# neuraloperator/pde-policylearning

Hardware: NVIDIA B200
Metric: fno2d_fwd_bwd_samples_per_s (higher is better)
Workload: dtype f32

## Files before the change

include/b2no.h:

```cpp
#ifndef B2NO_H
#define B2NO_H

#include <stdint.h>

#ifdef __cplusplus
extern "C" {
#endif

#define B2NO_MAX_DIM 3
#define B2NO_ABI_VERSION 5

enum { B2NO_NORM_BACKWARD = 0, B2NO_NORM_FORWARD = 1, B2NO_NORM_ORTHO = 2 };
enum { B2NO_ACT_NONE = 0, B2NO_ACT_GELU = 1, B2NO_ACT_RELU = 2, B2NO_ACT_SIGMOID = 3, B2NO_ACT_SELU = 4,
       B2NO_ACT_TANH = 5 };
enum { B2NO_E_ARG = -1, B2NO_E_UNSUPPORTED = -2, B2NO_E_NODEVICE = -3 };

typedef struct {
  int32_t ndim;
  int32_t nin[B2NO_MAX_DIM];
  int32_t nfft[B2NO_MAX_DIM];
  int32_t nout[B2NO_MAX_DIM];
  int32_t half[B2NO_MAX_DIM];
  int32_t norm;
  int32_t spec_layout;
} b2no_geom;

typedef struct b2no_plan b2no_plan;

typedef struct {
  const float* corner[4];
  int64_t stride_i, stride_o;
  int64_t stride_k[B2NO_MAX_DIM];
} b2no_weights;

typedef struct {
  const float* bias;
  const float* pw_w;  const float* pw_x;  int32_t pw_ci;  int32_t pw_transposed;
  const float* pw2_w; const float* pw2_x; int32_t pw2_ci; int32_t pw2_transposed;
  const float* add;
  const float* mul;
  float* preact;
  int32_t act;
  const float* dact_z;
  int32_t dact;
  const float* gate_z;
  const float* gate_h;
  int64_t mul_bstride;
  int64_t gate_bstride;
} b2no_epilogue;

int b2no_version(void);
const char* b2no_error_string(int code);
int b2no_device_info(int* sm_count, int* cc_major, int* cc_minor, int64_t* l2_bytes);

int b2no_plan_create(const b2no_geom* geom, b2no_plan** out);
int b2no_plan_destroy(b2no_plan* plan);
int b2no_plan_layout_supported(const b2no_plan* plan, int64_t batch, int64_t channels);
int b2no_plan_kept(const b2no_plan* plan, int32_t kept[B2NO_MAX_DIM]);
int64_t b2no_plan_workspace_floats(const b2no_plan* plan, int64_t batch, int64_t channels);
int b2no_set_tensor_core_mode(int on);
int b2no_set_precision(int mode);
int64_t b2no_tensor_core_launches(void);

int b2no_dft_forward(const b2no_plan* plan, int which, const float* x, float* spec, float* work,
                     int64_t bc, void* stream);
int b2no_dft_inverse(const b2no_plan* plan, int which, const float* spec, float* y, float* work,
                     int batch, int channels, int64_t pixels, const b2no_epilogue* epi, void* stream);

int b2no_mix(const b2no_plan* plan, int mode, const float* in, const b2no_weights* w, float* out,
             int batch, int ci, int co, int accumulate, void* stream);
int b2no_mix_dw(const b2no_plan* plan, const float* xh, const float* gyh, const b2no_weights* dw,
                int batch, int ci, int co, int accumulate, void* stream);

int b2no_act_bwd(const float* gy, const float* z, float* gz, int64_t n, int act, void* stream);
int64_t b2no_pw_wgrad_scratch_floats(int ci, int co);
int b2no_pw_wgrad(const float* g, const float* x, float* dw, float* db, float* partial, int batch, int ci,
                  int co, int64_t pixels, void* stream);
int b2no_dft_inverse_wgrad(const b2no_plan* plan, int which, const float* spec, float* y, float* work, int batch, int channels,
                           int64_t pixels, const b2no_epilogue* epi, const float* wg_x, int wg_ci, float* dw, float* db,
                           float* partial, void* stream);
int b2no_mlp_head_fwd(const float* x, const float* w1, const float* b1, const float* w2, const float* b2,
                      float* out, int batch, int ci, int hidden, int64_t pixels, int b1_per_sample,
                      int act, void* stream);
int64_t b2no_mlp_head_bwd_scratch_floats(int hidden);
int b2no_mlp_head_bwd_supported(int ci, int hidden, int64_t pixels);
int b2no_mlp_head_bwd(const float* x, const float* w1, const float* b1, const float* w2, const float* g, float* gx,
                      float* gz, float* dw2, float* partial, int batch, int ci, int hidden, int64_t pixels,
                      int b1_per_sample, int act, const float* dact_z, int dact, void* stream);
int64_t b2no_mlp_head_bwd_fused_scratch_floats(int ci, int hidden);
int b2no_mlp_head_bwd_fused_supported(int ci, int hidden, int64_t pixels);
int b2no_mlp_head_bwd_fused(const float* x, const float* w1, const float* b1, const float* w2, const float* g, float* gx,
                            float* grads, float* partial, int batch, int ci, int hidden, int64_t pixels, int act,
                            const float* dact_z, int dact, void* stream);
int b2no_rno_gate_fwd(const float* z, const float* z2, const float* hhat, const float* h, float* out,
                      int64_t n, void* stream);
int b2no_rno_gate_bwd(const float* g, const float* z, const float* z2, const float* hhat, const float* h,
                      float* gz, float* gz2, float* ghhat, float* gh, int64_t n, void* stream);
int b2no_rno_cell_bwd(const float* g, const float* h, const float* zz2, const float* ah, float* g_zz2, float* g_ah,
                      float* g_h, int batch, int c, int64_t p, void* stream);
int b2no_rno_reset_bwd(const float* g_rh, const float* h, const float* ar, float* g_ar, float* g_h, int64_t n,
                       void* stream);
int b2no_rel_l2_sums(const float* x, const float* y, float* sums, int batch, int64_t n_per_sample, void* stream);
int b2no_rel_l2_bwd(const float* x, const float* y, const float* coef, float* dx, int batch,
                    int64_t n_per_sample, void* stream);
int b2no_rel_l2_finish(const float* sums, float* loss, float* coef, int batch, int size_average, void* stream);
int b2no_rel_l2_bwd_g(const float* x, const float* y, const float* coef, const float* g, float* dx, int batch,
                      int64_t n_per_sample, void* stream);

int64_t b2no_pino_residual_scratch_floats(int B, int N, int T, int which);
int b2no_pino_residual_fwd(const float* w, const float* u0, const float* forcing, const float* nu, float t_interval,
                           float* du_p, float* fields, float* partial, float* loss, float* coef, int B, int N, int T,
                           void* stream);
int b2no_pino_residual_bwd(const float* w, const float* u0, const float* forcing, const float* nu, float t_interval,
                           const float* du_p, const float* fields, const float* coef, const float* gup, float* dw,
                           int B, int N, int T, void* stream);

int b2no_adam_step(float* param, const float* grad, float* exp_avg, float* exp_avg_sq, int64_t n, int* step_counter,
                   float lr, float beta1, float beta2, float eps, float weight_decay, float grad_scale, void* stream);
int64_t b2no_kernel_launches(void);

int b2no_gather_segments(float* flat, const void* src_ptrs, const int64_t* offsets, const int64_t* counts, int nseg,
                         void* stream);

int b2no_tc_peak_probe(int kind, int n_mma, double* flops, void* stream);

#ifdef __cplusplus
}
#endif
#endif
```

pde_policylearning_b200/_lib.py:

```python
from __future__ import annotations

import ctypes as C
import os
import subprocess
import sys

_HERE = os.path.dirname(os.path.abspath(__file__))
LIB_PATH = os.environ.get("B2NO_LIB") or os.path.join(_HERE, "libb2no.so")
CSRC = os.path.join(_HERE, "csrc")
SOURCES = ["plan.cu", "spectral.cu", "pointwise.cu", "tc_pointwise.cu", "tc_wgrad.cu", "tc_mlp.cu", "tc_head_bwd.cu", "tc_dft.cu", "tc_mix.cu", "tc_peak.cu", "pino_loss.cu", "optim.cu"]

MAX_DIM = 3
NORM = {"backward": 0, "forward": 1, "ortho": 2}
ACT = {None: 0, "none": 0, "identity": 0, "gelu": 1, "relu": 2, "sigmoid": 3, "selu": 4, "tanh": 5}


class Geom(C.Structure):
    _fields_ = [("ndim", C.c_int32), ("nin", C.c_int32 * MAX_DIM), ("nfft", C.c_int32 * MAX_DIM),
                ("nout", C.c_int32 * MAX_DIM), ("half", C.c_int32 * MAX_DIM), ("norm", C.c_int32),
                ("spec_layout", C.c_int32)]


class Weights(C.Structure):
    _fields_ = [("corner", C.c_void_p * 4), ("stride_i", C.c_int64), ("stride_o", C.c_int64),
                ("stride_k", C.c_int64 * MAX_DIM)]


class Epilogue(C.Structure):
    _fields_ = [("bias", C.c_void_p),
                ("pw_w", C.c_void_p), ("pw_x", C.c_void_p), ("pw_ci", C.c_int32), ("pw_transposed", C.c_int32),
                ("pw2_w", C.c_void_p), ("pw2_x", C.c_void_p), ("pw2_ci", C.c_int32), ("pw2_transposed", C.c_int32),
                ("add", C.c_void_p), ("mul", C.c_void_p), ("preact", C.c_void_p), ("act", C.c_int32),
                ("dact_z", C.c_void_p), ("dact", C.c_int32),
                ("gate_z", C.c_void_p), ("gate_h", C.c_void_p), ("mul_bstride", C.c_int64), ("gate_bstride", C.c_int64)]


NVCC_FLAGS = ["-O3", "-std=c++17", "-gencode", "arch=compute_100a,code=sm_100a", "-lineinfo", "-Xcompiler", "-fPIC"]
HEADERS = [os.path.join(CSRC, "common.cuh"), os.path.join(CSRC, "tc.cuh"), os.path.join(_HERE, "..", "include", "b2no.h")]


def build(force: bool = False, verbose: bool = False) -> str:
    from concurrent.futures import ThreadPoolExecutor
    hdr_time = max(os.path.getmtime(h) for h in HEADERS)
    if not force and os.path.exists(LIB_PATH) and os.path.getmtime(LIB_PATH) >= max(
            [hdr_time] + [os.path.getmtime(os.path.join(CSRC, s)) for s in SOURCES]):
        return LIB_PATH
    bdir = os.path.join(CSRC, "_build")
    os.makedirs(bdir, exist_ok=True)
    jobs, objs = [], []
    for s in SOURCES:
        src, obj = os.path.join(CSRC, s), os.path.join(bdir, s[:-3] + ".o")
        objs.append(obj)
        if force or not os.path.exists(obj) or os.path.getmtime(obj) < max(os.path.getmtime(src), hdr_time):
            jobs.append(["nvcc"] + NVCC_FLAGS + ["-c", "-o", obj, src])
    if not jobs and os.path.exists(LIB_PATH) and os.path.getmtime(LIB_PATH) >= max(os.path.getmtime(o) for o in objs):
        return LIB_PATH

    def run(cmd):
        if verbose:
            print(" ".join(cmd), file=sys.stderr)
        subprocess.run(cmd, check=True)

    with ThreadPoolExecutor(max_workers=min(8, max(1, len(jobs)))) as ex:
        list(ex.map(run, jobs))
    run(["nvcc"] + NVCC_FLAGS + ["-shared", "-o", LIB_PATH] + objs)
    return LIB_PATH


_lib = None


def lib():
    global _lib
    if _lib is not None:
        return _lib
    if not os.path.exists(LIB_PATH):
        raise RuntimeError(
            f"{LIB_PATH} not found: build it with `python -c 'import __graft_entry__ as g; g.build()'` "
            "(nvcc, sm_100a).  There is no CPU / PyTorch fallback for the spectral-conv hot path.")
    L = C.CDLL(LIB_PATH)
    vp, i32, i64 = C.c_void_p, C.c_int, C.c_int64
    L.b2no_version.restype = i32
    L.b2no_error_string.restype = C.c_char_p
    L.b2no_error_string.argtypes = [i32]
    L.b2no_device_info.argtypes = [C.POINTER(i32), C.POINTER(i32), C.POINTER(i32), C.POINTER(i64)]
    L.b2no_plan_create.argtypes = [C.POINTER(Geom), C.POINTER(vp)]
    L.b2no_plan_destroy.argtypes = [vp]
    L.b2no_plan_kept.argtypes = [vp, C.POINTER(C.c_int32 * MAX_DIM)]
    L.b2no_plan_layout_supported.argtypes = [vp, i64, i64]
    L.b2no_plan_workspace_floats.restype = i64
    L.b2no_plan_workspace_floats.argtypes = [vp, i64, i64]
    L.b2no_set_tensor_core_mode.argtypes = [i32]
    L.b2no_set_precision.argtypes = [i32]
    L.b2no_tensor_core_launches.restype = i64
    L.b2no_kernel_launches.restype = i64
    L.b2no_dft_forward.argtypes = [vp, i32, vp, vp, vp, i64, vp]
    L.b2no_dft_inverse.argtypes = [vp, i32, vp, vp, vp, i32, i32, i64, C.POINTER(Epilogue), vp]
    L.b2no_mix.argtypes = [vp, i32, vp, C.POINTER(Weights), vp, i32, i32, i32, i32, vp]
    L.b2no_mix_dw.argtypes = [vp, vp, vp, C.POINTER(Weights), i32, i32, i32, i32, vp]
    L.b2no_act_bwd.argtypes = [vp, vp, vp, i64, i32, vp]
    L.b2no_pw_wgrad_scratch_floats.restype = i64
    L.b2no_pw_wgrad_scratch_floats.argtypes = [i32, i32]
    L.b2no_pw_wgrad.argtypes = [vp, vp, vp, vp, vp, i32, i32, i32, i64, vp]
    L.b2no_dft_inverse_wgrad.argtypes = [vp, i32, vp, vp, vp, i32, i32, i64, C.POINTER(Epilogue), vp, i32, vp, vp, vp, vp]
    L.b2no_mlp_head_fwd.argtypes = [vp, vp, vp, vp, vp, vp, i32, i32, i32, i64, i32, i32, vp]
    L.b2no_mlp_head_bwd_supported.argtypes = [i32, i32, i64]
    L.b2no_mlp_head_bwd_scratch_floats.restype = i64
    L.b2no_mlp_head_bwd_scratch_floats.argtypes = [i32]
    L.b2no_mlp_head_bwd.argtypes = [vp] * 9 + [i32, i32, i32, i64, i32, i32, vp, i32, vp]
    L.b2no_mlp_head_bwd_fused_supported.argtypes = [i32, i32, i64]
    L.b2no_mlp_head_bwd_fused_scratch_floats.restype = i64
    L.b2no_mlp_head_bwd_fused_scratch_floats.argtypes = [i32, i32]
    L.b2no_mlp_head_bwd_fused.argtypes = [vp] * 8 + [i32, i32, i32, i64, i32, vp, i32, vp]
    L.b2no_rno_gate_fwd.argtypes = [vp, vp, vp, vp, vp, i64, vp]
    L.b2no_rno_gate_bwd.argtypes = [vp] * 9 + [i64, vp]
    L.b2no_rno_cell_bwd.argtypes = [vp] * 7 + [i32, i32, i64, vp]
    L.b2no_rno_reset_bwd.argtypes = [vp] * 5 + [i64, vp]
    L.b2no_rel_l2_sums.argtypes = [vp, vp, vp, i32, i64, vp]
    L.b2no_rel_l2_bwd.argtypes = [vp, vp, vp, vp, i32, i64, vp]
    L.b2no_rel_l2_finish.argtypes = [vp, vp, vp, i32, i32, vp]
    L.b2no_rel_l2_bwd_g.argtypes = [vp, vp, vp, vp, vp, i32, i64, vp]
    L.b2no_gather_segments.argtypes = [vp, vp, vp, vp, i32, vp]
    f32 = C.c_float
    L.b2no_adam_step.argtypes = [vp, vp, vp, vp, i64, vp, f32, f32, f32, f32, f32, f32, vp]
    L.b2no_pino_residual_scratch_floats.restype = i64
    L.b2no_pino_residual_scratch_floats.argtypes = [i32, i32, i32, i32]
    L.b2no_pino_residual_fwd.argtypes = [vp, vp, vp, vp, f32, vp, vp, vp, vp, vp, i32, i32, i32, vp]
    L.b2no_pino_residual_bwd.argtypes = [vp, vp, vp, vp, f32, vp, vp, vp, vp, vp, i32, i32, i32, vp]
    L.b2no_tc_peak_probe.argtypes = [i32, i32, C.POINTER(C.c_double), vp]
    for name in EXPORTS:
        getattr(L, name)
    _lib = L
    return L


EXPORTS = [
    "b2no_version", "b2no_error_string", "b2no_device_info",
    "b2no_plan_create", "b2no_plan_destroy", "b2no_plan_kept", "b2no_plan_layout_supported", "b2no_plan_workspace_floats",
    "b2no_set_tensor_core_mode", "b2no_set_precision", "b2no_tensor_core_launches", "b2no_kernel_launches",
    "b2no_dft_forward", "b2no_dft_inverse", "b2no_mix", "b2no_mix_dw",
    "b2no_act_bwd", "b2no_pw_wgrad_scratch_floats", "b2no_pw_wgrad", "b2no_dft_inverse_wgrad", "b2no_mlp_head_fwd", "b2no_mlp_head_bwd_scratch_floats", "b2no_mlp_head_bwd_supported", "b2no_mlp_head_bwd",
    "b2no_mlp_head_bwd_fused_scratch_floats", "b2no_mlp_head_bwd_fused_supported", "b2no_mlp_head_bwd_fused",
    "b2no_rno_gate_fwd", "b2no_rno_gate_bwd", "b2no_rno_cell_bwd", "b2no_rno_reset_bwd", "b2no_rel_l2_sums", "b2no_rel_l2_bwd",
    "b2no_rel_l2_finish", "b2no_rel_l2_bwd_g", "b2no_adam_step", "b2no_gather_segments",
    "b2no_tc_peak_probe", "b2no_pino_residual_scratch_floats", "b2no_pino_residual_fwd", "b2no_pino_residual_bwd",
]


def check(code: int, what: str = "") -> None:
    if code != 0:
        msg = lib().b2no_error_string(int(code)).decode()
        raise RuntimeError(f"b2no {what} failed: {msg} (code {code})")
```

pde_policylearning_b200/csrc/common.cuh:

```cuda
#pragma once
#include <cuda_runtime.h>
#include <stdint.h>
#include "../../include/b2no.h"

#define B2NO_CHECK_CUDA(expr)                      \
  do {                                             \
    cudaError_t _e = (expr);                       \
    if (_e != cudaSuccess) return (int)_e;         \
  } while (0)

extern long long g_b2no_launches;
#define B2NO_LAUNCH_CHECK()                        \
  do {                                             \
    cudaError_t _e = cudaGetLastError();           \
    if (_e != cudaSuccess) return (int)_e;         \
    g_b2no_launches++;                             \
  } while (0)

static inline int b2no_ceil_div(long a, long b) { return (int)((a + b - 1) / b); }
static inline int b2no_round_up(int a, int b) { return ((a + b - 1) / b) * b; }

int b2no_sm_count();
int b2no_tc_passes();
bool b2no_tc_available();
int b2no_tc_mlp_fwd(const float* x, const float* w1, const float* b1, const float* w2, const float* b2, float* out, int batch,
                    int ci, int hidden, int co2, long pixels, int b1_per_sample, int act, cudaStream_t st);
int b2no_tc_wgrad(const float* g, const float* x, float* partial, int max_blocks, int batch, int ci, int co, long pixels,
                  int* nblk, cudaStream_t st);
struct b2no_tc_wg {
  const float* x;
  int ci;
  float* partial;
  int* nblk;
};
int b2no_tc_pointwise(const b2no_plan* plan, int which, const float* spec, float* y, float* work, int batch, int channels,
                      long pixels, const b2no_epilogue* e, cudaStream_t st, const b2no_tc_wg* wg = nullptr);

struct b2no_tc_tables {
  float* timg;
  int Ks, Qp, R;
};

struct b2no_tc_fwd_tables {
  float* tb;
  float* mimg;
  int W, H, N1, Kx, Ky;
};
int b2no_tc_dft_forward(const b2no_plan* plan, int which, const float* x, float* spec, long planes, cudaStream_t st);

struct b2no_plan {
  b2no_geom g;
  b2no_tc_tables tc[2];
  b2no_tc_fwd_tables tcf[2];
  int K[B2NO_MAX_DIM];
  int device;
  float* t_in;
  float* t_out;
  int npad_in, npad_out, q2, qc, nchunk, qpad;
  float2* m_fwd[2];
  float2* m_inv[2];
  float2* m_adjinv[2];
  float2* m_adjfwd[2];
  int* row_corner[2];
  int* row_local[2];
};

struct ModeMap {
  const int* corner[2];
  const int* local[2];
  int K[3];
  int ndim;
};

__device__ __forceinline__ void decode_mode(const ModeMap& mm, const b2no_weights& w, int k, int* corner,
                                            long* woff) {
  int c = 0;
  long off = 0;
  const int d = mm.ndim;
  int rem = k;
  int idx[3] = {0, 0, 0};
  for (int j = d - 1; j >= 0; j--) {
    idx[j] = rem % mm.K[j];
    rem /= mm.K[j];
  }
  for (int j = 0; j < d - 1; j++) {
    c = c * 2 + mm.corner[j][idx[j]];
    off += (long)mm.local[j][idx[j]] * w.stride_k[j];
  }
  off += (long)idx[d - 1] * w.stride_k[d - 1];
  *corner = c;
  *woff = off;
}

static inline ModeMap make_mode_map(const b2no_plan* p) {
  ModeMap mm;
  mm.ndim = p->g.ndim;
  for (int j = 0; j < 3; j++) mm.K[j] = j < p->g.ndim ? p->K[j] : 1;
  for (int j = 0; j < 2; j++) { mm.corner[j] = p->row_corner[j]; mm.local[j] = p->row_local[j]; }
  return mm;
}

static inline int total_modes(const b2no_plan* p) {
  int kt = 1;
  for (int j = 0; j < p->g.ndim; j++) kt *= p->K[j];
  return kt;
}

int b2no_tc_mix_feasible(int batch, int ci, int co, int mode);
int b2no_tc_mix_dw_feasible(int batch, int ci, int co);
int b2no_tc_mix(const b2no_plan* p, int mode, const float* in, const b2no_weights* w, float* out, int batch, int ci, int co,
                int accumulate, cudaStream_t st);
int b2no_tc_mix_dw(const b2no_plan* p, const float* xh, const float* gyh, const b2no_weights* dw, int batch, int ci, int co,
                   int accumulate, cudaStream_t st);

__device__ __forceinline__ float b2no_erf(float x) {
  x = fminf(fmaxf(x, -4.0f), 4.0f);
  const float x2 = x * x;
  float p = -2.72614225801306e-10f;
  p = fmaf(p, x2, 2.77068142495902e-08f);
  p = fmaf(p, x2, -2.10102402082508e-06f);
  p = fmaf(p, x2, -5.69250639462346e-05f);
  p = fmaf(p, x2, -7.34990630326855e-04f);
  p = fmaf(p, x2, -2.95459980854025e-03f);
  p = fmaf(p, x2, -1.60960333262415e-02f);
  float q = -1.45660718464996e-05f;
  q = fmaf(q, x2, -2.13374055278905e-04f);
  q = fmaf(q, x2, -1.68282697438203e-03f);
  q = fmaf(q, x2, -7.37332916720468e-03f);
  q = fmaf(q, x2, -1.42647390514189e-02f);
  return __fdividef(x * p, q);
}

__device__ __forceinline__ float2 b2no_f2(float a) { return make_float2(a, a); }
__device__ __forceinline__ float b2no_rcp(float x) {
  float r;
  asm("rcp.approx.ftz.f32 %0, %1;" : "=f"(r) : "f"(x));
  return r;
}
__device__ __forceinline__ float b2no_ex2(float x) {
  float r;
  asm("ex2.approx.ftz.f32 %0, %1;" : "=f"(r) : "f"(x));
  return r;
}
__device__ __forceinline__ float2 b2no_erf2(float2 x) {
  x.x = fminf(fmaxf(x.x, -4.0f), 4.0f);
  x.y = fminf(fmaxf(x.y, -4.0f), 4.0f);
  const float2 x2 = __fmul2_rn(x, x);
  float2 p = b2no_f2(-2.72614225801306e-10f);
  p = __ffma2_rn(p, x2, b2no_f2(2.77068142495902e-08f));
  p = __ffma2_rn(p, x2, b2no_f2(-2.10102402082508e-06f));
  p = __ffma2_rn(p, x2, b2no_f2(-5.69250639462346e-05f));
  p = __ffma2_rn(p, x2, b2no_f2(-7.34990630326855e-04f));
  p = __ffma2_rn(p, x2, b2no_f2(-2.95459980854025e-03f));
  p = __ffma2_rn(p, x2, b2no_f2(-1.60960333262415e-02f));
  float2 q = b2no_f2(-1.45660718464996e-05f);
  q = __ffma2_rn(q, x2, b2no_f2(-2.13374055278905e-04f));
  q = __ffma2_rn(q, x2, b2no_f2(-1.68282697438203e-03f));
  q = __ffma2_rn(q, x2, b2no_f2(-7.37332916720468e-03f));
  q = __ffma2_rn(q, x2, b2no_f2(-1.42647390514189e-02f));
  const float2 r = make_float2(b2no_rcp(q.x), b2no_rcp(q.y));
  return __fmul2_rn(__fmul2_rn(x, p), r);
}
__device__ __forceinline__ float2 b2no_gelu2(float2 x) {
  const float2 e = b2no_erf2(__fmul2_rn(x, b2no_f2(0.70710678118654752440f)));
  const float2 h = __fmul2_rn(x, b2no_f2(0.5f));
  return __ffma2_rn(h, e, h);
}
__device__ __forceinline__ void b2no_gelu2_both(float2 x, float2* val, float2* grad) {
  const float2 ax = make_float2(fabsf(x.x), fabsf(x.y));
  const float2 den = __ffma2_rn(ax, b2no_f2(0.23164189f), b2no_f2(1.0f));
  const float2 t = make_float2(b2no_rcp(den.x), b2no_rcp(den.y));
  float2 q = __ffma2_rn(b2no_f2(1.061405429f), t, b2no_f2(-1.453152027f));
  q = __ffma2_rn(q, t, b2no_f2(1.421413741f));
  q = __ffma2_rn(q, t, b2no_f2(-0.284496736f));
  q = __ffma2_rn(q, t, b2no_f2(0.254829592f));
  q = __fmul2_rn(q, t);
  const float2 a = __fmul2_rn(__fmul2_rn(x, x), b2no_f2(-0.72134752044448170368f));
  const float2 g = make_float2(b2no_ex2(a.x), b2no_ex2(a.y));
  const float2 h = __ffma2_rn(__fmul2_rn(q, g), b2no_f2(-0.5f), b2no_f2(0.5f));
  const float2 cdf = __fadd2_rn(b2no_f2(0.5f), make_float2(copysignf(h.x, x.x), copysignf(h.y, x.y)));
  *val = __fmul2_rn(x, cdf);
  *grad = __ffma2_rn(__fmul2_rn(x, b2no_f2(0.39894228040143267794f)), g, cdf);
}
__device__ __forceinline__ float2 b2no_gelu2_grad(float2 x) {
  float2 v, g;
  b2no_gelu2_both(x, &v, &g);
  return g;
}

__device__ __forceinline__ float b2no_act(float x, int act) {
  switch (act) {
    case B2NO_ACT_GELU: return 0.5f * x * (1.0f + b2no_erf(x * 0.70710678118654752440f));
    case B2NO_ACT_RELU: return x > 0.f ? x : 0.f;
    case B2NO_ACT_SIGMOID: return 1.0f / (1.0f + expf(-x));
    case B2NO_ACT_SELU: {
      const float scale = 1.0507009873554804934193349852946f, alpha = 1.6732632423543772848170429916717f;
      return x > 0.f ? scale * x : scale * alpha * expm1f(x);
    }
    case B2NO_ACT_TANH: return tanhf(x);
    default: return x;
  }
}

__device__ __forceinline__ float b2no_act_grad(float x, int act) {
  switch (act) {
    case B2NO_ACT_GELU: {
      const float cdf = 0.5f * (1.0f + b2no_erf(x * 0.70710678118654752440f));
      const float pdf = 0.39894228040143267794f * __expf(-0.5f * x * x);
      return cdf + x * pdf;
    }
    case B2NO_ACT_RELU: return x > 0.f ? 1.f : 0.f;
    case B2NO_ACT_SIGMOID: {
      const float s = 1.0f / (1.0f + expf(-x));
      return s * (1.0f - s);
    }
    case B2NO_ACT_SELU: {
      const float scale = 1.0507009873554804934193349852946f, alpha = 1.6732632423543772848170429916717f;
      return x > 0.f ? scale : scale * alpha * expf(x);
    }
    case B2NO_ACT_TANH: {
      const float t = tanhf(x);
      return 1.0f - t * t;
    }
    default: return 1.f;
  }
}
```

pde_policylearning_b200/csrc/spectral.cu:

```cuda
#include <string.h>
#include "common.cuh"

template <int QC>
__global__ void __launch_bounds__(256)
k_r2c_last(const float* __restrict__ x, float* __restrict__ out, const float* __restrict__ tab,
           long R, int N, int npad, int q2, int nchunk) {
  extern __shared__ float s_tab[];
  const int qpad = QC * nchunk;
  for (int i = threadIdx.x; i < qpad * npad; i += blockDim.x) s_tab[i] = tab[i];
  __syncthreads();

  const int lane = threadIdx.x & 31, warp = threadIdx.x >> 5;
  const int npl = (N + 31) >> 5;
  const long ngroups = (R + 7) >> 3;
  for (long g = (long)blockIdx.x * 8 + warp; g < ngroups; g += (long)gridDim.x * 8) {
    const long r0 = g << 3;
    for (int c = 0; c < nchunk; c++) {
      float v[8 * QC];
#pragma unroll
      for (int i = 0; i < 8 * QC; i++) v[i] = 0.f;
      for (int j = 0; j < npl; j++) {
        const int n = lane + (j << 5);
        float xv[8];
#pragma unroll
        for (int r = 0; r < 8; r++) xv[r] = (n < N && r0 + r < R) ? __ldg(x + (r0 + r) * N + n) : 0.f;
        const float* tq = s_tab + (size_t)(c * QC) * npad + n;
#pragma unroll
        for (int q = 0; q < QC; q++) {
          const float t = tq[(size_t)q * npad];
#pragma unroll
          for (int r = 0; r < 8; r++) v[r * QC + q] = fmaf(xv[r], t, v[r * QC + q]);
        }
      }
#pragma unroll
      for (int s = 0; s < 5; s++) {
        const int off = 16 >> s;
        const int half = (8 * QC) >> (s + 1);
        const bool upper = (lane & off) != 0;
#pragma unroll
        for (int i = 0; i < half; i++) {
          const float a = v[i], b = v[i + half];
          const float send = upper ? a : b;
          const float keep = upper ? b : a;
          v[i] = keep + __shfl_xor_sync(0xffffffffu, send, off);
        }
      }
      constexpr int PER = QC / 4;
#pragma unroll
      for (int i = 0; i < PER; i++) {
        const int idx = lane * PER + i;
        const int r = idx / QC, q = c * QC + idx % QC;
        if (r0 + r < R && q < q2) out[(r0 + r) * q2 + q] = v[i];
      }
    }
  }
}

template <int QC>
static int launch_r2c(const float* x, float* out, const float* tab, long R, int N, int npad, int q2,
                      int nchunk, cudaStream_t st) {
  const size_t smem = (size_t)QC * nchunk * npad * sizeof(float);
  if (smem > 200 * 1024) return B2NO_E_UNSUPPORTED;
  if (smem > 48 * 1024)
    B2NO_CHECK_CUDA(cudaFuncSetAttribute(k_r2c_last<QC>, cudaFuncAttributeMaxDynamicSharedMemorySize, (int)smem));
  const long ngroups = (R + 7) / 8;
  long blocks = (ngroups + 7) / 8;
  const long cap = (long)b2no_sm_count() * 8;
  if (blocks > cap) blocks = cap;
  if (blocks < 1) blocks = 1;
  k_r2c_last<QC><<<(unsigned)blocks, 256, smem, st>>>(x, out, tab, R, N, npad, q2, nchunk);
  B2NO_LAUNCH_CHECK();
  return 0;
}

template <int QL>
__global__ void __launch_bounds__(256)
k_r2c_rows(const float* __restrict__ x, float* __restrict__ out, const float* __restrict__ tab, long R, int N, int npad, int q2) {
  extern __shared__ float s_dyn[];
  constexpr int Q2P = 4 * QL;
  float* s_tabT = s_dyn;
  float* s_rows = s_dyn + (size_t)N * Q2P;
  for (int i = threadIdx.x; i < N * Q2P; i += 256) {
    const int n = i / Q2P, q = i - n * Q2P;
    s_tabT[i] = q < q2 ? tab[(size_t)q * npad + n] : 0.f;
  }
  __syncthreads();
  const int lane = threadIdx.x & 31, warp = threadIdx.x >> 5;
  float* rows = s_rows + (size_t)warp * 8 * N;
  const int r = lane >> 2, q0 = (lane & 3) * QL;
  const long ngroups = R >> 3;
  for (long g = (long)blockIdx.x * 8 + warp; g < ngroups; g += (long)gridDim.x * 8) {
    const float4* src = reinterpret_cast<const float4*>(x + (g << 3) * N);
    for (int i = lane; i < 2 * N; i += 32) reinterpret_cast<float4*>(rows)[i] = __ldg(src + i);
    __syncwarp();
    float acc[QL];
#pragma unroll
    for (int i = 0; i < QL; i++) acc[i] = 0.f;
    const float* xr = rows + r * N;
#pragma unroll 4
    for (int n = 0; n < N; n++) {
      const float xv = xr[n];
      const float* t = s_tabT + n * Q2P + q0;
#pragma unroll
      for (int i = 0; i < QL; i++) acc[i] = fmaf(xv, t[i], acc[i]);
    }
    float* dst = out + ((g << 3) + r) * q2 + q0;
#pragma unroll
    for (int i = 0; i < QL; i++)
      if (q0 + i < q2) dst[i] = acc[i];
    __syncwarp();
  }
}

template <int Q2P>
__global__ void __launch_bounds__(256)
k_r2c_rows32(const float* __restrict__ x, float* __restrict__ out, const float* __restrict__ tab, long R, int N, int npad, int q2) {
  extern __shared__ float s_dyn[];
  const int NS = N | 1;
  float* s_tabT = s_dyn;
  float* s_rows = s_dyn + (size_t)N * Q2P;
  for (int i = threadIdx.x; i < N * Q2P; i += 256) {
    const int n = i / Q2P, q = i - n * Q2P;
    s_tabT[i] = q < q2 ? tab[(size_t)q * npad + n] : 0.f;
  }
  __syncthreads();
  const int lane = threadIdx.x & 31, warp = threadIdx.x >> 5;
  float* rows = s_rows + (size_t)warp * 32 * NS;
  const long ngroups = R >> 5;
  for (long g = (long)blockIdx.x * 8 + warp; g < ngroups; g += (long)gridDim.x * 8) {
    const float* src = x + (g << 5) * N;
    if (NS == N) {
      const float4* s4 = reinterpret_cast<const float4*>(src);
      for (int i = lane; i < 8 * N; i += 32) reinterpret_cast<float4*>(rows)[i] = __ldg(s4 + i);
    } else {
      for (int i = lane; i < 32 * N; i += 32) {
        const int rr = i / N, n = i - rr * N;
        rows[rr * NS + n] = __ldg(src + i);
      }
    }
    __syncwarp();
    float acc[Q2P];
#pragma unroll
    for (int i = 0; i < Q2P; i++) acc[i] = 0.f;
    const float* xr = rows + lane * NS;
#pragma unroll 2
    for (int n = 0; n < N; n++) {
      const float xv = xr[n];
      const float4* t4 = reinterpret_cast<const float4*>(s_tabT + n * Q2P);
#pragma unroll
      for (int i = 0; i < Q2P / 4; i++) {
        const float4 t = t4[i];
        acc[4 * i] = fmaf(xv, t.x, acc[4 * i]);
        acc[4 * i + 1] = fmaf(xv, t.y, acc[4 * i + 1]);
        acc[4 * i + 2] = fmaf(xv, t.z, acc[4 * i + 2]);
        acc[4 * i + 3] = fmaf(xv, t.w, acc[4 * i + 3]);
      }
    }
    float* dst = out + ((g << 5) + lane) * q2;
    if (q2 == Q2P) {
#pragma unroll
      for (int i = 0; i < Q2P / 4; i++)
        reinterpret_cast<float4*>(dst)[i] = make_float4(acc[4 * i], acc[4 * i + 1], acc[4 * i + 2], acc[4 * i + 3]);
    } else {
#pragma unroll
      for (int i = 0; i < Q2P; i++)
        if (i < q2) dst[i] = acc[i];
    }
    __syncwarp();
  }
}

template <int Q2P>
static int launch_r2c_rows32(const float* x, float* out, const float* tab, long R, int N, int npad, int q2, cudaStream_t st) {
  const size_t smem = ((size_t)N * Q2P + (size_t)8 * 32 * (N | 1)) * sizeof(float);
  if (smem > 48 * 1024)
    B2NO_CHECK_CUDA(cudaFuncSetAttribute(k_r2c_rows32<Q2P>, cudaFuncAttributeMaxDynamicSharedMemorySize, (int)smem));
  const long ngroups = R / 32;
  long blocks = (ngroups + 7) / 8;
  const long cap = (long)b2no_sm_count() * 4;
  if (blocks > cap) blocks = cap;
  if (blocks < 1) blocks = 1;
  k_r2c_rows32<Q2P><<<(unsigned)blocks, 256, smem, st>>>(x, out, tab, R, N, npad, q2);
  B2NO_LAUNCH_CHECK();
  return 0;
}

template <int QL>
static int launch_r2c_rows(const float* x, float* out, const float* tab, long R, int N, int npad, int q2, cudaStream_t st) {
  const size_t smem = ((size_t)N * 4 * QL + (size_t)8 * 8 * N) * sizeof(float);
  if (smem > 48 * 1024)
    B2NO_CHECK_CUDA(cudaFuncSetAttribute(k_r2c_rows<QL>, cudaFuncAttributeMaxDynamicSharedMemorySize, (int)smem));
  const long ngroups = R / 8;
  long blocks = (ngroups + 7) / 8;
  const long cap = (long)b2no_sm_count() * 8;
  if (blocks > cap) blocks = cap;
  if (blocks < 1) blocks = 1;
  k_r2c_rows<QL><<<(unsigned)blocks, 256, smem, st>>>(x, out, tab, R, N, npad, q2);
  B2NO_LAUNCH_CHECK();
  return 0;
}

static int run_r2c(const b2no_plan* p, int which, const float* x, float* out, long R, cudaStream_t st) {
  const int d = p->g.ndim;
  const int N = which == 0 ? p->g.nin[d - 1] : p->g.nout[d - 1];
  const int npad = which == 0 ? p->npad_in : p->npad_out;
  const float* tab = which == 0 ? p->t_in : p->t_out;
  if (R % 32 == 0 && R >= 32 * 8 * 64 && p->q2 <= 16 && p->q2 % 4 == 0 && N >= 8 && N <= 160 && (((uintptr_t)x) & 15) == 0 &&
      (((uintptr_t)out) & 15) == 0) {
    if (p->q2 <= 8) return launch_r2c_rows32<8>(x, out, tab, R, N, npad, p->q2, st);
    return launch_r2c_rows32<16>(x, out, tab, R, N, npad, p->q2, st);
  }
  if (R % 8 == 0 && p->q2 <= 16 && N >= 8 && N <= 512 && (((uintptr_t)x) & 15) == 0) {
    if (p->q2 <= 4) return launch_r2c_rows<1>(x, out, tab, R, N, npad, p->q2, st);
    if (p->q2 <= 8) return launch_r2c_rows<2>(x, out, tab, R, N, npad, p->q2, st);
    return launch_r2c_rows<4>(x, out, tab, R, N, npad, p->q2, st);
  }
  switch (p->qc) {
    case 4: return launch_r2c<4>(x, out, tab, R, N, npad, p->q2, p->nchunk, st);
    case 8: return launch_r2c<8>(x, out, tab, R, N, npad, p->q2, p->nchunk, st);
    case 12: return launch_r2c<12>(x, out, tab, R, N, npad, p->q2, p->nchunk, st);
    case 16: return launch_r2c<16>(x, out, tab, R, N, npad, p->q2, p->nchunk, st);
  }
  return B2NO_E_UNSUPPORTED;
}

template <int MT>
__global__ void __launch_bounds__(128)
k_cmat(const float2* __restrict__ in, float2* __restrict__ out, const float2* __restrict__ T,
       long outer, int J, int M, int inner) {
  extern __shared__ float2 s_T[];
  const int m0 = blockIdx.y * MT;
  for (int idx = threadIdx.x; idx < J * MT; idx += blockDim.x) {
    const int j = idx / MT, mm = idx - j * MT;
    s_T[idx] = (m0 + mm < M) ? T[(size_t)j * M + m0 + mm] : make_float2(0.f, 0.f);
  }
  __syncthreads();
  const long total = outer * inner;
  for (long t = (long)blockIdx.x * blockDim.x + threadIdx.x; t < total; t += (long)gridDim.x * blockDim.x) {
    const long o = t / inner;
    const int i = (int)(t - o * inner);
    float2 acc[MT];
#pragma unroll
    for (int mm = 0; mm < MT; mm++) acc[mm] = make_float2(0.f, 0.f);
    const float2* src = in + (o * J) * inner + i;
#pragma unroll 4
    for (int j = 0; j < J; j++) {
      const float2 v = __ldg(src + (size_t)j * inner);
      const float2* trow = s_T + j * MT;
#pragma unroll
      for (int mm = 0; mm < MT; mm++) {
        const float2 w = trow[mm];
        acc[mm].x = fmaf(v.x, w.x, fmaf(-v.y, w.y, acc[mm].x));
        acc[mm].y = fmaf(v.x, w.y, fmaf(v.y, w.x, acc[mm].y));
      }
    }
#pragma unroll
    for (int mm = 0; mm < MT; mm++)
      if (m0 + mm < M) out[(o * M + m0 + mm) * inner + i] = acc[mm];
  }
}

template <int MT>
static int launch_cmat(const float2* in, float2* out, const float2* T, long outer, int J, int M, int inner,
                       cudaStream_t st) {
  const size_t smem = (size_t)J * MT * sizeof(float2);
  if (smem > 200 * 1024) return B2NO_E_UNSUPPORTED;
  if (smem > 48 * 1024)
    B2NO_CHECK_CUDA(cudaFuncSetAttribute(k_cmat<MT>, cudaFuncAttributeMaxDynamicSharedMemorySize, (int)smem));
  const long total = outer * inner;
  long bx = (total + 127) / 128;
  const long cap = (long)b2no_sm_count() * 16;
  if (bx > cap) bx = cap;
  if (bx < 1) bx = 1;
  dim3 grid((unsigned)bx, (unsigned)((M + MT - 1) / MT));
  k_cmat<MT><<<grid, 128, smem, st>>>(in, out, T, outer, J, M, inner);
  B2NO_LAUNCH_CHECK();
  return 0;
}

static int run_cmat(const float2* in, float2* out, const float2* T, long outer, int J, int M, int inner,
                    cudaStream_t st) {
  if (M <= 4) return launch_cmat<4>(in, out, T, outer, J, M, inner, st);
  if (M <= 8) return launch_cmat<8>(in, out, T, outer, J, M, inner, st);
  if (M <= 12 || M == 24) return launch_cmat<12>(in, out, T, outer, J, M, inner, st);
  return launch_cmat<16>(in, out, T, outer, J, M, inner, st);
}

template <int KL>
__global__ void __launch_bounds__(256)
k_fwd_plane32(const float* __restrict__ x, float2* __restrict__ spec, const float* __restrict__ tab, int npad,
              const float2* __restrict__ M, long planes, int H, int W, int K0, int Kl, int layout) {
  extern __shared__ float2 sm2[];
  float2* sT = sm2;
  float2* sM = sT + 32 * KL;
  float2* sA = sM + 32 * 32;
  const int lane = threadIdx.x & 31, warp = threadIdx.x >> 5;
  for (int i = threadIdx.x; i < 32 * KL; i += 256) {
    const int w = i / KL, ky = i - w * KL;
    sT[i] = (w < W && ky < Kl) ? make_float2(__ldg(tab + (size_t)(2 * ky) * npad + w), __ldg(tab + (size_t)(2 * ky + 1) * npad + w))
                               : make_float2(0.f, 0.f);
  }
  for (int i = threadIdx.x; i < 32 * 32; i += 256) {
    const int h = i >> 5, kx = i & 31;
    sM[i] = (h < H && kx < K0) ? __ldg(M + (size_t)h * K0 + kx) : make_float2(0.f, 0.f);
  }
  __syncthreads();
  float2* myA = sA + (size_t)warp * 32 * (KL + 2);
  for (long p0 = (long)blockIdx.x * 8; p0 < planes; p0 += (long)gridDim.x * 8) {
    const long plane = p0 + warp;
    const bool live = plane < planes;
    float xr[32];
#pragma unroll
    for (int w = 0; w < 32; w++) xr[w] = 0.f;
    if (live && lane < H) {
      const float4* row = reinterpret_cast<const float4*>(x + ((size_t)plane * H + lane) * W);
#pragma unroll
      for (int w4 = 0; w4 < 8; w4++)
        if (w4 * 4 < W) {
          const float4 v = __ldg(row + w4);
          xr[4 * w4] = v.x; xr[4 * w4 + 1] = v.y; xr[4 * w4 + 2] = v.z; xr[4 * w4 + 3] = v.w;
        }
    }
    float2 acc[KL];
#pragma unroll
    for (int k = 0; k < KL; k++) acc[k] = make_float2(0.f, 0.f);
#pragma unroll
    for (int w = 0; w < 32; w++) {
      if (w < W) {
        const float2 xx = make_float2(xr[w], xr[w]);
#pragma unroll
        for (int k = 0; k < KL; k += 2) {
          const float4 t = *reinterpret_cast<const float4*>(sT + w * KL + k);
          acc[k] = __ffma2_rn(xx, make_float2(t.x, t.y), acc[k]);
          acc[k + 1] = __ffma2_rn(xx, make_float2(t.z, t.w), acc[k + 1]);
        }
      }
    }
#pragma unroll
    for (int k = 0; k < KL; k++) myA[lane * (KL + 2) + k] = acc[k];
    __syncwarp();
    float2 pr[KL], pi[KL];
#pragma unroll
    for (int k = 0; k < KL; k++) { pr[k] = make_float2(0.f, 0.f); pi[k] = make_float2(0.f, 0.f); }
    for (int h = 0; h < H; h++) {
      const float2 m = sM[h * 32 + lane];
      const float2 mr = make_float2(m.x, m.x), mi = make_float2(m.y, m.y);
#pragma unroll
      for (int k = 0; k < KL; k += 2) {
        const float4 a = *reinterpret_cast<const float4*>(myA + h * (KL + 2) + k);
        pr[k] = __ffma2_rn(mr, make_float2(a.x, a.y), pr[k]);
        pi[k] = __ffma2_rn(mi, make_float2(a.x, a.y), pi[k]);
        pr[k + 1] = __ffma2_rn(mr, make_float2(a.z, a.w), pr[k + 1]);
        pi[k + 1] = __ffma2_rn(mi, make_float2(a.z, a.w), pi[k + 1]);
      }
    }
    if (layout == 0) {
      if (live && lane < K0) {
        float2* dst = spec + ((size_t)plane * K0 + lane) * Kl;
#pragma unroll
        for (int k = 0; k < KL; k++)
          if (k < Kl) dst[k] = make_float2(pr[k].x - pi[k].y, pr[k].y + pi[k].x);
      }
      __syncwarp();
    } else {
      if (live && lane < K0) {
        float2* dst = spec + (size_t)lane * Kl * planes + plane;
#pragma unroll
        for (int k = 0; k < KL; k++)
          if (k < Kl) dst[(size_t)k * planes] = make_float2(pr[k].x - pi[k].y, pr[k].y + pi[k].x);
      }
      __syncwarp();
    }
  }
}

static int launch_fwd_plane32(const b2no_plan* p, int which, const float* x, float* spec, long planes, cudaStream_t st) {
  const int32_t* n = which == 0 ? p->g.nin : p->g.nout;
  const int H = n[0], W = n[1], K0 = p->K[0], Kl = p->K[1];
  const float* tab = which == 0 ? p->t_in : p->t_out;
  const int npad = which == 0 ? p->npad_in : p->npad_out;
  const float2* M = which == 0 ? p->m_fwd[0] : p->m_adjinv[0];
  const int KL = Kl <= 8 ? 8 : (Kl <= 12 ? 12 : 16);
  const size_t smem = sizeof(float2) * ((size_t)32 * KL + 32 * 32 + (size_t)8 * 32 * (KL + 2));
  long blocks = (planes + 7) / 8;
  const long cap = (long)b2no_sm_count() * 8;
  if (blocks > cap) blocks = cap;
#define FP32_LAUNCH(K)                                                                                                      \
  do {                                                                                                                      \
    if (smem > 48 * 1024) B2NO_CHECK_CUDA(cudaFuncSetAttribute(k_fwd_plane32<K>, cudaFuncAttributeMaxDynamicSharedMemorySize, (int)smem)); \
    k_fwd_plane32<K><<<(unsigned)blocks, 256, smem, st>>>(x, (float2*)spec, tab, npad, M, planes, H, W, K0, Kl, p->g.spec_layout); \
  } while (0)
  if (KL == 8) FP32_LAUNCH(8); else if (KL == 12) FP32_LAUNCH(12); else FP32_LAUNCH(16);
#undef FP32_LAUNCH
  B2NO_LAUNCH_CHECK();
  return 0;
}

extern "C" int b2no_dft_forward(const b2no_plan* p, int which, const float* x, float* spec, float* work,
                                int64_t bc, void* stream) {
  if (!p || !x || !spec || bc < 1 || (which != 0 && which != 1)) return B2NO_E_ARG;
  cudaStream_t st = (cudaStream_t)stream;
  const int d = p->g.ndim;
  const int32_t* n = which == 0 ? p->g.nin : p->g.nout;
  const int Kl = p->K[d - 1];
  if (d == 1) return run_r2c(p, which, x, spec, bc, st);
  if (d == 2) {
    if (n[0] <= 32 && n[1] <= 32 && n[1] % 4 == 0 && p->K[0] <= 32 && Kl <= 16 && (((uintptr_t)x) & 15) == 0 &&
        (p->g.spec_layout == 0 || p->g.spec_layout == 1))
      return launch_fwd_plane32(p, which, x, spec, (long)bc, st);
    const int rc = b2no_tc_dft_forward(p, which, x, spec, (long)bc, st);
    if (rc != 1) return rc;
  }
  if (p->g.spec_layout != 0) return B2NO_E_UNSUPPORTED;
  if (!work) return B2NO_E_ARG;
  float2* A = (float2*)work;
  if (d == 2) {
    int rc = run_r2c(p, which, x, (float*)A, bc * n[0], st);
    if (rc) return rc;
    const float2* T = which == 0 ? p->m_fwd[0] : p->m_adjinv[0];
    return run_cmat(A, (float2*)spec, T, bc, n[0], p->K[0], Kl, st);
  }
  float2* Bb = A + (size_t)bc * n[0] * n[1] * Kl;
  int rc = run_r2c(p, which, x, (float*)A, bc * n[0] * n[1], st);
  if (rc) return rc;
  const float2* T1 = which == 0 ? p->m_fwd[1] : p->m_adjinv[1];
  rc = run_cmat(A, Bb, T1, bc * n[0], n[1], p->K[1], Kl, st);
  if (rc) return rc;
  const float2* T0 = which == 0 ? p->m_fwd[0] : p->m_adjinv[0];
  return run_cmat(Bb, (float2*)spec, T0, bc, n[0], p->K[0], p->K[1] * Kl, st);
}

template <int BT, int PT, bool CONJT>
__global__ void __launch_bounds__(128)
k_mix(const float2* __restrict__ in, float2* __restrict__ out, b2no_weights w, ModeMap mm, int B, int Cq,
      int Cp, int Kt, int accumulate) {
  const int k = blockIdx.x * blockDim.x + threadIdx.x;
  if (k >= Kt) return;
  const int b0 = blockIdx.y * BT, p0 = blockIdx.z * PT;
  int corner;
  long woff;
  decode_mode(mm, w, k, &corner, &woff);
  const float2* wbase = (const float2*)w.corner[corner] + woff;
  float2 acc[BT][PT];
#pragma unroll
  for (int bb = 0; bb < BT; bb++)
#pragma unroll
    for (int pp = 0; pp < PT; pp++) acc[bb][pp] = make_float2(0.f, 0.f);
  for (int q = 0; q < Cq; q++) {
    float2 xin[BT], wv[PT];
#pragma unroll
    for (int bb = 0; bb < BT; bb++)
      xin[bb] = (b0 + bb < B) ? __ldg(in + ((size_t)(b0 + bb) * Cq + q) * Kt + k) : make_float2(0.f, 0.f);
#pragma unroll
    for (int pp = 0; pp < PT; pp++) {
      float2 t = make_float2(0.f, 0.f);
      if (p0 + pp < Cp) {
        const long off = CONJT ? ((long)(p0 + pp) * w.stride_i + (long)q * w.stride_o)
                               : ((long)q * w.stride_i + (long)(p0 + pp) * w.stride_o);
        t = __ldg(wbase + off);
        if (CONJT) t.y = -t.y;
      }
      wv[pp] = t;
    }
#pragma unroll
    for (int bb = 0; bb < BT; bb++)
#pragma unroll
      for (int pp = 0; pp < PT; pp++) {
        acc[bb][pp].x = fmaf(xin[bb].x, wv[pp].x, fmaf(-xin[bb].y, wv[pp].y, acc[bb][pp].x));
        acc[bb][pp].y = fmaf(xin[bb].x, wv[pp].y, fmaf(xin[bb].y, wv[pp].x, acc[bb][pp].y));
      }
  }
#pragma unroll
  for (int bb = 0; bb < BT; bb++)
#pragma unroll
    for (int pp = 0; pp < PT; pp++)
      if (b0 + bb < B && p0 + pp < Cp) {
        float2* dst = out + ((size_t)(b0 + bb) * Cp + p0 + pp) * Kt + k;
        float2 r = acc[bb][pp];
        if (accumulate) { const float2 old = *dst; r.x += old.x; r.y += old.y; }
        *dst = r;
      }
}

template <bool CONJT>
__global__ void __launch_bounds__(256)
k_mix2(const float2* __restrict__ in, float2* __restrict__ out, b2no_weights w, ModeMap mm, int B, int Cq, int Cp,
       int Kt, int accumulate) {
  const long idx = (long)blockIdx.x * 256 + threadIdx.x;
  if (idx >= (long)B * Cp * Kt) return;
  const int k = (int)(idx % Kt);
  const long t = idx / Kt;
  const int pp = (int)(t % Cp), b = (int)(t / Cp);
  int corner;
  long woff;
  decode_mode(mm, w, k, &corner, &woff);
  const float2* wp = (const float2*)w.corner[corner] + woff + (CONJT ? (long)pp * w.stride_i : (long)pp * w.stride_o);
  const long wq = CONJT ? w.stride_o : w.stride_i;
  const float2* xp = in + (size_t)b * Cq * Kt + k;
  float2 acc = make_float2(0.f, 0.f);
  int q = 0;
  for (; q + 8 <= Cq; q += 8) {
    float2 xv[8], wv[8];
#pragma unroll
    for (int u = 0; u < 8; u++) {
      xv[u] = __ldg(xp + (size_t)(q + u) * Kt);
      wv[u] = __ldg(wp + (long)(q + u) * wq);
    }
#pragma unroll
    for (int u = 0; u < 8; u++) {
      const float wy = CONJT ? -wv[u].y : wv[u].y;
      acc.x = fmaf(xv[u].x, wv[u].x, fmaf(-xv[u].y, wy, acc.x));
      acc.y = fmaf(xv[u].x, wy, fmaf(xv[u].y, wv[u].x, acc.y));
    }
  }
  for (; q < Cq; q++) {
    const float2 xv = __ldg(xp + (size_t)q * Kt), wv = __ldg(wp + (long)q * wq);
    const float wy = CONJT ? -wv.y : wv.y;
    acc.x = fmaf(xv.x, wv.x, fmaf(-xv.y, wy, acc.x));
    acc.y = fmaf(xv.x, wy, fmaf(xv.y, wv.x, acc.y));
  }
  float2* dst = out + ((size_t)b * Cp + pp) * Kt + k;
  if (accumulate) { const float2 old = *dst; acc.x += old.x; acc.y += old.y; }
  *dst = acc;
}

__global__ void __launch_bounds__(256)
k_dw2(const float2* __restrict__ xh, const float2* __restrict__ gyh, b2no_weights w, ModeMap mm, int B, int Ci, int Co,
      int Kt, int accumulate) {
  const long idx = (long)blockIdx.x * 256 + threadIdx.x;
  if (idx >= (long)Ci * Co * Kt) return;
  const int k = (int)(idx % Kt);
  const long t = idx / Kt;
  const int o = (int)(t % Co), i = (int)(t / Co);
  const float2* xp = xh + (size_t)i * Kt + k;
  const float2* gp = gyh + (size_t)o * Kt + k;
  const size_t xs = (size_t)Ci * Kt, gs = (size_t)Co * Kt;
  float2 acc = make_float2(0.f, 0.f);
  int b = 0;
  for (; b + 8 <= B; b += 8) {
    float2 xv[8], gv[8];
#pragma unroll
    for (int u = 0; u < 8; u++) {
      xv[u] = __ldg(xp + (size_t)(b + u) * xs);
      gv[u] = __ldg(gp + (size_t)(b + u) * gs);
    }
#pragma unroll
    for (int u = 0; u < 8; u++) {
      acc.x = fmaf(xv[u].x, gv[u].x, fmaf(xv[u].y, gv[u].y, acc.x));
      acc.y = fmaf(xv[u].x, gv[u].y, fmaf(-xv[u].y, gv[u].x, acc.y));
    }
  }
  for (; b < B; b++) {
    const float2 xv = __ldg(xp + (size_t)b * xs), gv = __ldg(gp + (size_t)b * gs);
    acc.x = fmaf(xv.x, gv.x, fmaf(xv.y, gv.y, acc.x));
    acc.y = fmaf(xv.x, gv.y, fmaf(-xv.y, gv.x, acc.y));
  }
  int corner;
  long woff;
  decode_mode(mm, w, k, &corner, &woff);
  float2* dst = (float2*)w.corner[corner] + woff + (long)i * w.stride_i + (long)o * w.stride_o;
  if (accumulate) { const float2 old = *dst; acc.x += old.x; acc.y += old.y; }
  *dst = acc;
}

extern "C" int b2no_mix(const b2no_plan* p, int mode, const float* in, const b2no_weights* w, float* out,
                        int batch, int ci, int co, int accumulate, void* stream) {
  if (!p || !in || !w || !out || batch < 1 || ci < 1 || co < 1 || (mode != 0 && mode != 1)) return B2NO_E_ARG;
  cudaStream_t st = (cudaStream_t)stream;
  const int Kt = total_modes(p);
  const ModeMap mm = make_mode_map(p);
  {
    const int rc = b2no_tc_mix(p, mode, in, w, out, batch, ci, co, accumulate, st);
    if (rc != 1) return rc;
  }
  if (p->g.spec_layout != 0) return B2NO_E_UNSUPPORTED;
  const int Cq = mode == 0 ? ci : co, Cp = mode == 0 ? co : ci;
  const long total = (long)batch * Cp * Kt;
  const unsigned blocks = (unsigned)((total + 255) / 256);
  if (mode == 0)
    k_mix2<false><<<blocks, 256, 0, st>>>((const float2*)in, (float2*)out, *w, mm, batch, Cq, Cp, Kt, accumulate);
  else
    k_mix2<true><<<blocks, 256, 0, st>>>((const float2*)in, (float2*)out, *w, mm, batch, Cq, Cp, Kt, accumulate);
  B2NO_LAUNCH_CHECK();
  return 0;
}

template <int IT, int OT>
__global__ void __launch_bounds__(128)
k_dw(const float2* __restrict__ xh, const float2* __restrict__ gyh, b2no_weights w, ModeMap mm, int B, int Ci,
     int Co, int Kt, int accumulate) {
  const int k = blockIdx.x * blockDim.x + threadIdx.x;
  if (k >= Kt) return;
  const int i0 = blockIdx.y * IT, o0 = blockIdx.z * OT;
  int corner;
  long woff;
  decode_mode(mm, w, k, &corner, &woff);
  float2 acc[IT][OT];
#pragma unroll
  for (int ii = 0; ii < IT; ii++)
#pragma unroll
    for (int oo = 0; oo < OT; oo++) acc[ii][oo] = make_float2(0.f, 0.f);
  for (int b = 0; b < B; b++) {
    float2 xi[IT], go[OT];
#pragma unroll
    for (int ii = 0; ii < IT; ii++)
      xi[ii] = (i0 + ii < Ci) ? __ldg(xh + ((size_t)b * Ci + i0 + ii) * Kt + k) : make_float2(0.f, 0.f);
#pragma unroll
    for (int oo = 0; oo < OT; oo++)
      go[oo] = (o0 + oo < Co) ? __ldg(gyh + ((size_t)b * Co + o0 + oo) * Kt + k) : make_float2(0.f, 0.f);
#pragma unroll
    for (int ii = 0; ii < IT; ii++)
#pragma unroll
      for (int oo = 0; oo < OT; oo++) {
        acc[ii][oo].x = fmaf(xi[ii].x, go[oo].x, fmaf(xi[ii].y, go[oo].y, acc[ii][oo].x));
        acc[ii][oo].y = fmaf(xi[ii].x, go[oo].y, fmaf(-xi[ii].y, go[oo].x, acc[ii][oo].y));
      }
  }
  float2* wbase = (float2*)w.corner[corner] + woff;
#pragma unroll
  for (int ii = 0; ii < IT; ii++)
#pragma unroll
    for (int oo = 0; oo < OT; oo++)
      if (i0 + ii < Ci && o0 + oo < Co) {
        float2* dst = wbase + (long)(i0 + ii) * w.stride_i + (long)(o0 + oo) * w.stride_o;
        float2 r = acc[ii][oo];
        if (accumulate) { const float2 old = *dst; r.x += old.x; r.y += old.y; }
        *dst = r;
      }
}

template <int BT>
__global__ void __launch_bounds__(256)
k_dw_small(const float2* __restrict__ xh, const float2* __restrict__ gyh, b2no_weights w, ModeMap mm, int B, int Ci, int Co,
           int Kt, int accumulate) {
  const int k = blockIdx.x * 256 + threadIdx.x;
  const int i = blockIdx.y;
  if (k >= Kt) return;
  int corner;
  long woff;
  decode_mode(mm, w, k, &corner, &woff);
  float2 xv[BT];
#pragma unroll
  for (int b = 0; b < BT; b++) xv[b] = b < B ? __ldg(xh + ((size_t)b * Ci + i) * Kt + k) : make_float2(0.f, 0.f);
  float2* dst = (float2*)w.corner[corner] + woff + (long)i * w.stride_i;
  const float2* gp = gyh + k;
  for (int o = 0; o < Co; o++) {
    float2 acc = make_float2(0.f, 0.f);
#pragma unroll
    for (int b = 0; b < BT; b++) {
      if (b < B) {
        const float2 gv = __ldg(gp + ((size_t)b * Co + o) * Kt);
        acc.x = fmaf(xv[b].x, gv.x, fmaf(xv[b].y, gv.y, acc.x));
        acc.y = fmaf(xv[b].x, gv.y, fmaf(-xv[b].y, gv.x, acc.y));
      }
    }
    float2* d = dst + (long)o * w.stride_o;
    if (accumulate) { const float2 old = *d; acc.x += old.x; acc.y += old.y; }
    *d = acc;
  }
}

extern "C" int b2no_mix_dw(const b2no_plan* p, const float* xh, const float* gyh, const b2no_weights* dw,
                           int batch, int ci, int co, int accumulate, void* stream) {
  if (!p || !xh || !gyh || !dw || batch < 1 || ci < 1 || co < 1) return B2NO_E_ARG;
  cudaStream_t st = (cudaStream_t)stream;
  const int Kt = total_modes(p);
  const ModeMap mm = make_mode_map(p);
  {
    const int rc = b2no_tc_mix_dw(p, xh, gyh, dw, batch, ci, co, accumulate, st);
    if (rc != 1) return rc;
  }
  if (p->g.spec_layout != 0) return B2NO_E_UNSUPPORTED;
  if (batch <= 8 && Kt >= 256) {
    dim3 grid((unsigned)((Kt + 255) / 256), (unsigned)ci);
    if (batch <= 4)
      k_dw_small<4><<<grid, 256, 0, st>>>((const float2*)xh, (const float2*)gyh, *dw, mm, batch, ci, co, Kt, accumulate);
    else
      k_dw_small<8><<<grid, 256, 0, st>>>((const float2*)xh, (const float2*)gyh, *dw, mm, batch, ci, co, Kt, accumulate);
    B2NO_LAUNCH_CHECK();
    return 0;
  }
  const long total = (long)ci * co * Kt;
  k_dw2<<<(unsigned)((total + 255) / 256), 256, 0, st>>>((const float2*)xh, (const float2*)gyh, *dw, mm, batch, ci, co, Kt, accumulate);
  B2NO_LAUNCH_CHECK();
  return 0;
}

struct EpiDev {
  const float* bias;
  const float* pw_w; const float* pw_x; int pw_ci; int pw_t;
  const float* pw2_w; const float* pw2_x; int pw2_ci; int pw2_t;
  const float* add;
  const float* mul;
  float* preact;
  int act;
  const float* dz;
  int dact;
  const float* gate_z; const float* gate_h;
  long mul_bs, gate_bs;
};

template <int NPT, int OT>
__global__ void __launch_bounds__(256)
k_c2r_fused(const float2* __restrict__ spec, float* __restrict__ y, const float* __restrict__ tab, EpiDev e,
            int B, int Co, long RPI, int N, long P, int Kd, int npad) {
  extern __shared__ float smem[];
  const int n_ot = (Co + OT - 1) / OT;
  const int copad = n_ot * OT;
  const int q2 = spec ? 2 * Kd : 0;
  float* s_tab = smem;
  float* s_w1 = s_tab + (size_t)q2 * npad;
  float* s_w2 = s_w1 + (size_t)e.pw_ci * copad;
  for (int i = threadIdx.x; i < q2 * npad; i += blockDim.x) s_tab[i] = tab[i];
  for (int i = threadIdx.x; i < e.pw_ci * copad; i += blockDim.x) {
    const int ci = i / copad, o = i - ci * copad;
    float v = 0.f;
    if (o < Co) v = e.pw_t ? e.pw_w[(size_t)ci * Co + o] : e.pw_w[(size_t)o * e.pw_ci + ci];
    s_w1[i] = v;
  }
  for (int i = threadIdx.x; i < e.pw2_ci * copad; i += blockDim.x) {
    const int ci = i / copad, o = i - ci * copad;
    float v = 0.f;
    if (o < Co) v = e.pw2_t ? e.pw2_w[(size_t)ci * Co + o] : e.pw2_w[(size_t)o * e.pw2_ci + ci];
    s_w2[i] = v;
  }
  __syncthreads();

  const int lane = threadIdx.x & 31, warp = threadIdx.x >> 5;
  const int n_nc = (N + 32 * NPT - 1) / (32 * NPT);
  const long n_items = (long)B * RPI * n_nc * n_ot;
  const bool plain = !e.add && !e.preact && !e.mul && !e.dz && !e.gate_z && e.act == B2NO_ACT_NONE;
  for (long item = (long)blockIdx.x * 8 + warp; item < n_items; item += (long)gridDim.x * 8) {
    const int ot = (int)(item % n_ot);
    long t = item / n_ot;
    const int nc = (int)(t % n_nc);
    t /= n_nc;
    const long r = t % RPI;
    const int b = (int)(t / RPI);
    const int o0 = ot * OT;
    const int nbase = nc * 32 * NPT;

    float acc[OT][NPT];
#pragma unroll
    for (int oo = 0; oo < OT; oo++)
#pragma unroll
      for (int j = 0; j < NPT; j++) acc[oo][j] = 0.f;

    if (spec) {
      const float2* sp = spec + (((size_t)b * Co + o0) * RPI + r) * Kd;
      const size_t ostride = (size_t)RPI * Kd;
      for (int k = 0; k < Kd; k++) {
        float tr[NPT], ti[NPT];
#pragma unroll
        for (int j = 0; j < NPT; j++) {
          const int n = nbase + lane + 32 * j;
          tr[j] = s_tab[(size_t)(2 * k) * npad + n];
          ti[j] = s_tab[(size_t)(2 * k + 1) * npad + n];
        }
#pragma unroll
        for (int oo = 0; oo < OT; oo++) {
          if (o0 + oo < Co) {
            const float2 v = __ldg(sp + oo * ostride + k);
#pragma unroll
            for (int j = 0; j < NPT; j++) acc[oo][j] = fmaf(v.x, tr[j], fmaf(v.y, ti[j], acc[oo][j]));
          }
        }
      }
    }
    bool valid[NPT];
    long pix[NPT];
#pragma unroll
    for (int j = 0; j < NPT; j++) {
      const int n = nbase + lane + 32 * j;
      pix[j] = r * N + n;
      valid[j] = (n < N) && (pix[j] < P);
    }
    if (e.pw_ci > 0) {
      const float* xb = e.pw_x + (size_t)b * e.pw_ci * P;
      for (int i = 0; i < e.pw_ci; i++) {
        float xv[NPT];
#pragma unroll
        for (int j = 0; j < NPT; j++) xv[j] = valid[j] ? __ldg(xb + (size_t)i * P + pix[j]) : 0.f;
        const float* wr = s_w1 + (size_t)i * copad + o0;
#pragma unroll
        for (int oo = 0; oo < OT; oo++) {
          const float wv = wr[oo];
#pragma unroll
          for (int j = 0; j < NPT; j++) acc[oo][j] = fmaf(wv, xv[j], acc[oo][j]);
        }
      }
    }
    if (e.pw2_ci > 0) {
      const float* xb = e.pw2_x + (size_t)b * e.pw2_ci * P;
      for (int i = 0; i < e.pw2_ci; i++) {
        float xv[NPT];
#pragma unroll
        for (int j = 0; j < NPT; j++) xv[j] = valid[j] ? __ldg(xb + (size_t)i * P + pix[j]) : 0.f;
        const float* wr = s_w2 + (size_t)i * copad + o0;
#pragma unroll
        for (int oo = 0; oo < OT; oo++) {
          const float wv = wr[oo];
#pragma unroll
          for (int j = 0; j < NPT; j++) acc[oo][j] = fmaf(wv, xv[j], acc[oo][j]);
        }
      }
    }
#pragma unroll
    for (int oo = 0; oo < OT; oo++) {
      const int o = o0 + oo;
      if (o < Co) {
        const float bv = e.bias ? __ldg(e.bias + o) : 0.f;
        if (plain) {
          float* yr = y + ((size_t)b * Co + o) * P + (size_t)r * N + nbase + lane;
#pragma unroll
          for (int j = 0; j < NPT; j++)
            if (valid[j]) yr[32 * j] = acc[oo][j] + bv;
          continue;
        }
#pragma unroll
        for (int j = 0; j < NPT; j++) {
          if (valid[j]) {
            const size_t idx = ((size_t)b * Co + o) * P + pix[j];
            float z = acc[oo][j] + bv;
            if (e.add) z += __ldg(e.add + idx);
            if (e.preact) e.preact[idx] = z;
            float v = b2no_act(z, e.act);
            const size_t inner = (size_t)o * P + pix[j];
            if (e.mul) v *= __ldg(e.mul + (size_t)b * e.mul_bs + inner);
            if (e.dz) v *= b2no_act_grad(__ldg(e.dz + idx), e.dact);
            if (e.gate_z) v = fmaf(1.0f - __ldg(e.gate_z + (size_t)b * e.gate_bs + inner), __ldg(e.gate_h + idx), v);
            y[idx] = v;
          }
        }
      }
    }
  }
}

template <int NPT, int OT>
static int launch_c2r(const float2* spec, float* y, const float* tab, const EpiDev& e, int B, int Co, long RPI,
                      int N, long P, int Kd, int npad, cudaStream_t st) {
  const int n_ot = (Co + OT - 1) / OT;
  const int copad = n_ot * OT;
  const size_t smem = ((size_t)(spec ? 2 * Kd : 0) * npad + (size_t)(e.pw_ci + e.pw2_ci) * copad) * sizeof(float);
  if (smem > 200 * 1024) return B2NO_E_UNSUPPORTED;
  if (smem > 48 * 1024)
    B2NO_CHECK_CUDA(cudaFuncSetAttribute(k_c2r_fused<NPT, OT>, cudaFuncAttributeMaxDynamicSharedMemorySize, (int)smem));
  const int n_nc = (N + 32 * NPT - 1) / (32 * NPT);
  const long n_items = (long)B * RPI * n_nc * n_ot;
  long blocks = (n_items + 7) / 8;
  const long cap = (long)b2no_sm_count() * 4;
  if (blocks > cap) blocks = cap;
  if (blocks < 1) blocks = 1;
  k_c2r_fused<NPT, OT><<<(unsigned)blocks, 256, smem, st>>>(spec, y, tab, e, B, Co, RPI, N, P, Kd, npad);
  B2NO_LAUNCH_CHECK();
  return 0;
}

template <int NPT>
__global__ void __launch_bounds__(256)
k_c2r_plain8(const float2* __restrict__ spec, float* __restrict__ y, const float* __restrict__ tab,
             const float* __restrict__ bias, int B, int Co, long RPI, int N, long P, int npad) {
  constexpr int OT = 16, KD = 8;
  extern __shared__ float s_tab8[];
  for (int i = threadIdx.x; i < 2 * KD * npad; i += blockDim.x) s_tab8[i] = tab[i];
  __syncthreads();
  const int lane = threadIdx.x & 31, warp = threadIdx.x >> 5;
  const int n_ot = (Co + OT - 1) / OT;
  const int n_nc = (N + 32 * NPT - 1) / (32 * NPT);
  const long n_items = (long)B * RPI * n_nc * n_ot;
  const size_t ostride = (size_t)RPI * KD;
  auto fetch = [&](long item, float2 (&v)[4]) {
    const int ot = (int)(item % n_ot);
    long t = item / n_ot / n_nc;
    const long r = t % RPI;
    const int b = (int)(t / RPI);
    const float2* sp = spec + (((size_t)b * Co + ot * OT) * RPI + r) * KD;
#pragma unroll
    for (int m = 0; m < 4; m++) {
      const int idx = lane + 32 * m, oo = idx >> 3, k = idx & 7;
      v[m] = (ot * OT + oo < Co) ? __ldg(sp + oo * ostride + k) : make_float2(0.f, 0.f);
    }
  };
  long item = (long)blockIdx.x * 8 + warp;
  const long step = (long)gridDim.x * 8;
  float2 cur[4], nxt[4];
  if (item < n_items) fetch(item, cur);
  for (; item < n_items; item += step) {
    if (item + step < n_items) fetch(item + step, nxt);
    const int ot = (int)(item % n_ot);
    long t = item / n_ot;
    const int nc = (int)(t % n_nc);
    t /= n_nc;
    const long r = t % RPI;
    const int b = (int)(t / RPI);
    const int o0 = ot * OT, nbase = nc * 32 * NPT;
    float acc[OT][NPT];
#pragma unroll
    for (int oo = 0; oo < OT; oo++)
#pragma unroll
      for (int j = 0; j < NPT; j++) acc[oo][j] = 0.f;
#pragma unroll
    for (int k = 0; k < KD; k++) {
      float tr[NPT], ti[NPT];
#pragma unroll
      for (int j = 0; j < NPT; j++) {
        const int n = nbase + lane + 32 * j;
        tr[j] = s_tab8[(size_t)(2 * k) * npad + n];
        ti[j] = s_tab8[(size_t)(2 * k + 1) * npad + n];
      }
#pragma unroll
      for (int oo = 0; oo < OT; oo++) {
        const int idx = oo * KD + k;
        const float vx = __shfl_sync(0xffffffffu, cur[idx >> 5].x, idx & 31);
        const float vy = __shfl_sync(0xffffffffu, cur[idx >> 5].y, idx & 31);
#pragma unroll
        for (int j = 0; j < NPT; j++) acc[oo][j] = fmaf(vx, tr[j], fmaf(vy, ti[j], acc[oo][j]));
      }
    }
#pragma unroll
    for (int oo = 0; oo < OT; oo++) {
      const int o = o0 + oo;
      if (o < Co) {
        const float bv = bias ? __ldg(bias + o) : 0.f;
        float* yr = y + ((size_t)b * Co + o) * P + (size_t)r * N + nbase + lane;
#pragma unroll
        for (int j = 0; j < NPT; j++) {
          const int n = nbase + lane + 32 * j;
          if (n < N) yr[32 * j] = acc[oo][j] + bv;
        }
      }
    }
#pragma unroll
    for (int m = 0; m < 4; m++) cur[m] = nxt[m];
  }
}

template <int NPT>
static int launch_c2r_plain8(const float2* spec, float* y, const float* tab, const float* bias, int B, int Co, long RPI,
                             int N, long P, int npad, cudaStream_t st) {
  const size_t smem = (size_t)16 * npad * sizeof(float);
  if (smem > 48 * 1024)
    B2NO_CHECK_CUDA(cudaFuncSetAttribute(k_c2r_plain8<NPT>, cudaFuncAttributeMaxDynamicSharedMemorySize, (int)smem));
  const int n_ot = (Co + 15) / 16, n_nc = (N + 32 * NPT - 1) / (32 * NPT);
  const long n_items = (long)B * RPI * n_nc * n_ot;
  long blocks = (n_items + 7) / 8;
  const long cap = (long)b2no_sm_count() * 6;
  if (blocks > cap) blocks = cap;
  if (blocks < 1) blocks = 1;
  k_c2r_plain8<NPT><<<(unsigned)blocks, 256, smem, st>>>(spec, y, tab, bias, B, Co, RPI, N, P, npad);
  B2NO_LAUNCH_CHECK();
  return 0;
}

static int run_c2r(const float2* spec, float* y, const float* tab, const EpiDev& e, int B, int Co, long RPI, int N,
                   long P, int Kd, int npad, cudaStream_t st) {
  constexpr int OT = 16;
  const bool plain = !e.add && !e.preact && !e.mul && !e.dz && !e.gate_z && e.act == B2NO_ACT_NONE;
  if (spec && plain && e.pw_ci == 0 && e.pw2_ci == 0 && Kd == 8 && npad * 16 * 4 <= 160 * 1024) {
    if (N <= 32) return launch_c2r_plain8<1>(spec, y, tab, e.bias, B, Co, RPI, N, P, npad, st);
    if (N <= 64) return launch_c2r_plain8<2>(spec, y, tab, e.bias, B, Co, RPI, N, P, npad, st);
    if (N <= 96) return launch_c2r_plain8<3>(spec, y, tab, e.bias, B, Co, RPI, N, P, npad, st);
    if (N <= 128) return launch_c2r_plain8<4>(spec, y, tab, e.bias, B, Co, RPI, N, P, npad, st);
  }
  if (N <= 32) return launch_c2r<1, OT>(spec, y, tab, e, B, Co, RPI, N, P, Kd, npad, st);
  if (N <= 64) return launch_c2r<2, OT>(spec, y, tab, e, B, Co, RPI, N, P, Kd, npad, st);
  if (N <= 96) return launch_c2r<3, OT>(spec, y, tab, e, B, Co, RPI, N, P, Kd, npad, st);
  return launch_c2r<4, OT>(spec, y, tab, e, B, Co, RPI, N, P, Kd, npad, st);
}

extern "C" int b2no_plan_layout_supported(const b2no_plan* p, int64_t batch, int64_t channels) {
  if (!p || batch < 1 || channels < 1) return 0;
  if (p->g.spec_layout == 0) return 1;
  if (!b2no_tc_available() || p->g.ndim != 2) return 0;
  if (!p->tcf[0].tb || !p->tcf[1].tb || !p->tc[0].timg || !p->tc[1].timg) return 0;
  if (((long)p->g.nin[0] * p->g.nin[1]) % 128 != 0 || ((long)p->g.nout[0] * p->g.nout[1]) % 128 != 0) return 0;
  if (p->K[0] > 32) return 0;
  if (((size_t)2 * channels * ((size_t)p->K[0] * p->K[1] + 1) + (size_t)p->K[0] * 32) * 8 > 200 * 1024) return 0;
  const int c = (int)channels, b = (int)(batch > 1 << 30 ? 1 << 30 : batch);
  return b2no_tc_mix_feasible(b, c, c, 0) && b2no_tc_mix_feasible(b, c, 2 * c, 0) && b2no_tc_mix_feasible(b, c, 2 * c, 1) &&
         b2no_tc_mix_dw_feasible(b, c, c) && b2no_tc_mix_dw_feasible(b, c, 2 * c);
}

__global__ void k_fill_identity(float* m, int n) {
  const int i = blockIdx.x * blockDim.x + threadIdx.x;
  if (i < n * n) m[i] = (i / n == i % n) ? 1.0f : 0.0f;
}
static const float* identity_matrix(int n, cudaStream_t st) {
  static float* cache[8][129] = {};
  int dev = 0;
  if (n < 1 || n > 128 || cudaGetDevice(&dev) != cudaSuccess || dev < 0 || dev >= 8) return nullptr;
  if (!cache[dev][n]) {
    cudaStreamCaptureStatus cs = cudaStreamCaptureStatusNone;
    if (cudaStreamIsCapturing(st, &cs) != cudaSuccess || cs != cudaStreamCaptureStatusNone) return nullptr;
    float* m = nullptr;
    if (cudaMalloc(&m, (size_t)n * n * sizeof(float)) != cudaSuccess) return nullptr;
    k_fill_identity<<<(n * n + 255) / 256, 256, 0, st>>>(m, n);
    if (cudaGetLastError() != cudaSuccess) { cudaFree(m); return nullptr; }
    cache[dev][n] = m;
  }
  return cache[dev][n];
}

extern "C" int b2no_dft_inverse(const b2no_plan* p, int which, const float* spec, float* y, float* work,
                                int batch, int channels, int64_t pixels, const b2no_epilogue* epi, void* stream) {
  if (!y || batch < 1 || channels < 1 || (which != 0 && which != 1)) return B2NO_E_ARG;
  cudaStream_t st = (cudaStream_t)stream;
  EpiDev e;
  memset(&e, 0, sizeof(e));
  if (epi) {
    e.bias = epi->bias;
    e.pw_w = epi->pw_w; e.pw_x = epi->pw_x; e.pw_ci = (epi->pw_w && epi->pw_x) ? epi->pw_ci : 0; e.pw_t = epi->pw_transposed;
    e.pw2_w = epi->pw2_w; e.pw2_x = epi->pw2_x; e.pw2_ci = (epi->pw2_w && epi->pw2_x) ? epi->pw2_ci : 0; e.pw2_t = epi->pw2_transposed;
    e.add = epi->add; e.mul = epi->mul; e.preact = epi->preact; e.act = epi->act;
    e.dz = epi->dact_z; e.dact = epi->dact_z ? epi->dact : 0;
    e.gate_z = (epi->gate_z && epi->gate_h) ? epi->gate_z : nullptr; e.gate_h = e.gate_z ? epi->gate_h : nullptr;
    if (e.pw_ci < 0 || e.pw2_ci < 0 || epi->mul_bstride < 0 || epi->gate_bstride < 0) return B2NO_E_ARG;
  }
  if (epi && (spec == nullptr || (p && p->g.ndim == 2))) {
    long px = pixels;
    if (spec && p) {
      const int32_t* nn = which == 0 ? p->g.nout : p->g.nin;
      px = (long)nn[0] * nn[1];
      if (pixels > 0 && pixels != px) return B2NO_E_ARG;
    }
    const int rc = b2no_tc_pointwise(p, which, spec, y, work, batch, channels, px, epi, st);
    if (rc != 1) return rc;
  }
  if (spec && p && p->g.spec_layout != 0) return B2NO_E_UNSUPPORTED;
  auto set_strides = [&](long P_) {
    e.mul_bs = (epi && epi->mul_bstride) ? (long)epi->mul_bstride : (long)channels * P_;
    e.gate_bs = (epi && epi->gate_bstride) ? (long)epi->gate_bstride : (long)channels * P_;
  };
  if (!spec) {
    if (pixels < 1) return B2NO_E_ARG;
    set_strides(pixels);
    const int N = 128;
    const long RPI = (pixels + N - 1) / N;
    return run_c2r(nullptr, y, nullptr, e, batch, channels, RPI, N, pixels, 0, 128, st);
  }
  if (!p) return B2NO_E_ARG;
  const int d = p->g.ndim;
  const int32_t* n = which == 0 ? p->g.nout : p->g.nin;
  const int Kl = p->K[d - 1];
  const float* tab = which == 0 ? p->t_out : p->t_in;
  const int npad = which == 0 ? p->npad_out : p->npad_in;
  const long bc = (long)batch * channels;
  long P = 1;
  for (int j = 0; j < d; j++) P *= n[j];
  if (pixels > 0 && pixels != P) return B2NO_E_ARG;
  set_strides(P);
  if (d == 1) return run_c2r((const float2*)spec, y, tab, e, batch, channels, 1, n[0], P, Kl, npad, st);
  if (!work) return B2NO_E_ARG;
  float2* A = (float2*)work;
  if (d == 2) {
    const float2* T = which == 0 ? p->m_inv[0] : p->m_adjfwd[0];
    int rc = run_cmat((const float2*)spec, A, T, bc, p->K[0], n[0], Kl, st);
    if (rc) return rc;
    return run_c2r(A, y, tab, e, batch, channels, n[0], n[1], P, Kl, npad, st);
  }
  float2* Bb = A + (size_t)bc * n[0] * n[1] * Kl;
  const float2* T0 = which == 0 ? p->m_inv[0] : p->m_adjfwd[0];
  int rc = run_cmat((const float2*)spec, Bb, T0, bc, p->K[0], n[0], p->K[1] * Kl, st);
  if (rc) return rc;
  if (epi && e.pw_ci > 0 && b2no_tc_available() && P % 128 == 0) {
    float* img = work + 2 * ((size_t)bc * n[0] * n[1] * Kl + (size_t)bc * n[0] * p->K[1] * Kl) + (size_t)bc * P;
    const int rc3 = b2no_tc_pointwise(p, which, (const float*)Bb, y, img, batch, channels, P, epi, st);
    if (rc3 != 1) return rc3;
  }
  const float2* T1 = which == 0 ? p->m_inv[1] : p->m_adjfwd[1];
  rc = run_cmat(Bb, A, T1, bc * n[0], p->K[1], n[1], Kl, st);
  if (rc) return rc;
  if (epi && e.pw_ci > 0 && !e.add && b2no_tc_available() && P % 128 == 0) {
    float* T = (float*)(Bb + (size_t)bc * n[0] * p->K[1] * Kl);
    EpiDev e0;
    memset(&e0, 0, sizeof(e0));
    rc = run_c2r(A, T, tab, e0, batch, channels, (long)n[0] * n[1], n[2], P, Kl, npad, st);
    if (rc) return rc;
    b2no_epilogue epi2 = *epi;
    const float* ident = (!epi->pw2_w && channels <= 128) ? identity_matrix(channels, st) : nullptr;
    if (ident) {
      epi2.pw2_w = ident; epi2.pw2_x = T; epi2.pw2_ci = channels; epi2.pw2_transposed = 0;
    } else {
      epi2.add = T;
    }
    rc = b2no_tc_pointwise(nullptr, which, nullptr, y, nullptr, batch, channels, P, &epi2, st);
    if (rc == 1 && ident) {
      epi2 = *epi;
      epi2.add = T;
      rc = b2no_tc_pointwise(nullptr, which, nullptr, y, nullptr, batch, channels, P, &epi2, st);
    }
    if (rc != 1) return rc;
    EpiDev e2 = e;
    e2.add = T;
    return run_c2r(nullptr, y, nullptr, e2, batch, channels, (P + 127) / 128, 128, P, 0, 128, st);
  }
  return run_c2r(A, y, tab, e, batch, channels, (long)n[0] * n[1], n[2], P, Kl, npad, st);
}
```

pde_policylearning_b200/csrc/tc_pointwise.cu:

```cuda
#include <string.h>

#include "common.cuh"
#include "tc.cuh"

using namespace tc;

namespace {

constexpr int kParts = 2;
constexpr int kGroups = 2;
constexpr int kCW = 8;
constexpr int kEpiThreadsPw = 128 * kParts * kGroups;
constexpr int kGroupThreadsPw = 128 * kParts;
constexpr int kThreads = 192 + kEpiThreadsPw;

struct PwTc {
  int B, Co, Np, C1, C1p, C2, C2p, Ks, Qp, R, S;
  int NA;
  int Cz;
  int tiles_per_img;
  long tiles, tiles_per_cta, P;
  const float* w1; int w1_t;
  const float* w2; int w2_t;
  const float* ahi; const float* alo; const float* timg;
  const float* bias; const float* add; const float* mul; const float* dz;
  const float* gate_z; const float* gate_h;
  long mul_bs, gate_bs;
  float* preact; float* y;
  int act, dact;
  int npass;
  int zlen, q2, tz_npad;
  long RPI;
  const float* tz;
  int MW, NW, Cx, Cxp;
  float* wpart;
};

struct PwLayout {
  uint32_t w1h, w1l, w2h, w2l, bias, tzh, tzl, stages, stage_bytes, x2, xw, ah, al, dz, bars, total;
};

template <bool WG>
__host__ __device__ inline PwLayout pw_layout(const PwTc& p) {
  PwLayout L;
  const uint32_t wb1 = (uint32_t)p.Np * p.C1p * 4, wb2 = (uint32_t)p.Np * p.C2p * 4;
  const uint32_t xb1 = (uint32_t)p.C1p * (WG ? 1024 : 512), xb2 = (uint32_t)p.C2p * 512;
  const uint32_t xwb = WG ? (uint32_t)p.NW * 512 : 0u, ab = (uint32_t)p.Ks * p.Np * 4;
  uint32_t o = 0;
  L.w1h = o; o += wb1; L.w1l = o; o += wb1;
  L.w2h = o; o += wb2; L.w2l = o; o += wb2;
  L.bias = o; o += (uint32_t)p.Np * 4;
  L.tzh = o; o += (uint32_t)p.Qp * p.zlen * 4;
  L.tzl = o; o += (uint32_t)p.Qp * p.zlen * 4;
  o = (o + 1023u) & ~1023u;
  L.stages = o;
  L.x2 = xb1; L.xw = xb1 + xb2; L.ah = L.xw + xwb; L.al = L.ah + ab;
  L.dz = (L.al + ab + 127u) & ~127u;
  L.stage_bytes = (L.dz + (uint32_t)p.Cz * 512 + 1023u) & ~1023u;
  o += L.stage_bytes * p.S;
  L.bars = o;
  o += 8 * (2 * p.S + 8 + (WG ? 1 : 0)) + 16;
  L.total = o + 1024;
  return L;
}

__host__ __device__ inline uint32_t pw_tmem_cols_dx(const PwTc& p) {
  if (p.zlen) return 2u * p.Np + (uint32_t)p.NA * (2u * (p.C1p + p.C2p) + 2u * p.Ks);
  return 2u * p.Np + 2u * p.Ks + 2u * (uint32_t)p.NA * (p.C1p + p.C2p);
}
__host__ __device__ inline uint32_t pw_tmem_wcol(const PwTc& p) { return (pw_tmem_cols_dx(p) + 31u) & ~31u; }
template <bool WG>
__host__ __device__ inline uint32_t pw_tmem_cols(const PwTc& p) { return WG ? pw_tmem_wcol(p) + p.NW : pw_tmem_cols_dx(p); }

template <int MODE>
__device__ __forceinline__ float epi_value(float z, float mulv, float dzv, int act, int dact) {
  if (MODE == 1) return z;
  if (MODE == 2) return b2no_act(z, B2NO_ACT_GELU);
  if (MODE == 3) return z * dzv;
  float v = b2no_act(z, act) * mulv;
  if (dact) v *= b2no_act_grad(dzv, dact);
  return v;
}

template <int MODE, bool WG>
__global__ void __launch_bounds__(kThreads, 1)
k_pw_tc(const __grid_constant__ CUtensorMap tm1, const __grid_constant__ CUtensorMap tm2, const __grid_constant__ CUtensorMap tm3,
        const PwTc p) {
  extern __shared__ uint8_t smem_raw[];
  uint8_t* smem = (uint8_t*)(((uintptr_t)smem_raw + 1023) & ~(uintptr_t)1023);
  const PwLayout L = pw_layout<WG>(p);
  uint64_t* full = (uint64_t*)(smem + L.bars);
  uint64_t* empty = full + p.S;
  uint64_t* a_full = empty + p.S;
  uint64_t* a_empty = a_full + 2;
  uint64_t* acc_full = a_empty + 2;
  uint64_t* acc_empty = acc_full + 2;
  uint64_t* wdone = acc_empty + 2;
  uint32_t* tslot = (uint32_t*)(acc_empty + 2 + (WG ? 1 : 0));

  const int tid = threadIdx.x, warp = tid >> 5, lane = tid & 31;
  uint32_t ncols = 32;
  while (ncols < pw_tmem_cols<WG>(p)) ncols <<= 1;

  for (int i = tid; i < p.Np * p.C1p; i += kThreads) {
    const int n = i / p.C1p, k = i - n * p.C1p;
    float w = 0.f;
    if (n < p.Co && k < p.C1) w = p.w1_t ? p.w1[(size_t)k * p.Co + n] : p.w1[(size_t)n * p.C1 + k];
    const float hi = tf32_rna(w);
    *(float*)(smem + L.w1h + kmajor_off(n, k, p.C1p)) = hi;
    *(float*)(smem + L.w1l + kmajor_off(n, k, p.C1p)) = tf32_rna(w - hi);
  }
  for (int i = tid; i < p.Np * p.C2p; i += kThreads) {
    const int n = i / p.C2p, k = i - n * p.C2p;
    float w = 0.f;
    if (n < p.Co && k < p.C2) w = p.w2_t ? p.w2[(size_t)k * p.Co + n] : p.w2[(size_t)n * p.C2 + k];
    const float hi = tf32_rna(w);
    *(float*)(smem + L.w2h + kmajor_off(n, k, p.C2p)) = hi;
    *(float*)(smem + L.w2l + kmajor_off(n, k, p.C2p)) = tf32_rna(w - hi);
  }
  for (int i = tid; i < p.Np; i += kThreads) ((float*)(smem + L.bias))[i] = (p.bias && i < p.Co) ? p.bias[i] : 0.f;
  for (int i = tid; i < p.Qp * p.zlen; i += kThreads) {
    const int q = i / p.zlen, z = i - q * p.zlen;
    const float v = q < p.q2 ? p.tz[(size_t)q * p.tz_npad + z] : 0.f;
    const float hi = tf32_rna(v);
    ((float*)(smem + L.tzh))[i] = hi;
    ((float*)(smem + L.tzl))[i] = tf32_rna(v - hi);
  }
  if (WG) {
    for (uint32_t i = tid; i < (uint32_t)p.S * L.stage_bytes / 16u; i += kThreads)
      *(float4*)(smem + L.stages + i * 16u) = make_float4(0.f, 0.f, 0.f, 0.f);
    __syncthreads();
    const uint32_t ones = (uint32_t)(p.NW - 2 * p.Cxp) * 8u;
    for (uint32_t i = tid; i < (uint32_t)p.S * 4u * ones; i += kThreads) {
      const uint32_t s = i / (4u * ones), r = i - s * 4u * ones, j = r / ones;
      *(float4*)(smem + L.stages + s * L.stage_bytes + L.xw + j * (uint32_t)p.NW * 128u + (uint32_t)p.Cxp * 256u + (r - j * ones) * 16u) =
          make_float4(1.f, 1.f, 1.f, 1.f);
    }
  }
  if (tid == 0) {
    for (int s = 0; s < p.S; s++) { mbar_init(&full[s], 1); mbar_init(&empty[s], 1 + ((MODE == 3 && p.Cz) ? kGroupThreadsPw : 0)); }
    for (int a = 0; a < 2; a++) {
      mbar_init(&a_full[a], 128); mbar_init(&a_empty[a], 1);
      mbar_init(&acc_full[a], 1); mbar_init(&acc_empty[a], kGroupThreadsPw);
    }
    if (WG) mbar_init(wdone, 1);
    fence_barrier_init();
  }
  fence_proxy_async();
  if (warp == 1) tmem_alloc(tslot, ncols);
  if (warp == 0 && lane == 0) { tma_prefetch_desc(&tm1); if (p.C2p || WG) tma_prefetch_desc(&tm2); if (MODE == 3 && p.Cz) tma_prefetch_desc(&tm3); }
  tc_fence_before();
  __syncthreads();
  tc_fence_after();
  const uint32_t tbase = *tslot;
  const uint32_t t_hi = tbase + 2u * p.Np, t_lo = t_hi + p.Ks;
  const uint32_t x_width = 2u * (p.C1p + p.C2p);
  const uint32_t a_base = p.zlen ? tbase + 2u * p.Np : t_lo + p.Ks;
  const uint32_t a_width = p.zlen ? x_width + 2u * p.Ks : x_width;
  const uint32_t t_w = tbase + pw_tmem_wcol(p);

  const uint32_t xb1 = (uint32_t)p.C1p * 512, xb2 = (uint32_t)p.C2p * 512, ab = (uint32_t)p.Ks * p.Np * 4;
  const long t_first = (long)blockIdx.x * p.tiles_per_cta;
  const long t_end = t_first + p.tiles_per_cta < p.tiles ? t_first + p.tiles_per_cta : p.tiles;

  if (warp == 0) {
    if (lane == 0) {
      const uint32_t bytes = xb1 + xb2 + ab + ((MODE == 3) ? (uint32_t)p.Cz * 512 : 0u) + (WG ? (uint32_t)p.Cxp * 512 : 0u);
      int it = 0;
      for (long tile = t_first; tile < t_end; tile++, it++) {
        const int s = it % p.S;
        const uint32_t ph = (uint32_t)(it / p.S) & 1u;
        mbar_wait(&empty[s], ph ^ 1u);
        mbar_arrive_expect_tx(&full[s], bytes);
        uint8_t* st = smem + L.stages + (size_t)s * L.stage_bytes;
        const int b = (int)(tile / p.tiles_per_img);
        const int t_in_img = (int)(tile - (long)b * p.tiles_per_img);
        if (WG) {
          for (int j = 0; j < 4; j++) {
            tma_load_3d(st + (uint32_t)j * p.C1p * 256u, &tm1, &full[s], t_in_img * 128 + 32 * j, 0, b);
            tma_load_3d(st + L.xw + (uint32_t)j * p.NW * 128u, &tm2, &full[s], t_in_img * 128 + 32 * j, 0, b);
          }
        } else {
          tma_load_3d(st, &tm1, &full[s], t_in_img * 128, 0, b);
        }
        if (p.C2p) tma_load_3d(st + L.x2, &tm2, &full[s], t_in_img * 128, 0, b);
        if (MODE == 3 && p.Cz) tma_load_3d(st + L.dz, &tm3, &full[s], t_in_img * 128, 0, b);
        if (p.Ks) {
          const size_t off = p.zlen ? ((size_t)b * p.RPI + (size_t)(t_in_img * 128) / p.zlen) * p.Qp * p.Np
                                    : (size_t)tile * p.R * p.Qp * p.Np;
          bulk_load(st + L.ah, p.ahi + off, ab, &full[s]);
        }
      }
    }
  } else if (warp == 1) {
    {
      const uint32_t idesc = idesc_tf32(128, p.Np, 0, 0);
      const uint32_t sbase = smem_u32(smem);
      const uint64_t d_w1h = smem_desc(sbase + L.w1h, 128, (p.C1p / 4) * 128, LAYOUT_NONE);
      const uint64_t d_w1l = smem_desc(sbase + L.w1l, 128, (p.C1p / 4) * 128, LAYOUT_NONE);
      const uint64_t d_w2h = smem_desc(sbase + L.w2h, 128, (p.C2p / 4) * 128, LAYOUT_NONE);
      const uint64_t d_w2l = smem_desc(sbase + L.w2l, 128, (p.C2p / 4) * 128, LAYOUT_NONE);
      const uint32_t lbo_a = (uint32_t)(p.Np / 8) * 128;
      int it = 0;
      for (long tile = t_first; tile < t_end; tile++, it++) {
        const int s = it % p.S;
        const uint32_t ph = (uint32_t)(it / p.S) & 1u;
        const int a = it & 1;
        const uint32_t aph = (uint32_t)(it >> 1) & 1u;
        const int xi = p.NA == 2 ? a : 0;
        const uint32_t xph = p.NA == 2 ? aph : ((uint32_t)it & 1u);
        mbar_wait(&full[s], ph);
        mbar_wait(&a_full[xi], xph);
        mbar_wait(&acc_empty[a], aph ^ 1u);
        tc_fence_after();
        const uint32_t st = sbase + L.stages + (uint32_t)s * L.stage_bytes;
        const uint32_t d = tbase + (uint32_t)a * p.Np;
        const uint32_t xa = a_base + (uint32_t)xi * a_width;
        uint32_t acc = 0;
        if (elect_one()) {
          _Pragma("unroll") for (int pass = 0; pass < 3; pass++) {
            if (pass >= p.npass) break;
            const uint32_t ac = pass == 1 ? xa + p.C1p : xa;
            const uint64_t dw = pass == 2 ? d_w1l : d_w1h;
            for (int k = 0; k < p.C1p / 8; k++) {
              mma_tf32_ts(d, ac + 8 * k, dw + (uint64_t)(k * 16), idesc, acc);
              acc = 1;
            }
          }
          if (p.C2p) {
            const uint32_t x2 = xa + 2 * p.C1p;
            _Pragma("unroll") for (int pass = 0; pass < 3; pass++) {
            if (pass >= p.npass) break;
              const uint32_t ac = pass == 1 ? x2 + p.C2p : x2;
              const uint64_t dw = pass == 2 ? d_w2l : d_w2h;
              for (int k = 0; k < p.C2p / 8; k++) mma_tf32_ts(d, ac + 8 * k, dw + (uint64_t)(k * 16), idesc, 1);
            }
          }
          if (p.Ks) {
            const uint64_t d_ah = smem_desc(st + L.ah, lbo_a, 128, LAYOUT_NONE);
            const uint64_t d_al = smem_desc(st + L.al, lbo_a, 128, LAYOUT_NONE);
            _Pragma("unroll") for (int pass = 0; pass < 3; pass++) {
            if (pass >= p.npass) break;
              const uint32_t tcn = p.zlen ? (pass == 1 ? xa + x_width + p.Ks : xa + x_width) : (pass == 1 ? t_lo : t_hi);
              const uint64_t da = pass == 2 ? d_al : d_ah;
              for (int k = 0; k < p.Ks / 8; k++)
                mma_tf32_ts(d, tcn + 8 * k, da + (uint64_t)(k * (2 * lbo_a / 16)), idesc, 1);
            }
          }
        }
        if (elect_one()) {
          if (!WG) mma_commit(&empty[s]);
          mma_commit(&a_empty[xi]);
          mma_commit(&acc_full[a]);
        }
        __syncwarp();
        if (WG) {
          if (elect_one()) {
            const uint32_t idesc_w = idesc_tf32(p.MW, p.NW, 0, 0);
#pragma unroll 1
            for (int j = 0; j < 4; j++) {
              const uint64_t dg = smem_desc(st + (uint32_t)j * p.C1p * 256u, 16, 1024, LAYOUT_SW128);
              const uint64_t dxw = smem_desc(st + L.xw + (uint32_t)j * p.NW * 128u, 16, 1024, LAYOUT_SW128);
#pragma unroll
              for (int ks = 0; ks < 4; ks++)
                mma_tf32_ss(t_w, dg + (uint64_t)(ks * 2), dxw + (uint64_t)(ks * 2), idesc_w, (it > 0 || j > 0 || ks > 0) ? 1u : 0u);
            }
            mma_commit(&empty[s]);
          }
          __syncwarp();
        }
      }
      if (WG) {
        if (elect_one()) mma_commit(wdone);
        __syncwarp();
      }
    }
  } else if (warp < 6) {
    const int quad = warp & 3;
    const int m = quad * 32 + lane;
    const uint32_t lane_base = (uint32_t)(quad * 32) << 16;
    for (int c0 = 0; c0 < (p.zlen ? 0 : p.Ks); c0 += 8) {
      float hi[8], lo[8];
#pragma unroll
      for (int j = 0; j < 8; j++) {
        hi[j] = __ldg(p.timg + (size_t)m * p.Ks + c0 + j);
        lo[j] = __ldg(p.timg + (size_t)128 * p.Ks + (size_t)m * p.Ks + c0 + j);
      }
      tmem_st8(t_hi + lane_base + c0, hi);
      tmem_st8(t_lo + lane_base + c0, lo);
    }
    int it = 0;
    for (long tile = t_first; tile < t_end; tile++, it++) {
      const int s = it % p.S;
      const uint32_t ph = (uint32_t)(it / p.S) & 1u;
      const int a = p.NA == 2 ? (it & 1) : 0;
      const uint32_t aph = p.NA == 2 ? ((uint32_t)(it >> 1) & 1u) : ((uint32_t)it & 1u);
      mbar_wait(&full[s], ph);
      if (p.Ks) {
        const uint32_t ah = smem_u32(smem) + L.stages + (uint32_t)s * L.stage_bytes + L.ah;
        const uint32_t al = smem_u32(smem) + L.stages + (uint32_t)s * L.stage_bytes + L.al;
        for (int i = m * 4; i < p.Ks * p.Np; i += 512) {
          const float4 v = lds_v4(ah + (uint32_t)i * 4u);
          const float4 h = make_float4(tf32_rna(v.x), tf32_rna(v.y), tf32_rna(v.z), tf32_rna(v.w));
          sts_v4(ah + (uint32_t)i * 4u, h);
          sts_v4(al + (uint32_t)i * 4u, make_float4(tf32_rna(v.x - h.x), tf32_rna(v.y - h.y), tf32_rna(v.z - h.z), tf32_rna(v.w - h.w)));
        }
        fence_proxy_async();
      }
      mbar_wait(&a_empty[a], aph ^ 1u);
      tc_fence_after();
      const uint32_t sx = smem_u32(smem) + L.stages + (uint32_t)s * L.stage_bytes + (uint32_t)m * 4u;
      const uint32_t xa = a_base + (uint32_t)a * a_width + lane_base;
      if (WG) {
        const uint32_t stg = smem_u32(smem) + L.stages + (uint32_t)s * L.stage_bytes;
        const uint32_t gb = stg + (uint32_t)(m >> 5) * (uint32_t)p.C1p * 256u + (uint32_t)(m & 3) * 4u;
        const uint32_t sw = (uint32_t)(m >> 2) & 7u;
        const bool lo_rows = p.npass == 3;
        for (int c0 = 0; c0 < p.C1p; c0 += 8) {
          float hi[8], lo[8];
#pragma unroll
          for (int j = 0; j < 8; j++) hi[j] = lds_f32(gb + (uint32_t)(c0 + j) * 128u + ((sw ^ (uint32_t)j) << 4));
#pragma unroll
          for (int j = 0; j < 8; j++) lo[j] = tf32_lo(hi[j]);
          tmem_st8(xa + c0, hi);
          tmem_st8(xa + p.C1p + c0, lo);
          if (lo_rows) {
#pragma unroll
            for (int j = 0; j < 8; j++) sts_f32(gb + (uint32_t)(p.C1p + c0 + j) * 128u + ((sw ^ (uint32_t)j) << 4), lo[j]);
          }
        }
        if (lo_rows) {
          const uint32_t per_box = (uint32_t)p.Cxp * 8u;
          for (int j = 0; j < 4; j++) {
            const uint32_t xb = stg + L.xw + (uint32_t)j * (uint32_t)p.NW * 128u;
            for (uint32_t i = (uint32_t)m; i < per_box; i += 128u) {
              const float4 v = lds_v4(xb + i * 16u);
              sts_v4(xb + (uint32_t)p.Cxp * 128u + i * 16u, make_float4(tf32_lo(v.x), tf32_lo(v.y), tf32_lo(v.z), tf32_lo(v.w)));
            }
          }
        }
      } else {
        for (int c0 = 0; c0 < p.C1p; c0 += 8) {
          float hi[8], lo[8];
#pragma unroll
          for (int j = 0; j < 8; j++) hi[j] = lds_f32(sx + (uint32_t)(c0 + j) * 512u);
#pragma unroll
          for (int j = 0; j < 8; j++) lo[j] = tf32_lo(hi[j]);
          tmem_st8(xa + c0, hi);
          tmem_st8(xa + p.C1p + c0, lo);
        }
      }
      if (p.C2p) {
        const uint32_t sx2 = sx + L.x2;
        for (int c0 = 0; c0 < p.C2p; c0 += 8) {
          float hi[8], lo[8];
#pragma unroll
          for (int j = 0; j < 8; j++) hi[j] = lds_f32(sx2 + (uint32_t)(c0 + j) * 512u);
#pragma unroll
          for (int j = 0; j < 8; j++) lo[j] = tf32_lo(hi[j]);
          tmem_st8(xa + 2 * p.C1p + c0, hi);
          tmem_st8(xa + 2 * p.C1p + p.C2p + c0, lo);
        }
      }
      if (p.zlen) {
        const long tin = tile % p.tiles_per_img;
        const long pix = tin * 128 + m;
        const int r0 = (int)((tin * 128) / p.zlen);
        const int slot = (int)(pix / p.zlen) - r0, z = (int)(pix % p.zlen);
        const float* th = (const float*)(smem + L.tzh);
        const float* tl = (const float*)(smem + L.tzl);
        const uint32_t ta = xa + x_width;
        for (int c0 = 0; c0 < p.Ks; c0 += 8) {
          float hi[8], lo[8];
          const int sl = c0 / p.Qp, q0 = c0 - sl * p.Qp;
#pragma unroll
          for (int j = 0; j < 8; j++) {
            const bool on = sl == slot;
            hi[j] = on ? th[(q0 + j) * p.zlen + z] : 0.f;
            lo[j] = on ? tl[(q0 + j) * p.zlen + z] : 0.f;
          }
          tmem_st8(ta + c0, hi);
          tmem_st8(ta + p.Ks + c0, lo);
        }
      }
      tmem_st_wait();
      tc_fence_before();
      if (WG) fence_proxy_async();
      mbar_arrive(&a_full[a]);
    }
    if (WG) {
      mbar_wait(wdone, 0);
      tc_fence_after();
      const int r = p.MW == 64 ? quad * 16 + (lane & 15) : m;
      const int half = r >= p.C1p ? 1 : 0, o = r - half * p.C1p;
      const bool own = (p.MW != 64 || lane < 16) && o < p.C1;
      const bool any = t_end > t_first;
      float* pout = p.wpart + ((size_t)half * gridDim.x + blockIdx.x) * ((size_t)p.C1 * p.Cx + p.C1);
      const uint32_t tw = t_w + lane_base;
      for (int c0 = 0; c0 < p.Cxp; c0 += 8) {
        float v[8], u[8];
        tmem_ld8(tw + (uint32_t)c0, v);
        tmem_ld8(tw + (uint32_t)(p.Cxp + c0), u);
        tmem_ld_wait();
        if (own) {
#pragma unroll
          for (int j = 0; j < 8; j++)
            if (c0 + j < p.Cx) pout[(size_t)o * p.Cx + c0 + j] = any ? v[j] + u[j] : 0.f;
        }
      }
      float v[8];
      tmem_ld8(tw + 2u * (uint32_t)p.Cxp, v);
      tmem_ld_wait();
      if (own) pout[(size_t)p.C1 * p.Cx + o] = any ? v[0] : 0.f;
    }
  } else {
    const int sub = (warp - 6) >> 2, grp = sub & 1;
    const int part = sub >> 1;
    const int quad = warp & 3;
    const int t = quad * 32 + lane;
    const uint32_t lane_base = (uint32_t)(quad * 32) << 16;
    const uint32_t sbias = smem_u32(smem) + L.bias;
    const bool dz_ring = MODE == 3 && p.Cz > 0;
    const bool dz_single = p.Co <= kCW * kParts;
    int it = grp;
    for (long tile = t_first + grp; tile < t_end; tile += kGroups, it += kGroups) {
      const int a = it & 1;
      const uint32_t aph = (uint32_t)(it >> 1) & 1u;
      const int b = (int)(tile / p.tiles_per_img);
      const long px = (tile - (long)b * p.tiles_per_img) * 128 + t;
      const size_t base = (size_t)b * p.Co * p.P + px;
      const int s = it % p.S;
      const uint32_t sdz = smem_u32(smem) + L.stages + (uint32_t)s * L.stage_bytes + L.dz + (uint32_t)t * 4u;
      float dcur[kCW];
      if (dz_ring) {
        mbar_wait(&full[s], (uint32_t)(it / p.S) & 1u);
        if (dz_single) {
#pragma unroll
          for (int j = 0; j < kCW; j++) dcur[j] = (part * kCW + j < p.Cz) ? lds_f32(sdz + (uint32_t)(part * kCW + j) * 512u) : 0.f;
          mbar_arrive(&empty[s]);
        }
      }
      mbar_wait(&acc_full[a], aph);
      tc_fence_after();
      for (int c0 = part * kCW; c0 < p.Co; c0 += kCW * kParts) {
        float v[kCW];
        tmem_ld8(tbase + lane_base + (uint32_t)(a * p.Np + c0), v);
        if (MODE == 0) {
          float av[kCW], mv[kCW], dv[kCW], gzv[kCW], ghv[kCW];
#pragma unroll
          for (int j = 0; j < kCW; j++) {
            const bool ok = c0 + j < p.Co;
            const size_t idx = base + (size_t)(c0 + j) * p.P;
            const size_t inner = (size_t)(c0 + j) * p.P + px;
            av[j] = (p.add && ok) ? __ldg(p.add + idx) : 0.f;
            mv[j] = (p.mul && ok) ? __ldg(p.mul + (size_t)b * p.mul_bs + inner) : 1.f;
            dv[j] = (p.dz && ok) ? __ldg(p.dz + idx) : 0.f;
            gzv[j] = (p.gate_z && ok) ? __ldg(p.gate_z + (size_t)b * p.gate_bs + inner) : 1.f;
            ghv[j] = (p.gate_z && ok) ? __ldg(p.gate_h + idx) : 0.f;
          }
          tmem_ld_wait();
#pragma unroll
          for (int j = 0; j < kCW; j++) {
            if (c0 + j < p.Co) {
              const size_t idx = base + (size_t)(c0 + j) * p.P;
              const float z = v[j] + lds_f32(sbias + (uint32_t)(c0 + j) * 4u) + av[j];
              if (p.preact) p.preact[idx] = z;
              const float r = fmaf(1.0f - gzv[j], ghv[j], epi_value<0>(z, mv[j], dv[j], p.act, p.dact));
              p.y[idx] = r;
            }
          }
        } else {
          float dv[kCW];
          if (MODE == 3) {
            if (dz_ring && dz_single) {
#pragma unroll
              for (int j = 0; j < kCW; j++) dv[j] = dcur[j];
            } else if (dz_ring) {
#pragma unroll
              for (int j = 0; j < kCW; j++) dv[j] = (c0 + j < p.Cz) ? lds_f32(sdz + (uint32_t)(c0 + j) * 512u) : 0.f;
            } else {
#pragma unroll
              for (int j = 0; j < kCW; j++) dv[j] = (c0 + j < p.Co) ? __ldg(p.dz + base + (size_t)(c0 + j) * p.P) : 0.f;
            }
#pragma unroll
            for (int j = 0; j < kCW; j += 2) {
              const float2 gg = b2no_gelu2_grad(make_float2(dv[j], dv[j + 1]));
              dv[j] = gg.x; dv[j + 1] = gg.y;
            }
          }
          float bv[kCW];
#pragma unroll
          for (int j = 0; j < kCW; j += 4) *reinterpret_cast<float4*>(bv + j) = lds_v4_ro(sbias + (uint32_t)(c0 + j) * 4u);
          tmem_ld_wait();
#pragma unroll
          for (int j = 0; j < kCW; j++) v[j] += bv[j];
          float* yp = p.y + base + (size_t)c0 * p.P;
          if (MODE == 2) {
            if (p.preact) {
              float* zp = p.preact + base + (size_t)c0 * p.P;
#pragma unroll
              for (int j = 0; j < kCW; j++)
                if (c0 + j < p.Co) zp[(size_t)j * p.P] = v[j];
            }
#pragma unroll
            for (int j = 0; j < kCW; j += 2) {
              const float2 gg = b2no_gelu2(make_float2(v[j], v[j + 1]));
              v[j] = gg.x; v[j + 1] = gg.y;
            }
          } else if (MODE == 3) {
#pragma unroll
            for (int j = 0; j < kCW; j++) v[j] *= dv[j];
          }
#pragma unroll
          for (int j = 0; j < kCW; j++)
            if (c0 + j < p.Co) yp[(size_t)j * p.P] = v[j];
        }
      }
      tc_fence_before();
      mbar_arrive(&acc_empty[a]);
      if (dz_ring && !dz_single) mbar_arrive(&empty[s]);
    }
  }
  tc_fence_before();
  __syncthreads();
  if (warp == 1) tmem_dealloc(tbase, ncols);
}

constexpr int kInvHB = 32;
template <int KXM, bool PAIR>
__global__ void __launch_bounds__(256)
k_inv_h(const float2* __restrict__ spec, const float2* __restrict__ M, float* __restrict__ ahi, float* __restrict__ alo,
        int Co, int Np, int Kx, int H, int Ky, int Qp, int layout, int n0) {
  extern __shared__ float2 s_spec[];
  const int b = blockIdx.y, h0 = blockIdx.x * kInvHB;
  const int kk = Kx * Ky, stride = kk + 1;
  float2* s_m = s_spec + (size_t)Co * stride;
  const float2* sp = spec + (size_t)b * Co * kk;
  const int lane = threadIdx.x & 31, warp = threadIdx.x >> 5;
  if (layout == 0) {
    for (int o = warp; o < Co; o += 8)
      for (int r = lane; r < kk; r += 32) s_spec[o * stride + r] = __ldg(sp + (size_t)o * kk + r);
  } else if (layout == 2) {
    const int b3 = b / n0, x = b - b3 * n0;
    for (int o = warp; o < Co; o += 8) {
      const float2* so = spec + (((size_t)b3 * Co + o) * n0 + x) * kk;
      for (int r = lane; r < kk; r += 32) s_spec[o * stride + r] = __ldg(so + r);
    }
  } else {
    const size_t nb = gridDim.y;
    for (int idx = threadIdx.x; idx < Co * kk; idx += 256) {
      const int r = idx / Co, o = idx - r * Co;
      s_spec[o * stride + r] = __ldg(spec + ((size_t)r * nb + b) * Co + o);
    }
  }
  for (int i = threadIdx.x; i < Kx * kInvHB; i += 256) {
    const int kx = i / kInvHB, hl = i - kx * kInvHB;
    s_m[i] = (h0 + hl < H) ? __ldg(M + (size_t)kx * H + h0 + hl) : make_float2(0.f, 0.f);
  }
  __syncthreads();
  const int ng = Np >> 3, nq = Qp >> 2;
  const int rows = H - h0 < kInvHB ? H - h0 : kInvHB;
  if (PAIR) {
    const int per_row = nq * ng * 8;
    for (int e = threadIdx.x; e < per_row; e += 256) {
      const int o8 = e & 7;
      const int r = e >> 3;
      const int og = r % ng, kq = r / ng;
      const int ky0 = kq * 2, o = og * 8 + o8;
      const bool valid0 = o < Co && ky0 < Ky, valid1 = o < Co && ky0 + 1 < Ky;
      float2 v0[KXM], v1[KXM];
#pragma unroll
      for (int kx = 0; kx < KXM; kx++) {
        v0[kx] = (valid0 && kx < Kx) ? s_spec[o * stride + kx * Ky + ky0] : make_float2(0.f, 0.f);
        v1[kx] = (valid1 && kx < Kx) ? s_spec[o * stride + kx * Ky + ky0 + 1] : make_float2(0.f, 0.f);
      }
      const size_t off0 = ((size_t)b * H + h0) * Qp * Np + (size_t)kq * ng * 32 + og * 32 + o8 * 4;
      for (int hl = 0; hl < rows; hl++) {
        float2 a0 = make_float2(0.f, 0.f), b0 = a0, a1 = a0, b1 = a0;
#pragma unroll
        for (int kx = 0; kx < KXM; kx++) {
          if (kx < Kx) {
            const float2 m = s_m[kx * kInvHB + hl];
            const float2 mr = make_float2(m.x, m.x), mi = make_float2(m.y, m.y);
            a0 = __ffma2_rn(mr, v0[kx], a0);
            b0 = __ffma2_rn(mi, v0[kx], b0);
            a1 = __ffma2_rn(mr, v1[kx], a1);
            b1 = __ffma2_rn(mi, v1[kx], b1);
          }
        }
        const size_t off = off0 + (size_t)hl * Qp * Np;
        *reinterpret_cast<float4*>(ahi + off) = make_float4(a0.x - b0.y, a0.y + b0.x, a1.x - b1.y, a1.y + b1.x);
      }
    }
  } else {
    const int per_row = nq * ng * 16;
    for (int e = threadIdx.x; e < per_row; e += 256) {
      const int l0 = e & 1, o8 = (e >> 1) & 7;
      const int r = e >> 4;
      const int og = r % ng, kq = r / ng;
      const int ky = kq * 2 + l0, o = og * 8 + o8;
      const bool valid = o < Co && ky < Ky;
      float2 v[KXM];
#pragma unroll
      for (int kx = 0; kx < KXM; kx++)
        v[kx] = (valid && kx < Kx) ? s_spec[o * stride + kx * Ky + ky] : make_float2(0.f, 0.f);
      const size_t off0 = ((size_t)b * H + h0) * Qp * Np + (size_t)kq * ng * 32 + og * 32 + o8 * 4 + l0 * 2;
      for (int hl = 0; hl < rows; hl++) {
        float2 a0 = make_float2(0.f, 0.f), b0 = a0;
#pragma unroll
        for (int kx = 0; kx < KXM; kx++) {
          if (kx < Kx) {
            const float2 m = s_m[kx * kInvHB + hl];
            a0 = __ffma2_rn(make_float2(m.x, m.x), v[kx], a0);
            b0 = __ffma2_rn(make_float2(m.y, m.y), v[kx], b0);
          }
        }
        const size_t off = off0 + (size_t)hl * Qp * Np;
        *reinterpret_cast<float2*>(ahi + off) = make_float2(a0.x - b0.y, a0.y + b0.x);
      }
    }
  }
}

int g_tc_state = -1;
long g_tc_launches = 0;
int g_tc_npass = 3;

}

bool b2no_tc_available() {
  if (g_tc_state < 0) {
    int on = 1;
    int dev = 0, major = 0;
    if (cudaGetDevice(&dev) != cudaSuccess || cudaDeviceGetAttribute(&major, cudaDevAttrComputeCapabilityMajor, dev) != cudaSuccess ||
        major != 10)
      on = 0;
    if (on && !encode_fn()) on = 0;
    g_tc_state = on;
  }
  return g_tc_state == 1;
}

extern "C" int64_t b2no_tensor_core_launches(void) { return g_tc_launches; }
int b2no_tc_passes() { return g_tc_npass; }
extern "C" int b2no_set_precision(int mode) {
  g_tc_npass = mode == 1 ? 1 : 3;
  return g_tc_npass == 1 ? 1 : 0;
}
void b2no_tc_count_launch() { g_tc_launches++; }

extern "C" int b2no_set_tensor_core_mode(int on) {
  g_tc_state = -1;
  if (!on) { g_tc_state = 0; return 0; }
  return b2no_tc_available() ? 1 : 0;
}

int b2no_tc_pointwise(const b2no_plan* plan, int which, const float* spec, float* y, float* work, int batch, int channels,
                      long pixels, const b2no_epilogue* e, cudaStream_t st, const b2no_tc_wg* wg) {
  if (!b2no_tc_available()) return 1;
  if (!e || !e->pw_w || !e->pw_x || e->pw_ci < 1) return 1;
  if (pixels % 128 != 0 || channels > 256 || e->pw_ci > 128 || e->pw2_ci > 128) return 1;
  if (((uintptr_t)e->pw_x | (uintptr_t)y) & 15) return 1;
  const bool has2 = e->pw2_w && e->pw2_x && e->pw2_ci > 0;
  if (has2 && ((uintptr_t)e->pw2_x & 15)) return 1;
  PwTc p;
  memset(&p, 0, sizeof(p));
  p.B = batch; p.Co = channels; p.Np = b2no_round_up(channels, 16); p.P = pixels;
  p.C1 = e->pw_ci; p.C1p = b2no_round_up(e->pw_ci, 8);
  p.C2 = has2 ? e->pw2_ci : 0; p.C2p = has2 ? b2no_round_up(e->pw2_ci, 8) : 0;
  p.tiles_per_img = (int)(pixels / 128);
  p.tiles = (long)batch * p.tiles_per_img;
  p.w1 = e->pw_w; p.w1_t = e->pw_transposed; p.w2 = has2 ? e->pw2_w : nullptr; p.w2_t = e->pw2_transposed;
  p.bias = e->bias; p.add = e->add; p.mul = e->mul; p.dz = e->dact_z; p.preact = e->preact; p.y = y;
  p.act = e->act; p.dact = e->dact_z ? e->dact : 0;
  p.gate_z = (e->gate_z && e->gate_h) ? e->gate_z : nullptr; p.gate_h = p.gate_z ? e->gate_h : nullptr;
  p.mul_bs = e->mul_bstride ? (long)e->mul_bstride : (long)channels * pixels;
  p.gate_bs = e->gate_bstride ? (long)e->gate_bstride : (long)channels * pixels;
  const bool three_d = spec && plan && plan->g.ndim == 3;
  if (spec && !three_d) {
    if (!plan || plan->g.ndim != 2 || !work) return 1;
    const b2no_tc_tables& tt = plan->tc[which];
    if (!tt.timg) return 1;
    p.Ks = tt.Ks; p.Qp = tt.Qp; p.R = tt.R; p.timg = tt.timg;
    const int32_t* n = which == 0 ? plan->g.nout : plan->g.nin;
    if ((long)n[0] * n[1] != pixels) return B2NO_E_ARG;
    const size_t afl = (size_t)batch * n[0] * p.Qp * p.Np;
    p.ahi = work;
    p.alo = work + afl;
  }
  if (three_d) {
    if (!work) return 1;
    const int32_t* n = which == 0 ? plan->g.nout : plan->g.nin;
    if ((long)n[0] * n[1] * n[2] != pixels) return B2NO_E_ARG;
    p.zlen = n[2]; p.q2 = 2 * plan->K[2]; p.Qp = b2no_round_up(p.q2, 8);
    p.R = 127 / p.zlen + 2; p.Ks = p.R * p.Qp;
    p.RPI = (long)n[0] * n[1];
    p.tz = which == 0 ? plan->t_out : plan->t_in;
    p.tz_npad = which == 0 ? plan->npad_out : plan->npad_in;
    if (p.zlen < 8 || p.Ks > 192 || plan->K[1] > 32 || p.Qp > 64) return 1;
    p.ahi = work;
    p.alo = work;
  }
  if (wg) {
    if (!spec || three_d || has2 || p.C1p > 64 || wg->ci < 1 || wg->ci > 112 || ((uintptr_t)wg->x & 15)) return 1;
    p.Cx = wg->ci; p.Cxp = b2no_round_up(wg->ci, 8);
    p.MW = 2 * p.C1p <= 64 ? 64 : 128;
    p.NW = b2no_round_up(2 * p.Cxp + 1, p.MW == 64 ? 8 : 16);
    p.wpart = wg->partial;
  }
  p.NA = 2;
  auto tmem_cols = [&]() { return wg ? pw_tmem_cols<true>(p) : pw_tmem_cols<false>(p); };
  auto layout = [&]() { return wg ? pw_layout<true>(p) : pw_layout<false>(p); };
  if (tmem_cols() > 512) p.NA = 1;
  if (tmem_cols() > 512) return 1;
  const bool extras = p.add || p.mul || p.gate_z;
  int mode = 0;
  if (!extras && !p.dact && p.act == B2NO_ACT_NONE && !p.preact) mode = 1;
  else if (!extras && !p.dact && p.act == B2NO_ACT_GELU) mode = 2;
  else if (!extras && p.dact == B2NO_ACT_GELU && p.act == B2NO_ACT_NONE && !p.preact) mode = 3;
  if (wg && mode != 1) return 1;
  if (mode == 3 && (((uintptr_t)p.dz & 15) == 0) && channels <= kCW * kParts * kGroups) p.Cz = b2no_round_up(channels, 8);
  int dev = 0, max_smem = 0;
  B2NO_CHECK_CUDA(cudaGetDevice(&dev));
  B2NO_CHECK_CUDA(cudaDeviceGetAttribute(&max_smem, cudaDevAttrMaxSharedMemoryPerBlockOptin, dev));
  PwLayout L;
  for (p.S = 6; p.S >= 2; p.S--) {
    L = layout();
    if ((int)L.total <= max_smem) break;
  }
  if (p.S < 3 && p.Cz) {
    p.Cz = 0;
    for (p.S = 6; p.S >= 2; p.S--) {
      L = layout();
      if ((int)L.total <= max_smem) break;
    }
  }
  if (p.S < 2) return 1;

  CUtensorMap tm1, tm2, tm3;
  {
    uint64_t dims[3] = {(uint64_t)pixels, (uint64_t)p.C1, (uint64_t)batch};
    uint64_t str[3] = {4, (uint64_t)pixels * 4, (uint64_t)pixels * 4 * p.C1};
    uint32_t box[3] = {128, (uint32_t)p.C1p, 1};
    if (wg) box[0] = 32;
    if (make_tmap_f32(&tm1, e->pw_x, 3, dims, str, box, wg ? CU_TENSOR_MAP_SWIZZLE_128B : CU_TENSOR_MAP_SWIZZLE_NONE)) return 1;
    tm2 = tm1;
    if (wg) {
      uint64_t dimsw[3] = {(uint64_t)pixels, (uint64_t)p.Cx, (uint64_t)batch};
      uint64_t strw[3] = {4, (uint64_t)pixels * 4, (uint64_t)pixels * 4 * p.Cx};
      uint32_t boxw[3] = {32, (uint32_t)p.Cxp, 1};
      if (make_tmap_f32(&tm2, wg->x, 3, dimsw, strw, boxw, CU_TENSOR_MAP_SWIZZLE_128B)) return 1;
    }
    if (has2) {
      uint64_t dims2[3] = {(uint64_t)pixels, (uint64_t)p.C2, (uint64_t)batch};
      uint64_t str2[3] = {4, (uint64_t)pixels * 4, (uint64_t)pixels * 4 * p.C2};
      uint32_t box2[3] = {128, (uint32_t)p.C2p, 1};
      if (make_tmap_f32(&tm2, e->pw2_x, 3, dims2, str2, box2, CU_TENSOR_MAP_SWIZZLE_NONE)) return 1;
    }
    tm3 = tm1;
    if (p.Cz) {
      uint64_t dims3[3] = {(uint64_t)pixels, (uint64_t)channels, (uint64_t)batch};
      uint64_t str3[3] = {4, (uint64_t)pixels * 4, (uint64_t)pixels * 4 * channels};
      uint32_t box3[3] = {128, (uint32_t)p.Cz, 1};
      if (make_tmap_f32(&tm3, p.dz, 3, dims3, str3, box3, CU_TENSOR_MAP_SWIZZLE_NONE)) return 1;
    }
  }
  if (spec) {
    const int32_t* n = which == 0 ? plan->g.nout : plan->g.nin;
    const int jd = three_d ? 1 : 0;
    const float2* M = which == 0 ? plan->m_inv[jd] : plan->m_adjfwd[jd];
    const int ikx = plan->K[jd], iky = plan->K[jd + 1], ih = n[jd];
    const int ilayout = three_d ? 2 : plan->g.spec_layout, in0 = three_d ? n[0] : 1;
    const size_t smem = ((size_t)channels * (ikx * iky + 1) + (size_t)ikx * kInvHB) * sizeof(float2);
    if (smem > 200 * 1024) return 1;
    if ((long)batch * in0 > 65535) return 1;
    dim3 grid((unsigned)((ih + kInvHB - 1) / kInvHB), (unsigned)(batch * in0));
    if (three_d) {
      B2NO_CHECK_CUDA(cudaMemsetAsync(work + (size_t)batch * p.RPI * p.Qp * p.Np, 0, (size_t)(p.R + 1) * p.Qp * p.Np * sizeof(float), st));
    }
    const bool pair = (p.Qp / 4) * (p.Np / 8) * 8 >= 256;
#define INVH_LAUNCH1(KXM, PAIR)                                                                                         \
  do {                                                                                                                  \
    if (smem > 48 * 1024) B2NO_CHECK_CUDA(cudaFuncSetAttribute(k_inv_h<KXM, PAIR>, cudaFuncAttributeMaxDynamicSharedMemorySize, (int)smem)); \
    k_inv_h<KXM, PAIR><<<grid, 256, smem, st>>>((const float2*)spec, M, (float*)p.ahi, (float*)p.alo, channels, p.Np, ikx, ih, \
                                                iky, p.Qp, ilayout, in0);                                               \
  } while (0)
#define INVH_LAUNCH(KXM)                                                                                                \
  do {                                                                                                                  \
    if (pair) INVH_LAUNCH1(KXM, true); else INVH_LAUNCH1(KXM, false);                                                   \
  } while (0)
    const int kx = ikx;
    if (kx <= 8) INVH_LAUNCH(8);
    else if (kx <= 12) INVH_LAUNCH(12);
    else if (kx <= 16) INVH_LAUNCH(16);
    else if (kx <= 24) INVH_LAUNCH(24);
    else if (kx <= 32) INVH_LAUNCH(32);
    else return 1;
#undef INVH_LAUNCH1
#undef INVH_LAUNCH
    B2NO_LAUNCH_CHECK();
  }
  long grid = p.tiles < b2no_sm_count() ? p.tiles : b2no_sm_count();
  p.tiles_per_cta = (p.tiles + grid - 1) / grid;
  grid = (p.tiles + p.tiles_per_cta - 1) / p.tiles_per_cta;
  p.npass = b2no_tc_passes();
#define LAUNCH(M, W)                                                                                                  \
  do {                                                                                                                \
    B2NO_CHECK_CUDA(cudaFuncSetAttribute(k_pw_tc<M, W>, cudaFuncAttributeMaxDynamicSharedMemorySize, (int)L.total));  \
    k_pw_tc<M, W><<<(unsigned)grid, kThreads, L.total, st>>>(tm1, tm2, tm3, p);                                           \
  } while (0)
  if (wg) {
    LAUNCH(1, true);
    *wg->nblk = 2 * (int)grid;
  } else {
    switch (mode) {
      case 1: LAUNCH(1, false); break;
      case 2: LAUNCH(2, false); break;
      case 3: LAUNCH(3, false); break;
      default: LAUNCH(0, false); break;
    }
  }
#undef LAUNCH
  B2NO_LAUNCH_CHECK();
  g_tc_launches++;
  return 0;
}
```

pde_policylearning_b200/functional.py:

```python
from __future__ import annotations

import math
from typing import List, Optional, Sequence

import torch

from . import ops
from .ops import SpecGeom, get_plan


def _contig(t: torch.Tensor) -> torch.Tensor:
    return t if t.is_contiguous() else t.contiguous()


def _fused_wgrad_ok(g: torch.Tensor) -> bool:
    return g.is_cuda


def _geom_has_overlap(geom: SpecGeom) -> bool:
    g = geom.resolved()
    return any(2 * g.half[j] > g.nfft[j] for j in range(g.ndim - 1))


class SpectralBlockFn(torch.autograd.Function):

    @staticmethod
    def forward(ctx, x, bias, pw_w, geom: SpecGeom, act, *corners):
        ops._require_cuda(x)
        x = _contig(x.float())
        plan = get_plan(geom, x.device)
        B, ci = x.shape[:2]
        co = corners[0].shape[1]
        if corners[0].shape[0] != ci:
            raise ValueError(f"input has {ci} channels, weights expect {corners[0].shape[0]}")
        det = [c.detach() for c in corners]
        xh = ops.dft_forward(plan, 0, x)
        yh = ops.mix(plan, 0, xh, det, ci, co)
        need_z = act not in (None, "none") and any(ctx.needs_input_grad)
        grid = plan.geom.nout
        z = torch.empty((B, co) + tuple(grid), dtype=torch.float32, device=x.device) if need_z else None
        pw2d = None
        if pw_w is not None:
            if tuple(plan.geom.nout) != tuple(plan.geom.nin):
                raise NotImplementedError("fused 1x1 skip needs matching input/output grids")
            pw2d = _contig(pw_w.detach().reshape(pw_w.shape[0], -1).float())
        epi = ops.make_epilogue(bias=None if bias is None else _contig(bias.detach().reshape(-1).float()),
                                pw_w=pw2d, pw_x=x if pw2d is not None else None, preact=z, act=act)
        y = ops.dft_inverse(plan, 0, yh, epi)
        ctx.geom, ctx.act = geom, act
        ctx.has_bias, ctx.has_pw = bias is not None, pw_w is not None
        ctx.pw_shape = None if pw_w is None else tuple(pw_w.shape)
        ctx.bias_shape = None if bias is None else tuple(bias.shape)
        ctx.save_for_backward(x, xh, z, pw2d, *det)
        return y

    @staticmethod
    def backward(ctx, gy):
        x, xh, z, pw2d, *det = ctx.saved_tensors
        geom, act = ctx.geom, ctx.act
        plan = get_plan(geom, x.device)
        B, ci = x.shape[:2]
        co = det[0].shape[1]
        gy = _contig(gy.float())
        gz = ops.act_bwd(gy, z, act) if z is not None else gy
        need_x, need_b, need_pw = ctx.needs_input_grad[0], ctx.needs_input_grad[1], ctx.needs_input_grad[2]
        need_w = any(ctx.needs_input_grad[5:])
        gyh = ops.dft_forward(plan, 1, gz)
        dbias = dpw = dx = None
        dcorners: List[Optional[torch.Tensor]] = [None] * len(det)
        if need_w:
            dcorners = ops.mix_dw(plan, xh, gyh, det, needs_zero=_geom_has_overlap(geom))
        fused = None
        if need_x:
            gxh = ops.mix(plan, 1, gyh, det, ci, co)
            epi = ops.make_epilogue(pw_w=pw2d, pw_x=gz if pw2d is not None else None, pw_transposed=True)
            if need_pw and _fused_wgrad_ok(gz):
                fused = ops.dft_inverse_wgrad(plan, 1, gxh, epi, x, need_bias=need_b)
            dx = fused[0] if fused is not None else ops.dft_inverse(plan, 1, gxh, epi)
        if need_pw:
            dpw, db2 = fused[1:] if fused is not None else ops.pw_wgrad(gz, x, need_bias=need_b)
            dpw = dpw.reshape(ctx.pw_shape)
            if need_b:
                dbias = db2.reshape(ctx.bias_shape)
        elif need_b:
            dc = gyh.reshape(B, co, -1)[:, :, 0].real.sum(dim=0) / plan.s_i
            dbias = dc.reshape(ctx.bias_shape)
        return (dx, dbias, dpw, None, None) + tuple(dcorners)


def spectral_block(x, corners: Sequence[torch.Tensor], geom: SpecGeom, bias=None, pw_weight=None, act=None):
    return SpectralBlockFn.apply(x, bias, pw_weight, geom, act, *corners)


class FNOStackFn(torch.autograd.Function):

    @staticmethod
    def forward(ctx, x, geom: SpecGeom, acts, n_corners, bias_all, *params):
        ops._require_cuda(x)
        x = _contig(x.float())
        plan = get_plan(geom, x.device)
        per = 1 + n_corners
        L = len(params) // per
        need_grad = any(ctx.needs_input_grad)
        saved, meta = [], []
        cur = x
        b2d = _contig(bias_all.detach().reshape(L, -1).float())
        for l in range(L):
            pw_w = params[l * per]
            det = [c.detach() for c in params[l * per + 1:(l + 1) * per]]
            B, ci = cur.shape[:2]
            co = det[0].shape[1]
            xh = ops.dft_forward(plan, 0, cur)
            yh = ops.mix(plan, 0, xh, det, ci, co)
            act = acts[l]
            need_z = act not in (None, "none") and need_grad
            z = torch.empty((B, co) + tuple(plan.geom.nout), dtype=torch.float32, device=x.device) if need_z else None
            pw2d = _contig(pw_w.detach().reshape(pw_w.shape[0], -1).float())
            epi = ops.make_epilogue(bias=b2d[l], pw_w=pw2d, pw_x=cur, preact=z, act=act)
            y = ops.dft_inverse(plan, 0, yh, epi)
            saved += [cur, xh, z if z is not None else cur.new_empty(0), pw2d] + det
            meta.append((tuple(pw_w.shape), ci, co, need_z))
            cur = y
        ctx.geom, ctx.acts, ctx.n_corners, ctx.meta = geom, acts, n_corners, meta
        ctx.bias_shape = tuple(bias_all.shape)
        ctx.save_for_backward(*saved)
        return cur

    @staticmethod
    def backward(ctx, gy):
        geom, acts, nc, meta = ctx.geom, ctx.acts, ctx.n_corners, ctx.meta
        saved = ctx.saved_tensors
        per_s = 4 + nc
        L = len(meta)
        plan = get_plan(geom, gy.device)
        per = 1 + nc
        grads = [None] * (L * per)
        need_bias = ctx.needs_input_grad[4]
        dbias = gy.new_empty((L, meta[0][2])) if need_bias else None
        g = _contig(gy.float())
        if meta[L - 1][3]:
            g = ops.act_bwd(g, saved[(L - 1) * per_s + 2], acts[L - 1])
        for l in range(L - 1, -1, -1):
            x, xh, _, pw2d = saved[l * per_s: l * per_s + 4]
            det = list(saved[l * per_s + 4: (l + 1) * per_s])
            pw_shape, ci, co, _ = meta[l]
            need = ctx.needs_input_grad[5 + l * per: 5 + (l + 1) * per]
            gyh = ops.dft_forward(plan, 1, g)
            if any(need[1:]):
                dcs = ops.mix_dw(plan, xh, gyh, det, needs_zero=_geom_has_overlap(geom))
                for j in range(nc):
                    grads[l * per + 1 + j] = dcs[j]
            need_wgrad = need_bias or need[0]
            db_out = dbias[l] if need_bias else None
            fused = None
            if l > 0 or ctx.needs_input_grad[0]:
                gxh = ops.mix(plan, 1, gyh, det, ci, co)
                zprev = saved[(l - 1) * per_s + 2] if (l > 0 and meta[l - 1][3]) else None
                epi = ops.make_epilogue(pw_w=pw2d, pw_x=g, pw_transposed=True, dact_z=zprev,
                                        dact=acts[l - 1] if zprev is not None else None)
                if need_wgrad and _fused_wgrad_ok(g):
                    fused = ops.dft_inverse_wgrad(plan, 1, gxh, epi, x, need_bias=need_bias, db_out=db_out)
                if fused is None:
                    if need_wgrad:
                        dpw, _ = ops.pw_wgrad(g, x, need_bias=need_bias, db_out=db_out)
                        grads[l * per] = dpw.reshape(pw_shape)
                    g = ops.dft_inverse(plan, 1, gxh, epi)
                else:
                    g = fused[0]
                    grads[l * per] = fused[1].reshape(pw_shape)
            elif need_wgrad:
                dpw, _ = ops.pw_wgrad(g, x, need_bias=need_bias, db_out=db_out)
                grads[l * per] = dpw.reshape(pw_shape)
        return (g if ctx.needs_input_grad[0] else None, None, None, None,
                dbias.reshape(ctx.bias_shape) if need_bias else None) + tuple(grads)


def fno_stack(x, geom: SpecGeom, bias_all, layers, acts):
    flat = []
    for pw_w, corners in layers:
        flat += [pw_w] + list(corners)
    return FNOStackFn.apply(x, geom, tuple(acts), len(layers[0][1]), bias_all, *flat)


class PointwiseConvFn(torch.autograd.Function):

    @staticmethod
    def forward(ctx, x, weight, bias, act):
        ops._require_cuda(x)
        x = _contig(x.float())
        B, ci = x.shape[:2]
        grid = tuple(x.shape[2:])
        w2d = _contig(weight.detach().reshape(weight.shape[0], -1).float())
        co = w2d.shape[0]
        if w2d.shape[1] != ci:
            raise ValueError(f"input has {ci} channels, weight expects {w2d.shape[1]}")
        need_z = act not in (None, "none") and any(ctx.needs_input_grad)
        z = torch.empty((B, co) + grid, dtype=torch.float32, device=x.device) if need_z else None
        epi = ops.make_epilogue(bias=None if bias is None else _contig(bias.detach().float()), pw_w=w2d, pw_x=x,
                                preact=z, act=act)
        y = ops.pointwise(B, co, grid, x.device, epi)
        ctx.act = act
        ctx.w_shape = tuple(weight.shape)
        ctx.save_for_backward(x, z, w2d)
        return y

    @staticmethod
    def backward(ctx, gy):
        x, z, w2d = ctx.saved_tensors
        gy = _contig(gy.float())
        gz = ops.act_bwd(gy, z, ctx.act) if z is not None else gy
        dx = dw = db = None
        if ctx.needs_input_grad[0]:
            epi = ops.make_epilogue(pw_w=w2d, pw_x=gz, pw_transposed=True)
            dx = ops.pointwise(x.shape[0], x.shape[1], tuple(x.shape[2:]), x.device, epi)
        if ctx.needs_input_grad[1] or ctx.needs_input_grad[2]:
            dw, db = ops.pw_wgrad(gz, x, need_bias=ctx.needs_input_grad[2])
            dw = dw.reshape(ctx.w_shape)
        return dx, dw, db, None


def pointwise_conv(x, weight, bias=None, act=None):
    return PointwiseConvFn.apply(x, weight, bias, act)


class PointwiseConv2Fn(torch.autograd.Function):

    @staticmethod
    def forward(ctx, x, weight, bias, act, x2, weight2):
        ops._require_cuda(x, x2)
        x, x2 = _contig(x.float()), _contig(x2.float())
        B, ci = x.shape[:2]
        grid = tuple(x.shape[2:])
        if tuple(x2.shape[2:]) != grid or x2.shape[0] != B:
            raise ValueError("both operands must share batch and grid")
        w2d = _contig(weight.detach().reshape(weight.shape[0], -1).float())
        w2d2 = _contig(weight2.detach().reshape(weight2.shape[0], -1).float())
        co = w2d.shape[0]
        need_z = act not in (None, "none") and any(ctx.needs_input_grad)
        z = torch.empty((B, co) + grid, dtype=torch.float32, device=x.device) if need_z else None
        epi = ops.make_epilogue(bias=None if bias is None else _contig(bias.detach().float()), pw_w=w2d, pw_x=x,
                                pw2_w=w2d2, pw2_x=x2, preact=z, act=act)
        y = ops.pointwise(B, co, grid, x.device, epi)
        ctx.act = act
        ctx.w_shape, ctx.w2_shape = tuple(weight.shape), tuple(weight2.shape)
        ctx.save_for_backward(x, x2, z, w2d, w2d2)
        return y

    @staticmethod
    def backward(ctx, gy):
        x, x2, z, w2d, w2d2 = ctx.saved_tensors
        gy = _contig(gy.float())
        gz = ops.act_bwd(gy, z, ctx.act) if z is not None else gy
        dx = dw = db = dx2 = dw2 = None
        if ctx.needs_input_grad[0]:
            dx = ops.pointwise(x.shape[0], x.shape[1], tuple(x.shape[2:]), x.device,
                               ops.make_epilogue(pw_w=w2d, pw_x=gz, pw_transposed=True))
        if ctx.needs_input_grad[4]:
            dx2 = ops.pointwise(x2.shape[0], x2.shape[1], tuple(x2.shape[2:]), x2.device,
                                ops.make_epilogue(pw_w=w2d2, pw_x=gz, pw_transposed=True))
        if ctx.needs_input_grad[1] or ctx.needs_input_grad[2]:
            dw, db = ops.pw_wgrad(gz, x, need_bias=ctx.needs_input_grad[2])
            dw = dw.reshape(ctx.w_shape)
        if ctx.needs_input_grad[5]:
            dw2, _ = ops.pw_wgrad(gz, x2, need_bias=False)
            dw2 = dw2.reshape(ctx.w2_shape)
        return dx, dw, db, None, dx2, dw2


def pointwise_conv2(x, weight, bias, act, x2, weight2):
    return PointwiseConv2Fn.apply(x, weight, bias, act, x2, weight2)


class MlpHeadFn(torch.autograd.Function):

    @staticmethod
    def forward(ctx, x, w1, b1, w2, b2, act):
        ops._require_cuda(x)
        x = _contig(x.float())
        w1m = _contig(w1.detach().reshape(w1.shape[0], -1).float())
        w2v = _contig(w2.detach().reshape(-1).float())
        b1c = None if b1 is None else _contig(b1.detach().float())
        out = ops.mlp_head_fwd(x, w1m, b1c, w2v, None if b2 is None else _contig(b2.detach().float()), act)
        ctx.act = act
        ctx.shapes = (tuple(w1.shape), None if b1 is None else tuple(b1.shape), tuple(w2.shape),
                      None if b2 is None else tuple(b2.shape))
        ctx.save_for_backward(x, w1m, b1c, w2v)
        return out

    @staticmethod
    def backward(ctx, g):
        x, w1m, b1c, w2v = ctx.saved_tensors
        g = _contig(g.float())
        need_x, need_w1, need_b1, need_w2, need_b2 = ctx.needs_input_grad[:5]
        per_sample_b1 = b1c is not None and b1c.dim() == 2
        if (not per_sample_b1 and g.data_ptr() % 16 == 0
                and ops.mlp_head_bwd_fused_supported(x.shape[1], w1m.shape[0], math.prod(x.shape[2:]))):
            gx, dw1, db1, dw2, db2 = ops.mlp_head_bwd_fused(x, w1m, b1c, w2v, g, ctx.act)
            db2 = db2.reshape(ctx.shapes[3]) if need_b2 else None
            return (gx if need_x else None, dw1.reshape(ctx.shapes[0]) if need_w1 else None,
                    db1.reshape(ctx.shapes[1]) if (need_b1 and b1c is not None) else None,
                    dw2.reshape(ctx.shapes[2]) if need_w2 else None, db2, None)
        res = ops.mlp_head_bwd(x, w1m, b1c, w2v, g, ctx.act, want_gz=need_w1 or need_b1)
        if res is None:
            raise RuntimeError("mlp_head backward: shape lost its tensor-core kernel between forward and backward")
        gx, gz, dw2 = res
        dw1 = db1 = None
        if need_w1 or need_b1:
            per_sample = b1c is not None and b1c.dim() == 2
            dw1, db1 = ops.pw_wgrad(gz, x, need_bias=need_b1 and not per_sample)
            dw1 = dw1.reshape(ctx.shapes[0])
            if need_b1 and per_sample:
                db1 = gz.sum(dim=tuple(range(2, gz.dim())))
            if db1 is not None:
                db1 = db1.reshape(ctx.shapes[1])
        db2 = g.sum().reshape(ctx.shapes[3]) if need_b2 else None
        return (gx if need_x else None, dw1 if need_w1 else None, db1 if need_b1 else None,
                dw2.reshape(ctx.shapes[2]) if need_w2 else None, db2, None)


def mlp_head_fused_available(x, w1, w2, b1, needs_grad: bool) -> bool:
    if not x.is_cuda or w2.reshape(-1, w1.shape[0]).shape[0] != 1 or (b1 is not None and b1.dim() > 2):
        return False
    if needs_grad:
        return bool(ops.mlp_head_bwd_supported(x.shape[1], w1.shape[0], math.prod(x.shape[2:]))) and x.data_ptr() % 16 == 0
    return x.shape[1] in (8, 16, 32, 64)


def mlp_head(x, w1, b1, w2, b2, act="gelu"):
    ops._require_cuda(x, w1, b1, w2, b2)
    needs_grad = torch.is_grad_enabled() and any(
        t is not None and t.requires_grad for t in (x, w1, b1, w2, b2))
    if mlp_head_fused_available(x, w1, w2, b1, needs_grad):
        if needs_grad:
            return MlpHeadFn.apply(x, w1, b1, w2, b2, act)
        return ops.mlp_head_fwd(_contig(x.float()), _contig(w1.reshape(w1.shape[0], -1).float()),
                                None if b1 is None else _contig(b1.float()), _contig(w2.reshape(-1).float()),
                                None if b2 is None else _contig(b2.float()), act)
    if b1 is not None and b1.dim() == 2:
        raise ValueError("mlp_head: a per-sample bias needs the fused head kernel (mlp_head_fused_available); pass the "
                         "per-sample term as a 1-channel map through pointwise_conv2 instead")
    h = pointwise_conv(x, w1, b1, act)
    return pointwise_conv(h, w2, b2, None)


class RelL2Fn(torch.autograd.Function):

    @staticmethod
    def forward(ctx, x, y, size_average):
        ops._require_cuda(x, y)
        B = x.shape[0]
        xf, yf = _contig(x.float()).reshape(B, -1), _contig(y.float()).reshape(B, -1)
        sums = ops.rel_l2_sums(xf, yf)
        loss, coef = ops.rel_l2_finish(sums, bool(size_average))
        ctx.save_for_backward(xf, yf, coef, sums)
        ctx.x_shape, ctx.y_shape = tuple(x.shape), tuple(y.shape)
        return loss

    @staticmethod
    def backward(ctx, g):
        xf, yf, coef, sums = ctx.saved_tensors
        dx = ops.rel_l2_bwd_g(xf, yf, coef, _contig(g.float()))
        dy = None
        if ctx.needs_input_grad[1]:
            ratio = (g.float() * coef * sums[:, 0] / sums[:, 1]).reshape(-1, 1)
            dy = (-dx - ratio * yf).reshape(ctx.y_shape)
        return dx.reshape(ctx.x_shape), dy, None


def rel_l2_loss(x, y, size_average=True):
    return RelL2Fn.apply(x, y, size_average)


class RnoGateFn(torch.autograd.Function):

    @staticmethod
    def forward(ctx, z, z2, hhat, h):
        z, z2, hhat, h = (_contig(t.float()) for t in (z, z2, hhat, h))
        ctx.save_for_backward(z, z2, hhat, h)
        return ops.rno_gate_fwd(z, z2, hhat, h)

    @staticmethod
    def backward(ctx, g):
        z, z2, hhat, h = ctx.saved_tensors
        return tuple(ops.rno_gate_bwd(_contig(g.float()), z, z2, hhat, h))


def rno_gate(z, z2, hhat, h):
    return RnoGateFn.apply(z, z2, hhat, h)


_RNO_XCHUNK = 8192


class RnoLayerFn(torch.autograd.Function):

    @staticmethod
    def forward(ctx, x_tm, h0, geom: SpecGeom, return_sequences: bool, *params):
        ops._require_cuda(x_tm, h0)
        x_tm, h0 = _contig(x_tm.float()), _contig(h0.float())
        Tn, B, Cc, H, W = x_tm.shape
        plan, geom = _rno_plan(geom, x_tm.device, B, Cc)
        pk = _rno_pack(params, Cc)
        xf = x_tm.reshape(Tn * B, Cc, H, W)
        Gzz2 = torch.empty((Tn * B, 2 * Cc, H, W), dtype=torch.float32, device=xf.device)
        Gr = torch.empty((Tn * B, Cc, H, W), dtype=torch.float32, device=xf.device)
        Gh = torch.empty_like(Gr)
        chunk = max(1, _RNO_XCHUNK // B) * B
        Xh = []
        for s in range(0, Tn * B, chunk):
            e = min(Tn * B, s + chunk)
            xs = xf[s:e]
            xh = ops.dft_forward(plan, 0, xs)
            Xh.append(xh)
            for Wc, Pm, bias, co, G in ((pk["Wx_zz2"], pk["Px_zz2"], pk["bias_zz2"], 2 * Cc, Gzz2),
                                        (pk["Wx_r"], pk["Px_r"], pk["bias_r"], Cc, Gr),
                                        (pk["Wx_h"], pk["Px_h"], pk["bias_h"], Cc, Gh)):
                S = ops.mix(plan, 0, xh, Wc, Cc, co)
                ops.dft_inverse(plan, 0, S, ops.make_epilogue(bias=bias, pw_w=Pm, pw_x=xs), out=G[s:e])
        Gzz2, Gr, Gh = (G.reshape(Tn, B, -1, H, W) for G in (Gzz2, Gr, Gh))
        need_grad = any(ctx.needs_input_grad)
        hs = []
        saved = []
        h = h0
        for t in range(Tn):
            Hh = ops.dft_forward(plan, 0, h)
            S = ops.mix(plan, 0, Hh, pk["Wh_zz2"], Cc, 2 * Cc)
            zz2 = ops.dft_inverse(plan, 0, S, ops.make_epilogue(pw_w=pk["Ph_zz2"], pw_x=h, add=Gzz2[t], act="sigmoid"))
            S = ops.mix(plan, 0, Hh, pk["Wh_r"], Cc, Cc)
            ar = torch.empty_like(h) if need_grad else None
            rh = ops.dft_inverse(plan, 0, S, ops.make_epilogue(pw_w=pk["Ph_r"], pw_x=h, add=Gr[t], act="sigmoid", mul=h,
                                                                preact=ar))
            RHh = ops.dft_forward(plan, 0, rh)
            S = ops.mix(plan, 0, RHh, pk["W6"], Cc, Cc)
            ah = torch.empty_like(h) if need_grad else None
            hn = ops.dft_inverse(plan, 0, S, ops.make_epilogue(pw_w=pk["P6"], pw_x=rh, add=Gh[t], act="selu", preact=ah,
                                                                mul=zz2[:, Cc:], gate_z=zz2[:, :Cc], gate_h=h))
            if return_sequences:
                hs.append(hn)
            if need_grad:
                saved += [h, Hh, zz2, ar, rh, RHh, ah]
            h = hn
        ctx.geom, ctx.dims, ctx.return_sequences = geom, (Tn, B, Cc, H, W), return_sequences
        ctx.param_shapes = [tuple(p.shape) for p in params]
        ctx.n_chunks, ctx.chunk = len(Xh), chunk
        if need_grad:
            ctx.save_for_backward(xf, *Xh, *[p.detach() for p in params], *saved)
        return torch.stack(hs, dim=0) if return_sequences else h

    @staticmethod
    def backward(ctx, gout):
        Tn, B, Cc, H, W = ctx.dims
        geom = ctx.geom
        sv = ctx.saved_tensors
        nch = ctx.n_chunks
        xf, Xh = sv[0], sv[1:1 + nch]
        params = sv[1 + nch:37 + nch]
        steps = sv[37 + nch:]
        plan = get_plan(geom, xf.device)
        pk = _rno_pack(params, Cc)
        dev = xf.device
        gout = _contig(gout.float())
        gGzz2 = torch.empty((Tn, B, 2 * Cc, H, W), dtype=torch.float32, device=dev)
        gGr = torch.empty((Tn, B, Cc, H, W), dtype=torch.float32, device=dev)
        gGh = torch.empty_like(gGr)
        overlap = _geom_has_overlap(geom)
        zl = torch.zeros_like if overlap else torch.empty_like
        dWh_zz2 = [zl(w) for w in pk["Wh_zz2"]]
        dWh_r = [zl(w) for w in pk["Wh_r"]]
        dW6 = [zl(w) for w in pk["W6"]]
        dPh_zz2 = dPh_r = dP6 = None

        def acc_(a, d):
            return d if a is None else a.add_(d)

        g = gout[Tn - 1] if ctx.return_sequences else gout
        first = True
        for t in range(Tn - 1, -1, -1):
            h, Hh, zz2, ar, rh, RHh, ah = steps[7 * t: 7 * t + 7]
            if ctx.return_sequences and t < Tn - 1:
                g = g + gout[t]
            g_hdir = ops.rno_cell_bwd(_contig(g), h, zz2, ah, gGzz2[t], gGh[t])
            g_ah = gGh[t]
            gY = ops.dft_forward(plan, 1, g_ah)
            ops.mix_dw(plan, RHh, gY, pk["W6"], False, out=dW6, accumulate=not first)
            gRH = ops.mix(plan, 1, gY, pk["W6"], Cc, Cc)
            g_rh = ops.dft_inverse(plan, 1, gRH, ops.make_epilogue(pw_w=pk["P6"], pw_x=g_ah, pw_transposed=True))
            dP6 = acc_(dP6, ops.pw_wgrad(g_ah, rh, need_bias=False)[0])
            ops.rno_reset_bwd(g_rh, h, ar, gGr[t], g_hdir)
            g_azz2, g_ar = gGzz2[t], gGr[t]
            gYz = ops.dft_forward(plan, 1, g_azz2)
            gYr = ops.dft_forward(plan, 1, g_ar)
            ops.mix_dw(plan, Hh, gYz, pk["Wh_zz2"], False, out=dWh_zz2, accumulate=not first)
            ops.mix_dw(plan, Hh, gYr, pk["Wh_r"], False, out=dWh_r, accumulate=not first)
            gH = ops.mix(plan, 1, gYz, pk["Wh_zz2"], Cc, 2 * Cc)
            ops.mix(plan, 1, gYr, pk["Wh_r"], Cc, Cc, out=gH, accumulate=True)
            t1 = ops.pointwise(B, Cc, (H, W), dev, ops.make_epilogue(pw_w=pk["Ph_zz2"], pw_x=g_azz2, pw_transposed=True,
                                                                     add=g_hdir))
            g = ops.dft_inverse(plan, 1, gH, ops.make_epilogue(pw_w=pk["Ph_r"], pw_x=g_ar, pw_transposed=True, add=t1))
            dPh_zz2 = acc_(dPh_zz2, ops.pw_wgrad(g_azz2, h, need_bias=False)[0])
            dPh_r = acc_(dPh_r, ops.pw_wgrad(g_ar, h, need_bias=False)[0])
            first = False
        g_h0 = g if ctx.needs_input_grad[1] else None
        need_x = ctx.needs_input_grad[0]
        gx = torch.empty_like(xf) if need_x else None
        dWx = {k: [zl(w) for w in pk[k]] for k in ("Wx_zz2", "Wx_r", "Wx_h")}
        dPx, dbx = {}, {}
        groups = (("Wx_zz2", "Px_zz2", gGzz2.reshape(Tn * B, 2 * Cc, H, W), 2 * Cc),
                  ("Wx_r", "Px_r", gGr.reshape(Tn * B, Cc, H, W), Cc),
                  ("Wx_h", "Px_h", gGh.reshape(Tn * B, Cc, H, W), Cc))
        firstc = True
        for j, s in enumerate(range(0, Tn * B, ctx.chunk)):
            e = min(Tn * B, s + ctx.chunk)
            xs, xh = xf[s:e], Xh[j]
            gX = None
            for wk, pkey, G, co in groups:
                gs = G[s:e]
                gY = ops.dft_forward(plan, 1, gs)
                ops.mix_dw(plan, xh, gY, pk[wk], False, out=dWx[wk], accumulate=not firstc)
                dw, db = ops.pw_wgrad(gs, xs, need_bias=True)
                dPx[pkey] = acc_(dPx.get(pkey), dw)
                dbx[pkey] = acc_(dbx.get(pkey), db)
                if need_x:
                    if gX is None:
                        gX = ops.mix(plan, 1, gY, pk[wk], Cc, co)
                    else:
                        ops.mix(plan, 1, gY, pk[wk], Cc, co, out=gX, accumulate=True)
            if need_x:
                n = e - s
                t1 = ops.pointwise(n, Cc, (H, W), dev, ops.make_epilogue(pw_w=pk["Px_zz2"], pw_x=groups[0][2][s:e],
                                                                         pw_transposed=True))
                t2 = ops.pointwise(n, Cc, (H, W), dev, ops.make_epilogue(pw_w=pk["Px_h"], pw_x=groups[2][2][s:e],
                                                                         pw_transposed=True, add=t1))
                ops.dft_inverse(plan, 1, gX, ops.make_epilogue(pw_w=pk["Px_r"], pw_x=groups[1][2][s:e], pw_transposed=True,
                                                               add=t2), out=gx[s:e])
            firstc = False
        C = Cc
        sp = {1: (dWx["Wx_zz2"], 0), 7: (dWx["Wx_zz2"], 1), 3: (dWx["Wx_r"], None), 5: (dWx["Wx_h"], None),
              2: (dWh_zz2, 0), 8: (dWh_zz2, 1), 4: (dWh_r, None), 6: (dW6, None)}
        pw = {1: (dPx["Px_zz2"], 0), 7: (dPx["Px_zz2"], 1), 3: (dPx["Px_r"], None), 5: (dPx["Px_h"], None),
              2: (dPh_zz2, 0), 8: (dPh_zz2, 1), 4: (dPh_r, None), 6: (dP6, None)}
        db_zz2, db_r, db_h = dbx["Px_zz2"], dbx["Px_r"], dbx["Px_h"]
        cbg = {1: db_zz2[:C], 2: db_zz2[:C], 7: db_zz2[C:], 8: db_zz2[C:], 3: db_r, 4: db_r, 5: db_h, 6: db_h}
        grads = []
        for k in range(1, 9):
            gl, half = sp[k]
            for j in (0, 1):
                w = gl[j] if half is None else gl[j][:, half * C:(half + 1) * C]
                grads.append(w.reshape(ctx.param_shapes[4 * (k - 1) + j]))
            m, half = pw[k]
            m = m if half is None else m[half * C:(half + 1) * C]
            grads.append(m.reshape(ctx.param_shapes[4 * (k - 1) + 2]))
            grads.append(cbg[k].reshape(ctx.param_shapes[4 * (k - 1) + 3]))
        for v in (db_zz2[:C], db_r, db_h, db_zz2[C:]):
            grads.append(v.sum().reshape(()))
        gx_out = gx.reshape(Tn, B, Cc, H, W) if need_x else None
        return (gx_out, g_h0, None, None) + tuple(grads)


def _rno_plan(geom: SpecGeom, device, batch: int, channels: int):
    g1 = geom.with_layout(1)
    try:
        p1 = get_plan(g1, device)
        if p1.layout_supported(batch, channels):
            return p1, g1
    except (RuntimeError, NotImplementedError):
        pass
    g0 = geom.with_layout(0)
    return get_plan(g0, device), g0


def _rno_pack(params, C):
    P_ = [p.detach() for p in params]
    fw = lambda k, j: P_[4 * (k - 1) + j]
    cw = lambda k: P_[4 * (k - 1) + 2].reshape(C, C).float()
    cb = lambda k: P_[4 * (k - 1) + 3].float()
    b1, b2, b3, b4 = (P_[32 + i].float() for i in range(4))
    cat = torch.cat
    return {
        "Wx_zz2": [cat((fw(1, j), fw(7, j)), dim=1).contiguous() for j in (0, 1)],
        "Wx_r": [_contig(fw(3, j)) for j in (0, 1)], "Wx_h": [_contig(fw(5, j)) for j in (0, 1)],
        "Wh_zz2": [cat((fw(2, j), fw(8, j)), dim=1).contiguous() for j in (0, 1)],
        "Wh_r": [_contig(fw(4, j)) for j in (0, 1)], "W6": [_contig(fw(6, j)) for j in (0, 1)],
        "Px_zz2": cat((cw(1), cw(7)), dim=0).contiguous(), "Px_r": _contig(cw(3)), "Px_h": _contig(cw(5)),
        "Ph_zz2": cat((cw(2), cw(8)), dim=0).contiguous(), "Ph_r": _contig(cw(4)), "P6": _contig(cw(6)),
        "bias_zz2": cat((cb(1) + cb(2) + b1, cb(7) + cb(8) + b4)).contiguous(),
        "bias_r": (cb(3) + cb(4) + b2).contiguous(), "bias_h": (cb(5) + cb(6) + b3).contiguous(),
    }


def rno_layer_supported(x, C, H, W) -> bool:
    return x.is_cuda and H == W and (C * H * W) % 4 == 0


def rno_layer(x_tm, h0, geom: SpecGeom, return_sequences, params):
    return RnoLayerFn.apply(x_tm, h0, geom, bool(return_sequences), *params)
```

pde_policylearning_b200/ops.py:

```python
from __future__ import annotations

import ctypes as C
import math
from dataclasses import dataclass
from typing import List, Optional, Sequence, Tuple

import torch

from . import _lib
from ._lib import ACT, NORM, Epilogue, Geom, Weights, check


_REPLAYED = [0]


def launch_count() -> int:
    return int(_lib.lib().b2no_kernel_launches()) + _REPLAYED[0]


def set_tensor_core_mode(on: bool) -> bool:
    return bool(_lib.lib().b2no_set_tensor_core_mode(1 if on else 0))


def set_precision(mode: str) -> str:
    modes = {"fp32": 0, "3xtf32": 0, "tf32": 1, "fast": 1}
    if mode not in modes:
        raise ValueError(f"precision mode {mode!r}: expected 'fp32' or 'tf32'")
    return "tf32" if _lib.lib().b2no_set_precision(modes[mode]) == 1 else "fp32"


def tensor_core_launches() -> int:
    return int(_lib.lib().b2no_tensor_core_launches())


def _require_cuda(*tensors):
    for t in tensors:
        if t is None:
            continue
        if not t.is_cuda:
            raise RuntimeError(
                "pde_policylearning_b200: the spectral-conv hot path runs only on CUDA (sm_100a); "
                f"got a tensor on {t.device}.  There is no CPU fallback.")
        if t.device.index != torch.cuda.current_device():
            raise RuntimeError(f"pde_policylearning_b200: tensor on {t.device} but the current CUDA device is "
                               f"cuda:{torch.cuda.current_device()}; call torch.cuda.set_device first")


def _ptr(t: Optional[torch.Tensor]):
    return None if t is None else C.c_void_p(t.data_ptr())


def _stream():
    return C.c_void_p(torch.cuda.current_stream().cuda_stream)


@dataclass(frozen=True)
class SpecGeom:
    nin: Tuple[int, ...]
    half: Tuple[int, ...]
    norm: str = "backward"
    nfft: Optional[Tuple[int, ...]] = None
    nout: Optional[Tuple[int, ...]] = None
    layout: int = 0

    def resolved(self) -> "SpecGeom":
        nfft = tuple(self.nin) if self.nfft is None else tuple(self.nfft)
        nout = nfft if self.nout is None else tuple(self.nout)
        return SpecGeom(tuple(self.nin), tuple(self.half), self.norm, nfft, nout, int(self.layout))

    def with_layout(self, layout: int) -> "SpecGeom":
        return SpecGeom(self.nin, self.half, self.norm, self.nfft, self.nout, int(layout))

    @property
    def ndim(self):
        return len(self.nin)

    def scales(self):
        g = self.resolved()
        n, npr = math.prod(g.nfft), math.prod(g.nout)
        if g.norm == "forward":
            return 1.0 / n, 1.0
        if g.norm == "backward":
            return 1.0, 1.0 / npr
        if g.norm == "ortho":
            return 1.0 / math.sqrt(n), 1.0 / math.sqrt(npr)
        raise ValueError(f"unknown fft norm {g.norm!r}")


class Plan:
    def __init__(self, geom: SpecGeom, device: torch.device):
        g = geom.resolved()
        if not 1 <= g.ndim <= _lib.MAX_DIM:
            raise NotImplementedError(f"spectral conv supports 1-3 spatial dims, got {g.ndim}")
        if g.norm not in NORM:
            raise ValueError(f"unknown fft norm {g.norm!r}")
        for j in range(g.ndim - 1):
            if g.half[j] > g.nfft[j]:
                raise ValueError("kept modes exceed the grid size")
        cg = Geom()
        cg.ndim = g.ndim
        for j in range(g.ndim):
            cg.nin[j], cg.nfft[j], cg.nout[j], cg.half[j] = g.nin[j], g.nfft[j], g.nout[j], g.half[j]
        cg.norm = NORM[g.norm]
        cg.spec_layout = int(g.layout)
        handle = C.c_void_p()
        with torch.cuda.device(device):
            check(_lib.lib().b2no_plan_create(C.byref(cg), C.byref(handle)), "plan_create")
        self.handle = handle
        self.geom = g
        self.device = device
        kept = (C.c_int32 * _lib.MAX_DIM)()
        check(_lib.lib().b2no_plan_kept(handle, C.byref(kept)), "plan_kept")
        self.kept = tuple(int(kept[j]) for j in range(g.ndim))
        self.modes = math.prod(self.kept)
        self.s_f, self.s_i = g.scales()
        self.layout = int(g.layout)

    def spec_shape(self, batch: int, channels: int):
        return (self.kept + (batch, channels)) if self.layout else ((batch, channels) + self.kept)

    def spec_bc(self, spec: torch.Tensor):
        if self.layout:
            if tuple(spec.shape[:-2]) != self.kept:
                raise ValueError(f"expected kept modes {self.kept} (mode-major), got {tuple(spec.shape)}")
            return int(spec.shape[-2]), int(spec.shape[-1])
        if tuple(spec.shape[2:]) != self.kept:
            raise ValueError(f"expected kept modes {self.kept}, got {tuple(spec.shape[2:])}")
        return int(spec.shape[0]), int(spec.shape[1])

    def layout_supported(self, batch: int, channels: int) -> bool:
        return bool(_lib.lib().b2no_plan_layout_supported(self.handle, batch, channels))

    def workspace(self, batch: int, channels: int) -> Optional[torch.Tensor]:
        n = int(_lib.lib().b2no_plan_workspace_floats(self.handle, batch, channels))
        if n < 0:
            check(n, "workspace")
        if n == 0:
            return None
        return torch.empty(n, dtype=torch.float32, device=self.device)

    def __del__(self):
        try:
            if self.handle:
                _lib.lib().b2no_plan_destroy(self.handle)
        except Exception:
            pass


_plans = {}


def get_plan(geom: SpecGeom, device: torch.device) -> Plan:
    key = (geom.resolved(), device.index if device.index is not None else torch.cuda.current_device())
    p = _plans.get(key)
    if p is None:
        p = Plan(geom, torch.device("cuda", key[1]))
        _plans[key] = p
    return p


def weights_struct(corners: Sequence[torch.Tensor], ndim: int) -> Weights:
    w = Weights()
    t0 = corners[0]
    for i, t in enumerate(corners):
        _require_cuda(t)
        if t.is_complex():
            if t.dtype != torch.complex64:
                raise TypeError("spectral weights must be complex64")
            strides = t.stride()
        else:
            if t.dtype != torch.float32 or t.shape[-1] != 2 or t.stride(-1) != 1:
                raise TypeError("real-pair spectral weights must be float32 (..., 2) with unit last stride")
            if any(s % 2 for s in t.stride()[:-1]):
                raise TypeError("real-pair weight strides must be even")
            strides = tuple(s // 2 for s in t.stride()[:-1])
        if i == 0:
            s0 = strides
        elif tuple(strides) != tuple(s0) or t.shape != t0.shape:
            raise ValueError("all corner weights must share shape and strides")
        w.corner[i] = t.data_ptr()
    w.stride_i, w.stride_o = s0[0], s0[1]
    for j in range(ndim):
        w.stride_k[j] = s0[2 + j]
    return w


def dft_forward(plan: Plan, which: int, x: torch.Tensor, out: Optional[torch.Tensor] = None) -> torch.Tensor:
    _require_cuda(x)
    assert x.dtype == torch.float32 and x.is_contiguous()
    B, Cc = x.shape[:2]
    grid = plan.geom.nin if which == 0 else plan.geom.nout
    if tuple(x.shape[2:]) != tuple(grid):
        raise ValueError(f"expected grid {tuple(grid)}, got {tuple(x.shape[2:])}")
    if out is None:
        spec = torch.empty(plan.spec_shape(B, Cc), dtype=torch.complex64, device=x.device)
    else:
        spec = out
        assert spec.dtype == torch.complex64 and spec.is_contiguous() and tuple(spec.shape) == plan.spec_shape(B, Cc)
    work = plan.workspace(B, Cc)
    check(_lib.lib().b2no_dft_forward(plan.handle, which, _ptr(x), _ptr(spec), _ptr(work), B * Cc, _stream()),
          "dft_forward")
    return spec


def make_epilogue(bias=None, pw_w=None, pw_x=None, pw_transposed=False, pw2_w=None, pw2_x=None,
                  pw2_transposed=False, add=None, mul=None, preact=None, act=None, dact_z=None, dact=None,
                  gate_z=None, gate_h=None) -> Epilogue:
    e = Epilogue()
    keep = []
    for name, t in (("bias", bias), ("pw_w", pw_w), ("pw_x", pw_x), ("pw2_w", pw2_w), ("pw2_x", pw2_x),
                    ("add", add), ("mul", mul), ("preact", preact), ("dact_z", dact_z), ("gate_z", gate_z),
                    ("gate_h", gate_h)):
        if t is not None:
            _require_cuda(t)
            assert t.dtype == torch.float32, name
            if name in ("mul", "gate_z") and not t.is_contiguous():
                assert t.dim() >= 2 and t[0].is_contiguous(), name
                setattr(e, name + "_bstride" if name == "mul" else "gate_bstride", t.stride(0))
            else:
                assert t.is_contiguous(), name
            setattr(e, name, t.data_ptr())
            keep.append(t)
    if (gate_z is None) != (gate_h is None):
        raise ValueError("gate_z and gate_h go together")
    if pw_w is not None:
        e.pw_ci = pw_x.shape[1]
        e.pw_transposed = 1 if pw_transposed else 0
    if pw2_w is not None:
        e.pw2_ci = pw2_x.shape[1]
        e.pw2_transposed = 1 if pw2_transposed else 0
    e.act = ACT[act]
    e.dact = ACT[dact] if dact_z is not None else 0
    e._keep = keep
    return e


def dft_inverse(plan: Plan, which: int, spec: torch.Tensor, epi: Optional[Epilogue] = None,
                out: Optional[torch.Tensor] = None) -> torch.Tensor:
    _require_cuda(spec)
    assert spec.dtype == torch.complex64 and spec.is_contiguous()
    B, Cc = plan.spec_bc(spec)
    grid = plan.geom.nout if which == 0 else plan.geom.nin
    y = out if out is not None else torch.empty((B, Cc) + tuple(grid), dtype=torch.float32, device=spec.device)
    work = plan.workspace(B, Cc)
    check(_lib.lib().b2no_dft_inverse(plan.handle, which, _ptr(spec), _ptr(y), _ptr(work), B, Cc,
                                      math.prod(grid), C.byref(epi) if epi is not None else None, _stream()),
          "dft_inverse")
    return y


def pointwise(batch: int, channels: int, grid: Tuple[int, ...], device, epi: Epilogue) -> torch.Tensor:
    y = torch.empty((batch, channels) + tuple(grid), dtype=torch.float32, device=device)
    check(_lib.lib().b2no_dft_inverse(None, 0, None, _ptr(y), None, batch, channels, math.prod(grid),
                                      C.byref(epi), _stream()), "pointwise")
    return y


def mix(plan: Plan, mode: int, spec: torch.Tensor, corners: Sequence[torch.Tensor], ci: int, co: int,
        out: Optional[torch.Tensor] = None, accumulate: bool = False) -> torch.Tensor:
    _require_cuda(spec)
    assert spec.dtype == torch.complex64 and spec.is_contiguous()
    B, cspec = plan.spec_bc(spec)
    cin, cout = (ci, co) if mode == 0 else (co, ci)
    assert cspec == cin, (spec.shape, cin)
    if out is None:
        out = torch.empty(plan.spec_shape(B, cout), dtype=torch.complex64, device=spec.device)
        accumulate = False
    w = weights_struct(corners, plan.geom.ndim)
    check(_lib.lib().b2no_mix(plan.handle, mode, _ptr(spec), C.byref(w), _ptr(out), B, ci, co,
                              1 if accumulate else 0, _stream()), "mix")
    return out


def mix_dw(plan: Plan, xh: torch.Tensor, gyh: torch.Tensor, like: Sequence[torch.Tensor], needs_zero: bool,
           out: Optional[Sequence[torch.Tensor]] = None, accumulate: bool = False):
    B, ci = plan.spec_bc(xh)
    co = plan.spec_bc(gyh)[1]
    if out is None:
        alloc = torch.zeros_like if needs_zero else torch.empty_like
        grads = [alloc(t, memory_format=torch.contiguous_format) for t in like]
        accumulate = False
    else:
        grads = list(out)
    w = weights_struct(grads, plan.geom.ndim)
    check(_lib.lib().b2no_mix_dw(plan.handle, _ptr(xh), _ptr(gyh), C.byref(w), B, ci, co, 1 if accumulate else 0,
                                 _stream()), "mix_dw")
    return grads


def act_bwd(gy: torch.Tensor, z: torch.Tensor, act) -> torch.Tensor:
    gz = torch.empty_like(gy)
    check(_lib.lib().b2no_act_bwd(_ptr(gy), _ptr(z), _ptr(gz), gy.numel(), ACT[act], _stream()), "act_bwd")
    return gz


def pw_wgrad(g: torch.Tensor, x: torch.Tensor, need_bias: bool, db_out: Optional[torch.Tensor] = None):
    B, co = g.shape[:2]
    ci = x.shape[1]
    P = math.prod(g.shape[2:])
    L = _lib.lib()
    n = int(L.b2no_pw_wgrad_scratch_floats(ci, co))
    partial = torch.empty(n, dtype=torch.float32, device=g.device)
    dw = torch.empty((co, ci), dtype=torch.float32, device=g.device)
    db = None
    if need_bias:
        db = db_out if db_out is not None else torch.empty((co,), dtype=torch.float32, device=g.device)
        assert db.is_contiguous() and db.numel() == co and db.dtype == torch.float32
    check(L.b2no_pw_wgrad(_ptr(g), _ptr(x), _ptr(dw), _ptr(db), _ptr(partial), B, ci, co, P, _stream()), "pw_wgrad")
    return dw, db


def dft_inverse_wgrad(plan: Plan, which: int, spec: torch.Tensor, epi: Epilogue, x: torch.Tensor, need_bias: bool,
                      db_out: Optional[torch.Tensor] = None):
    _require_cuda(spec, x)
    assert spec.dtype == torch.complex64 and spec.is_contiguous()
    assert x.dtype == torch.float32 and x.is_contiguous()
    B, Cc = plan.spec_bc(spec)
    grid = plan.geom.nout if which == 0 else plan.geom.nin
    if tuple(x.shape) != (B, x.shape[1]) + tuple(grid):
        raise ValueError(f"x {tuple(x.shape)} does not match batch {B} and grid {tuple(grid)}")
    co, ci = int(epi.pw_ci), int(x.shape[1])
    L = _lib.lib()
    y = torch.empty((B, Cc) + tuple(grid), dtype=torch.float32, device=spec.device)
    work = plan.workspace(B, Cc)
    partial = torch.empty(int(L.b2no_pw_wgrad_scratch_floats(ci, co)), dtype=torch.float32, device=spec.device)
    dw = torch.empty((co, ci), dtype=torch.float32, device=spec.device)
    db = None
    if need_bias:
        db = db_out if db_out is not None else torch.empty((co,), dtype=torch.float32, device=spec.device)
        assert db.is_contiguous() and db.numel() == co and db.dtype == torch.float32
    rc = L.b2no_dft_inverse_wgrad(plan.handle, which, _ptr(spec), _ptr(y), _ptr(work), B, Cc, math.prod(grid), C.byref(epi),
                                  _ptr(x), ci, _ptr(dw), _ptr(db), _ptr(partial), _stream())
    if rc == -2:
        return None
    check(rc, "dft_inverse_wgrad")
    return y, dw, db


def mlp_head_fwd(x, w1, b1, w2, b2, act="gelu") -> torch.Tensor:
    B, ci = x.shape[:2]
    grid = tuple(x.shape[2:])
    hidden = w1.shape[0]
    per_sample = b1 is not None and b1.dim() == 2
    out = torch.empty((B, 1) + grid, dtype=torch.float32, device=x.device)
    check(_lib.lib().b2no_mlp_head_fwd(_ptr(x), _ptr(w1), _ptr(b1), _ptr(w2), _ptr(b2), _ptr(out), B, ci, hidden,
                                       math.prod(grid), 1 if per_sample else 0, ACT[act], _stream()), "mlp_head_fwd")
    return out


def mlp_head_bwd_supported(ci: int, hidden: int, pixels: int) -> bool:
    return bool(_lib.lib().b2no_mlp_head_bwd_supported(ci, hidden, pixels))


def mlp_head_bwd(x, w1, b1, w2, g, act="gelu", want_gz=True, dact_z=None, dact=None):
    B, ci = x.shape[:2]
    grid = tuple(x.shape[2:])
    hidden = w1.shape[0]
    P = math.prod(grid)
    L = _lib.lib()
    per_sample = b1 is not None and b1.dim() == 2
    gx = torch.empty_like(x)
    gz = torch.empty((B, hidden) + grid, dtype=torch.float32, device=x.device) if want_gz else None
    dw2 = torch.empty((hidden,), dtype=torch.float32, device=x.device)
    partial = torch.empty(int(L.b2no_mlp_head_bwd_scratch_floats(hidden)), dtype=torch.float32, device=x.device)
    rc = L.b2no_mlp_head_bwd(_ptr(x), _ptr(w1), _ptr(b1), _ptr(w2), _ptr(g), _ptr(gx), _ptr(gz), _ptr(dw2), _ptr(partial),
                             B, ci, hidden, P, 1 if per_sample else 0, ACT[act], _ptr(dact_z),
                             ACT[dact] if dact_z is not None else 0, _stream())
    if rc == -2:
        return None
    check(rc, "mlp_head_bwd")
    return gx, gz, dw2


def mlp_head_bwd_fused_supported(ci: int, hidden: int, pixels: int) -> bool:
    return bool(_lib.lib().b2no_mlp_head_bwd_fused_supported(ci, hidden, pixels))


def mlp_head_bwd_fused(x, w1, b1, w2, g, act="gelu", dact_z=None, dact=None):
    B, ci = x.shape[:2]
    hidden = w1.shape[0]
    P = math.prod(x.shape[2:])
    L = _lib.lib()
    assert b1 is None or b1.dim() == 1
    gx = torch.empty_like(x)
    grads = torch.empty((hidden * ci + 2 * hidden + 1,), dtype=torch.float32, device=x.device)
    partial = torch.empty(int(L.b2no_mlp_head_bwd_fused_scratch_floats(ci, hidden)), dtype=torch.float32, device=x.device)
    check(L.b2no_mlp_head_bwd_fused(_ptr(x), _ptr(w1), _ptr(b1), _ptr(w2), _ptr(g), _ptr(gx), _ptr(grads), _ptr(partial),
                                    B, ci, hidden, P, ACT[act], _ptr(dact_z), ACT[dact] if dact_z is not None else 0,
                                    _stream()), "mlp_head_bwd_fused")
    n = hidden * ci
    return gx, grads[:n].view(hidden, ci), grads[n:n + hidden], grads[n + hidden:n + 2 * hidden], grads[n + 2 * hidden:]


def rno_gate_fwd(z, z2, hh, h):
    out = torch.empty_like(h)
    check(_lib.lib().b2no_rno_gate_fwd(_ptr(z), _ptr(z2), _ptr(hh), _ptr(h), _ptr(out), h.numel(), _stream()), "gate")
    return out


def rno_gate_bwd(g, z, z2, hh, h):
    outs = [torch.empty_like(h) for _ in range(4)]
    check(_lib.lib().b2no_rno_gate_bwd(_ptr(g), _ptr(z), _ptr(z2), _ptr(hh), _ptr(h), *[_ptr(o) for o in outs],
                                       h.numel(), _stream()), "gate_bwd")
    return outs


def rno_cell_bwd(g, h, zz2, ah, g_zz2, g_ah):
    B, Cc = h.shape[:2]
    P = math.prod(h.shape[2:])
    g_h = torch.empty_like(h)
    for t in (g, h, zz2, ah, g_zz2, g_ah):
        assert t.is_contiguous() and t.dtype == torch.float32
    check(_lib.lib().b2no_rno_cell_bwd(_ptr(g), _ptr(h), _ptr(zz2), _ptr(ah), _ptr(g_zz2), _ptr(g_ah), _ptr(g_h), B, Cc, P,
                                       _stream()), "rno_cell_bwd")
    return g_h


def rno_reset_bwd(g_rh, h, ar, g_ar, g_h):
    for t in (g_rh, h, ar, g_ar, g_h):
        assert t.is_contiguous() and t.dtype == torch.float32
    check(_lib.lib().b2no_rno_reset_bwd(_ptr(g_rh), _ptr(h), _ptr(ar), _ptr(g_ar), _ptr(g_h), h.numel(), _stream()),
          "rno_reset_bwd")


def rel_l2_sums(x, y):
    B = x.shape[0]
    n = x.numel() // B
    sums = torch.empty((B, 2), dtype=torch.float32, device=x.device)
    check(_lib.lib().b2no_rel_l2_sums(_ptr(x), _ptr(y), _ptr(sums), B, n, _stream()), "rel_l2_sums")
    return sums


def rel_l2_bwd(x, y, coef):
    B = x.shape[0]
    dx = torch.empty_like(x)
    check(_lib.lib().b2no_rel_l2_bwd(_ptr(x), _ptr(y), _ptr(coef), _ptr(dx), B, x.numel() // B, _stream()), "rel_l2_bwd")
    return dx


def rel_l2_finish(sums, size_average: bool):
    B = sums.shape[0]
    loss = torch.empty((), dtype=torch.float32, device=sums.device)
    coef = torch.empty((B,), dtype=torch.float32, device=sums.device)
    check(_lib.lib().b2no_rel_l2_finish(_ptr(sums), _ptr(loss), _ptr(coef), B, 1 if size_average else 0, _stream()),
          "rel_l2_finish")
    return loss, coef


def rel_l2_bwd_g(x, y, coef, g):
    B = x.shape[0]
    dx = torch.empty_like(x)
    check(_lib.lib().b2no_rel_l2_bwd_g(_ptr(x), _ptr(y), _ptr(coef), _ptr(g), _ptr(dx), B, x.numel() // B, _stream()),
          "rel_l2_bwd_g")
    return dx


def gather_segments(flat, ptr_table, offsets, counts, nseg: int):
    check(_lib.lib().b2no_gather_segments(_ptr(flat), _ptr(ptr_table), _ptr(offsets), _ptr(counts), nseg, _stream()),
          "gather_segments")



def pino_residual_supported(n: int) -> bool:
    return 8 <= n <= 64 and n % 4 == 0


def pino_residual_fwd(w, u0, forcing2d, nu, t_interval: float):
    _require_cuda(w, u0, forcing2d, nu)
    B, N, _, T = w.shape
    for t in (w, u0, forcing2d, nu):
        assert t.dtype == torch.float32 and t.is_contiguous()
    dev = w.device
    du_p = torch.empty((B, T, N, N), dtype=torch.float32, device=dev)
    fields = torch.empty((4, B, T, N, N), dtype=torch.float32, device=dev)
    partial = torch.empty((B, T, 4), dtype=torch.float32, device=dev)
    loss2 = torch.empty((2,), dtype=torch.float32, device=dev)
    coef = torch.empty((B, 2), dtype=torch.float32, device=dev)
    check(_lib.lib().b2no_pino_residual_fwd(_ptr(w), _ptr(u0), _ptr(forcing2d), _ptr(nu), float(t_interval), _ptr(du_p),
                                            _ptr(fields), _ptr(partial), _ptr(loss2), _ptr(coef), B, N, T, _stream()),
          "pino_residual_fwd")
    return loss2, coef, du_p, fields


def pino_residual_bwd(w, u0, forcing2d, nu, t_interval: float, du_p, fields, coef, gup):
    B, N, _, T = w.shape
    assert gup.dtype == torch.float32 and gup.is_contiguous() and gup.numel() == 2
    dw = torch.empty_like(w)
    check(_lib.lib().b2no_pino_residual_bwd(_ptr(w), _ptr(u0), _ptr(forcing2d), _ptr(nu), float(t_interval), _ptr(du_p),
                                            _ptr(fields), _ptr(coef), _ptr(gup), _ptr(dw), B, N, T, _stream()),
          "pino_residual_bwd")
    return dw
```

Before: 30050.

## Fuse next layer's forward DFT into inverse-DFT pointwise epilogue kernel

The tensor-core pointwise/inverse-DFT kernel now also stages its output tile in shared memory and runs the W-direction forward DFT with extra tcgen05 MMAs into spare TMEM columns, writing partial spectra to a workspace. A small follow-up kernel does the H-direction reduction to produce the next layer's spectrum. The forward and backward FNO stack passes use this to skip a separate dft_forward pass over each intermediate activation. In exchange the kernel uses more shared memory, TMEM columns and barriers, and adds an extra launch plus a workspace round trip. It only applies for 2D grids with a width of 128 and at most 32 channels.

```diff
diff --git a/include/b2no.h b/include/b2no.h
--- a/include/b2no.h
+++ b/include/b2no.h
@@ -79,6 +79,9 @@
 int b2no_dft_inverse_wgrad(const b2no_plan* plan, int which, const float* spec, float* y, float* work, int batch, int channels,
                            int64_t pixels, const b2no_epilogue* epi, const float* wg_x, int wg_ci, float* dw, float* db,
                            float* partial, void* stream);
+int b2no_dft_inverse_fwd(const b2no_plan* plan, int which, const float* spec, float* y, float* work, int batch,
+                         int channels, int64_t pixels, const b2no_epilogue* epi, int fwd_which, float* fwd_spec,
+                         float* fwd_work, void* stream);
 int b2no_mlp_head_fwd(const float* x, const float* w1, const float* b1, const float* w2, const float* b2,
                       float* out, int batch, int ci, int hidden, int64_t pixels, int b1_per_sample,
                       int act, void* stream);
diff --git a/pde_policylearning_b200/_lib.py b/pde_policylearning_b200/_lib.py
--- a/pde_policylearning_b200/_lib.py
+++ b/pde_policylearning_b200/_lib.py
@@ -103,6 +103,7 @@
     L.b2no_pw_wgrad_scratch_floats.argtypes = [i32, i32]
     L.b2no_pw_wgrad.argtypes = [vp, vp, vp, vp, vp, i32, i32, i32, i64, vp]
     L.b2no_dft_inverse_wgrad.argtypes = [vp, i32, vp, vp, vp, i32, i32, i64, C.POINTER(Epilogue), vp, i32, vp, vp, vp, vp]
+    L.b2no_dft_inverse_fwd.argtypes = [vp, i32, vp, vp, vp, i32, i32, i64, C.POINTER(Epilogue), i32, vp, vp, vp]
     L.b2no_mlp_head_fwd.argtypes = [vp, vp, vp, vp, vp, vp, i32, i32, i32, i64, i32, i32, vp]
     L.b2no_mlp_head_bwd_supported.argtypes = [i32, i32, i64]
     L.b2no_mlp_head_bwd_scratch_floats.restype = i64
@@ -139,7 +140,7 @@
     "b2no_plan_create", "b2no_plan_destroy", "b2no_plan_kept", "b2no_plan_layout_supported", "b2no_plan_workspace_floats",
     "b2no_set_tensor_core_mode", "b2no_set_precision", "b2no_tensor_core_launches", "b2no_kernel_launches",
     "b2no_dft_forward", "b2no_dft_inverse", "b2no_mix", "b2no_mix_dw",
-    "b2no_act_bwd", "b2no_pw_wgrad_scratch_floats", "b2no_pw_wgrad", "b2no_dft_inverse_wgrad", "b2no_mlp_head_fwd", "b2no_mlp_head_bwd_scratch_floats", "b2no_mlp_head_bwd_supported", "b2no_mlp_head_bwd",
+    "b2no_act_bwd", "b2no_pw_wgrad_scratch_floats", "b2no_pw_wgrad", "b2no_dft_inverse_wgrad", "b2no_dft_inverse_fwd", "b2no_mlp_head_fwd", "b2no_mlp_head_bwd_scratch_floats", "b2no_mlp_head_bwd_supported", "b2no_mlp_head_bwd",
     "b2no_mlp_head_bwd_fused_scratch_floats", "b2no_mlp_head_bwd_fused_supported", "b2no_mlp_head_bwd_fused",
     "b2no_rno_gate_fwd", "b2no_rno_gate_bwd", "b2no_rno_cell_bwd", "b2no_rno_reset_bwd", "b2no_rel_l2_sums", "b2no_rel_l2_bwd",
     "b2no_rel_l2_finish", "b2no_rel_l2_bwd_g", "b2no_adam_step", "b2no_gather_segments",
diff --git a/pde_policylearning_b200/csrc/common.cuh b/pde_policylearning_b200/csrc/common.cuh
--- a/pde_policylearning_b200/csrc/common.cuh
+++ b/pde_policylearning_b200/csrc/common.cuh
@@ -33,8 +33,13 @@
   float* partial;
   int* nblk;
 };
+struct b2no_tc_fwd {
+  int which;
+  float* work;
+};
 int b2no_tc_pointwise(const b2no_plan* plan, int which, const float* spec, float* y, float* work, int batch, int channels,
-                      long pixels, const b2no_epilogue* e, cudaStream_t st, const b2no_tc_wg* wg = nullptr);
+                      long pixels, const b2no_epilogue* e, cudaStream_t st, const b2no_tc_wg* wg = nullptr,
+                      const b2no_tc_fwd* fwd = nullptr);
 
 struct b2no_tc_tables {
   float* timg;
diff --git a/pde_policylearning_b200/csrc/spectral.cu b/pde_policylearning_b200/csrc/spectral.cu
--- a/pde_policylearning_b200/csrc/spectral.cu
+++ b/pde_policylearning_b200/csrc/spectral.cu
@@ -430,6 +430,93 @@
   return run_cmat(Bb, (float2*)spec, T0, bc, n[0], p->K[0], p->K[1] * Kl, st);
 }
 
+constexpr int kFwdHCols = 32, kFwdHParts = 8;
+template <int KXM>
+__global__ void __launch_bounds__(kFwdHCols * kFwdHParts)
+k_fwd_h(const float2* __restrict__ part, float2* __restrict__ spec, const float2* __restrict__ M, int C, int H, int Kx, int Ky) {
+  extern __shared__ float2 s_fh[];
+  float2* s_red = s_fh + (size_t)H * Kx;
+  const int b = blockIdx.y, col = threadIdx.x & (kFwdHCols - 1), hp = threadIdx.x / kFwdHCols;
+  const int ncol = C * Ky, n = blockIdx.x * kFwdHCols + col;
+  for (int i = threadIdx.x; i < H * Kx; i += blockDim.x) s_fh[i] = __ldg(M + i);
+  __syncthreads();
+  float2 acc[KXM];
+#pragma unroll
+  for (int kx = 0; kx < KXM; kx++) acc[kx] = make_float2(0.f, 0.f);
+  if (n < ncol) {
+    const float2* src = part + (size_t)b * H * ncol + n;
+#pragma unroll 4
+    for (int h = hp; h < H; h += kFwdHParts) {
+      const float2 a = __ldg(src + (size_t)h * ncol);
+      const float2* m = s_fh + (size_t)h * Kx;
+#pragma unroll
+      for (int kx = 0; kx < KXM; kx++) {
+        if (kx < Kx) {
+          const float2 mv = m[kx];
+          acc[kx].x = fmaf(mv.x, a.x, fmaf(-mv.y, a.y, acc[kx].x));
+          acc[kx].y = fmaf(mv.x, a.y, fmaf(mv.y, a.x, acc[kx].y));
+        }
+      }
+    }
+  }
+  if (hp > 0) {
+#pragma unroll
+    for (int kx = 0; kx < KXM; kx++)
+      if (kx < Kx) s_red[((size_t)(hp - 1) * kFwdHCols + col) * Kx + kx] = acc[kx];
+  }
+  __syncthreads();
+  if (hp == 0 && n < ncol) {
+    const int c = n / Ky, ky = n - c * Ky;
+    float2* dst = spec + ((size_t)b * C + c) * Kx * Ky + ky;
+#pragma unroll
+    for (int kx = 0; kx < KXM; kx++) {
+      if (kx < Kx) {
+        float2 v = acc[kx];
+        for (int r = 0; r < kFwdHParts - 1; r++) {
+          const float2 u = s_red[((size_t)r * kFwdHCols + col) * Kx + kx];
+          v.x += u.x; v.y += u.y;
+        }
+        dst[(size_t)kx * Ky] = v;
+      }
+    }
+  }
+}
+
+extern "C" int b2no_dft_inverse_fwd(const b2no_plan* p, int which, const float* spec, float* y, float* work, int batch,
+                                    int channels, int64_t pixels, const b2no_epilogue* epi, int fwd_which, float* fwd_spec,
+                                    float* fwd_work, void* stream) {
+  if (!p || !spec || !y || !work || !epi || !fwd_spec || !fwd_work || batch < 1 || channels < 1 || (which != 0 && which != 1) ||
+      (fwd_which != 0 && fwd_which != 1))
+    return B2NO_E_ARG;
+  if (p->g.ndim != 2 || batch > 65535) return B2NO_E_UNSUPPORTED;
+  const int32_t* n = which == 0 ? p->g.nout : p->g.nin;
+  const long px = (long)n[0] * n[1];
+  if (pixels > 0 && pixels != px) return B2NO_E_ARG;
+  cudaStream_t st = (cudaStream_t)stream;
+  const b2no_tc_fwd f = {fwd_which, fwd_work};
+  const int rc = b2no_tc_pointwise(p, which, spec, y, work, batch, channels, px, epi, st, nullptr, &f);
+  if (rc == 1) return B2NO_E_UNSUPPORTED;
+  if (rc) return rc;
+  const b2no_tc_fwd_tables& tf = p->tcf[fwd_which];
+  const float2* M = fwd_which == 0 ? p->m_fwd[0] : p->m_adjinv[0];
+  const size_t smem = ((size_t)tf.H + (size_t)(kFwdHParts - 1) * kFwdHCols) * tf.Kx * sizeof(float2);
+  dim3 grid((unsigned)((channels * tf.Ky + kFwdHCols - 1) / kFwdHCols), (unsigned)batch);
+#define FWDH_LAUNCH(K)                                                                                                      \
+  do {                                                                                                                      \
+    if (smem > 48 * 1024) B2NO_CHECK_CUDA(cudaFuncSetAttribute(k_fwd_h<K>, cudaFuncAttributeMaxDynamicSharedMemorySize, (int)smem)); \
+    k_fwd_h<K><<<grid, kFwdHCols * kFwdHParts, smem, st>>>((const float2*)fwd_work, (float2*)fwd_spec, M, channels, tf.H,    \
+                                                           tf.Kx, tf.Ky);                                                  \
+  } while (0)
+  if (tf.Kx <= 8) FWDH_LAUNCH(8);
+  else if (tf.Kx <= 12) FWDH_LAUNCH(12);
+  else if (tf.Kx <= 16) FWDH_LAUNCH(16);
+  else if (tf.Kx <= 24) FWDH_LAUNCH(24);
+  else FWDH_LAUNCH(32);
+#undef FWDH_LAUNCH
+  B2NO_LAUNCH_CHECK();
+  return 0;
+}
+
 template <int BT, int PT, bool CONJT>
 __global__ void __launch_bounds__(128)
 k_mix(const float2* __restrict__ in, float2* __restrict__ out, b2no_weights w, ModeMap mm, int B, int Cq,
diff --git a/pde_policylearning_b200/csrc/tc_pointwise.cu b/pde_policylearning_b200/csrc/tc_pointwise.cu
--- a/pde_policylearning_b200/csrc/tc_pointwise.cu
+++ b/pde_policylearning_b200/csrc/tc_pointwise.cu
@@ -34,14 +34,22 @@
   const float* tz;
   int MW, NW, Cx, Cxp;
   float* wpart;
+  const float* ftb;
+  float* fwork;
+  int N1, Q2;
 };
 
 struct PwLayout {
-  uint32_t w1h, w1l, w2h, w2l, bias, tzh, tzl, stages, stage_bytes, x2, xw, ah, al, dz, bars, total;
+  uint32_t w1h, w1l, w2h, w2l, bias, tzh, tzl, ftb, fstg, stages, stage_bytes, x2, xw, ah, al, dz, bars, total;
 };
 
-template <bool WG>
+enum { kVarPlain = 0, kVarWg = 1, kVarFwd = 2 };
+constexpr uint32_t kFwdBox = 64 * 128;
+constexpr uint32_t kFwdStg = 4 * kFwdBox;
+
+template <int VAR>
 __host__ __device__ inline PwLayout pw_layout(const PwTc& p) {
+  constexpr bool WG = VAR == kVarWg, FWD = VAR == kVarFwd;
   PwLayout L;
   const uint32_t wb1 = (uint32_t)p.Np * p.C1p * 4, wb2 = (uint32_t)p.Np * p.C2p * 4;
   const uint32_t xb1 = (uint32_t)p.C1p * (WG ? 1024 : 512), xb2 = (uint32_t)p.C2p * 512;
@@ -52,14 +60,17 @@
   L.bias = o; o += (uint32_t)p.Np * 4;
   L.tzh = o; o += (uint32_t)p.Qp * p.zlen * 4;
   L.tzl = o; o += (uint32_t)p.Qp * p.zlen * 4;
+  o = (o + 127u) & ~127u;
+  L.ftb = o; o += FWD ? 2u * p.N1 * 128u * 4u : 0u;
   o = (o + 1023u) & ~1023u;
+  L.fstg = o; o += FWD ? (uint32_t)kGroups * kFwdStg : 0u;
   L.stages = o;
   L.x2 = xb1; L.xw = xb1 + xb2; L.ah = L.xw + xwb; L.al = L.ah + ab;
   L.dz = (L.al + ab + 127u) & ~127u;
   L.stage_bytes = (L.dz + (uint32_t)p.Cz * 512 + 1023u) & ~1023u;
   o += L.stage_bytes * p.S;
   L.bars = o;
-  o += 8 * (2 * p.S + 8 + (WG ? 1 : 0)) + 16;
+  o += 8 * (2 * p.S + 8 + (WG ? 1 : 0) + (FWD ? 8 : 0)) + 16;
   L.total = o + 1024;
   return L;
 }
@@ -69,8 +80,10 @@
   return 2u * p.Np + 2u * p.Ks + 2u * (uint32_t)p.NA * (p.C1p + p.C2p);
 }
 __host__ __device__ inline uint32_t pw_tmem_wcol(const PwTc& p) { return (pw_tmem_cols_dx(p) + 31u) & ~31u; }
-template <bool WG>
-__host__ __device__ inline uint32_t pw_tmem_cols(const PwTc& p) { return WG ? pw_tmem_wcol(p) + p.NW : pw_tmem_cols_dx(p); }
+template <int VAR>
+__host__ __device__ inline uint32_t pw_tmem_cols(const PwTc& p) {
+  return VAR == kVarWg ? pw_tmem_wcol(p) + p.NW : VAR == kVarFwd ? pw_tmem_wcol(p) + 4u * p.N1 : pw_tmem_cols_dx(p);
+}
 
 template <int MODE>
 __device__ __forceinline__ float epi_value(float z, float mulv, float dzv, int act, int dact) {
@@ -82,13 +95,14 @@
   return v;
 }
 
-template <int MODE, bool WG>
+template <int MODE, int VAR>
 __global__ void __launch_bounds__(kThreads, 1)
 k_pw_tc(const __grid_constant__ CUtensorMap tm1, const __grid_constant__ CUtensorMap tm2, const __grid_constant__ CUtensorMap tm3,
         const PwTc p) {
+  constexpr bool WG = VAR == kVarWg, FWD = VAR == kVarFwd;
   extern __shared__ uint8_t smem_raw[];
   uint8_t* smem = (uint8_t*)(((uintptr_t)smem_raw + 1023) & ~(uintptr_t)1023);
-  const PwLayout L = pw_layout<WG>(p);
+  const PwLayout L = pw_layout<VAR>(p);
   uint64_t* full = (uint64_t*)(smem + L.bars);
   uint64_t* empty = full + p.S;
   uint64_t* a_full = empty + p.S;
@@ -96,11 +110,15 @@
   uint64_t* acc_full = a_empty + 2;
   uint64_t* acc_empty = acc_full + 2;
   uint64_t* wdone = acc_empty + 2;
-  uint32_t* tslot = (uint32_t*)(acc_empty + 2 + (WG ? 1 : 0));
+  uint64_t* stg_full = wdone + (WG ? 1 : 0);
+  uint64_t* stg_empty = stg_full + 2;
+  uint64_t* fwd_full = stg_empty + 2;
+  uint64_t* fwd_empty = fwd_full + 2;
+  uint32_t* tslot = (uint32_t*)(acc_empty + 2 + (WG ? 1 : 0) + (FWD ? 8 : 0));
 
   const int tid = threadIdx.x, warp = tid >> 5, lane = tid & 31;
   uint32_t ncols = 32;
-  while (ncols < pw_tmem_cols<WG>(p)) ncols <<= 1;
+  while (ncols < pw_tmem_cols<VAR>(p)) ncols <<= 1;
 
   for (int i = tid; i < p.Np * p.C1p; i += kThreads) {
     const int n = i / p.C1p, k = i - n * p.C1p;
@@ -137,6 +155,12 @@
           make_float4(1.f, 1.f, 1.f, 1.f);
     }
   }
+  if (FWD) {
+    const float4* src = (const float4*)p.ftb;
+    for (int i = tid; i < 2 * p.N1 * 128 / 4; i += kThreads) *(float4*)(smem + L.ftb + (uint32_t)i * 16u) = __ldg(src + i);
+    for (uint32_t i = tid; i < (uint32_t)kGroups * kFwdStg / 16u; i += kThreads)
+      *(float4*)(smem + L.fstg + i * 16u) = make_float4(0.f, 0.f, 0.f, 0.f);
+  }
   if (tid == 0) {
     for (int s = 0; s < p.S; s++) { mbar_init(&full[s], 1); mbar_init(&empty[s], 1 + ((MODE == 3 && p.Cz) ? kGroupThreadsPw : 0)); }
     for (int a = 0; a < 2; a++) {
@@ -144,6 +168,12 @@
       mbar_init(&acc_full[a], 1); mbar_init(&acc_empty[a], kGroupThreadsPw);
     }
     if (WG) mbar_init(wdone, 1);
+    if (FWD) {
+      for (int g = 0; g < kGroups; g++) {
+        mbar_init(&stg_full[g], kGroupThreadsPw); mbar_init(&stg_empty[g], 1);
+        mbar_init(&fwd_full[g], 1); mbar_init(&fwd_empty[g], 128);
+      }
+    }
     fence_barrier_init();
   }
   fence_proxy_async();
@@ -201,6 +231,31 @@
       const uint64_t d_w2h = smem_desc(sbase + L.w2h, 128, (p.C2p / 4) * 128, LAYOUT_NONE);
       const uint64_t d_w2l = smem_desc(sbase + L.w2l, 128, (p.C2p / 4) * 128, LAYOUT_NONE);
       const uint32_t lbo_a = (uint32_t)(p.Np / 8) * 128;
+      auto fwd_mma = [&](int j) {
+        const int g = j & 1;
+        const uint32_t ph = (uint32_t)(j >> 1) & 1u;
+        mbar_wait(&stg_full[g], ph);
+        mbar_wait(&fwd_empty[g], ph ^ 1u);
+        tc_fence_after();
+        if (elect_one()) {
+          const uint32_t idesc_f = idesc_tf32(64, 2 * p.N1, 0, 0), idesc_l = idesc_tf32(64, p.N1, 0, 0);
+          const uint64_t dt = smem_desc(sbase + L.ftb, 128, 32 * 128, LAYOUT_NONE);
+          const uint32_t d = t_w + (uint32_t)(g * 2 * p.N1);
+#pragma unroll
+          for (int jb = 0; jb < 4; jb++) {
+            const uint64_t dy = smem_desc(sbase + L.fstg + (uint32_t)g * kFwdStg + (uint32_t)jb * kFwdBox, 16, 1024, LAYOUT_SW128);
+            const uint64_t dyl = dy + (uint64_t)(32 * 128 / 16);
+#pragma unroll
+            for (int ks = 0; ks < 4; ks++) {
+              mma_tf32_ss(d, dy + (uint64_t)(ks * 2), dt + (uint64_t)((jb * 4 + ks) * 16), idesc_f, (jb > 0 || ks > 0) ? 1u : 0u);
+              mma_tf32_ss(d, dyl + (uint64_t)(ks * 2), dt + (uint64_t)((jb * 4 + ks) * 16), idesc_l, 1u);
+            }
+          }
+          mma_commit(&stg_empty[g]);
+          mma_commit(&fwd_full[g]);
+        }
+        __syncwarp();
+      };
       int it = 0;
       for (long tile = t_first; tile < t_end; tile++, it++) {
         const int s = it % p.S;
@@ -269,7 +324,9 @@
           }
           __syncwarp();
         }
-      }
+        if (FWD && it > 0) fwd_mma(it - 1);
+      }
+      if (FWD && it > 0) fwd_mma(it - 1);
       if (WG) {
         if (elect_one()) mma_commit(wdone);
         __syncwarp();
@@ -289,6 +346,30 @@
       tmem_st8(t_hi + lane_base + c0, hi);
       tmem_st8(t_lo + lane_base + c0, lo);
     }
+    auto fwd_readout = [&](int j) {
+      const int g = j & 1;
+      mbar_wait(&fwd_full[g], (uint32_t)(j >> 1) & 1u);
+      tc_fence_after();
+      const long tile = t_first + j;
+      const int b = (int)(tile / p.tiles_per_img), h = (int)(tile - (long)b * p.tiles_per_img);
+      const int c = quad * 16 + (lane & 15);
+      const bool own = lane < 16 && c < p.Co;
+      float* dst = p.fwork + (((size_t)b * p.tiles_per_img + h) * p.Co + c) * p.Q2;
+      const uint32_t tf = t_w + lane_base + (uint32_t)(g * 2 * p.N1);
+      for (int c0 = 0; c0 < (quad < 2 ? p.N1 : 0); c0 += 8) {
+        float v[8], u[8];
+        tmem_ld8(tf + (uint32_t)c0, v);
+        tmem_ld8(tf + (uint32_t)(p.N1 + c0), u);
+        tmem_ld_wait();
+        if (own) {
+#pragma unroll
+          for (int q = 0; q < 8; q += 2)
+            if (c0 + q < p.Q2) *(float2*)(dst + c0 + q) = make_float2(v[q] + u[q], v[q + 1] + u[q + 1]);
+        }
+      }
+      tc_fence_before();
+      mbar_arrive(&fwd_empty[g]);
+    };
     int it = 0;
     for (long tile = t_first; tile < t_end; tile++, it++) {
       const int s = it % p.S;
@@ -387,6 +468,10 @@
       tc_fence_before();
       if (WG) fence_proxy_async();
       mbar_arrive(&a_full[a]);
+      if (FWD && it >= 3) fwd_readout(it - 3);
+    }
+    if (FWD) {
+      for (int j = it > 3 ? it - 3 : 0; j < it; j++) fwd_readout(j);
     }
     if (WG) {
       mbar_wait(wdone, 0);
@@ -422,12 +507,16 @@
     const uint32_t sbias = smem_u32(smem) + L.bias;
     const bool dz_ring = MODE == 3 && p.Cz > 0;
     const bool dz_single = p.Co <= kCW * kParts;
+    const uint32_t sy = smem_u32(smem) + L.fstg + (uint32_t)grp * kFwdStg + (uint32_t)quad * kFwdBox + (uint32_t)(lane & 3) * 4u;
+    const uint32_t swz = (uint32_t)(lane >> 2) & 7u;
+    const bool lo_rows = p.npass == 3;
     int it = grp;
     for (long tile = t_first + grp; tile < t_end; tile += kGroups, it += kGroups) {
       const int a = it & 1;
       const uint32_t aph = (uint32_t)(it >> 1) & 1u;
       const int b = (int)(tile / p.tiles_per_img);
-      const long px = (tile - (long)b * p.tiles_per_img) * 128 + t;
+      const int t_in_img = (int)(tile - (long)b * p.tiles_per_img);
+      const long px = (long)t_in_img * 128 + t;
       const size_t base = (size_t)b * p.Co * p.P + px;
       const int s = it % p.S;
       const uint32_t sdz = smem_u32(smem) + L.stages + (uint32_t)s * L.stage_bytes + L.dz + (uint32_t)t * 4u;
@@ -439,6 +528,9 @@
           for (int j = 0; j < kCW; j++) dcur[j] = (part * kCW + j < p.Cz) ? lds_f32(sdz + (uint32_t)(part * kCW + j) * 512u) : 0.f;
           mbar_arrive(&empty[s]);
         }
+      }
+      if (FWD && it >= kGroups) {
+        mbar_wait(&stg_empty[grp], (uint32_t)((it >> 1) - 1) & 1u);
       }
       mbar_wait(&acc_full[a], aph);
       tc_fence_after();
@@ -514,7 +606,21 @@
 #pragma unroll
           for (int j = 0; j < kCW; j++)
             if (c0 + j < p.Co) yp[(size_t)j * p.P] = v[j];
-        }
+          if (FWD) {
+#pragma unroll
+            for (int j = 0; j < kCW; j++) {
+              if (c0 + j < p.Co) {
+                const uint32_t sa = sy + (uint32_t)(c0 + j) * 128u + ((swz ^ (uint32_t)j) << 4);
+                sts_f32(sa, v[j]);
+                if (lo_rows) sts_f32(sa + 32u * 128u, tf32_lo(v[j]));
+              }
+            }
+          }
+        }
+      }
+      if (FWD) {
+        fence_proxy_async();
+        mbar_arrive(&stg_full[grp]);
       }
       tc_fence_before();
       mbar_arrive(&acc_empty[a]);
@@ -656,7 +762,8 @@
 }
 
 int b2no_tc_pointwise(const b2no_plan* plan, int which, const float* spec, float* y, float* work, int batch, int channels,
-                      long pixels, const b2no_epilogue* e, cudaStream_t st, const b2no_tc_wg* wg) {
+                      long pixels, const b2no_epilogue* e, cudaStream_t st, const b2no_tc_wg* wg, const b2no_tc_fwd* fwd) {
+  if (wg && fwd) return 1;
   if (!b2no_tc_available()) return 1;
   if (!e || !e->pw_w || !e->pw_x || e->pw_ci < 1) return 1;
   if (pixels % 128 != 0 || channels > 256 || e->pw_ci > 128 || e->pw2_ci > 128) return 1;
@@ -708,9 +815,16 @@
     p.NW = b2no_round_up(2 * p.Cxp + 1, p.MW == 64 ? 8 : 16);
     p.wpart = wg->partial;
   }
+  if (fwd) {
+    if (!spec || three_d || has2 || channels > 32 || plan->g.spec_layout != 0 || (fwd->which != 0 && fwd->which != 1)) return 1;
+    const b2no_tc_fwd_tables& tf = plan->tcf[fwd->which];
+    const int32_t* n = which == 0 ? plan->g.nout : plan->g.nin;
+    if (!tf.tb || tf.W != 128 || n[1] != 128 || tf.H != n[0] || !fwd->work || ((uintptr_t)fwd->work & 15)) return 1;
+    p.ftb = tf.tb; p.N1 = tf.N1; p.Q2 = 2 * tf.Ky; p.fwork = fwd->work;
+  }
   p.NA = 2;
-  auto tmem_cols = [&]() { return wg ? pw_tmem_cols<true>(p) : pw_tmem_cols<false>(p); };
-  auto layout = [&]() { return wg ? pw_layout<true>(p) : pw_layout<false>(p); };
+  auto tmem_cols = [&]() { return wg ? pw_tmem_cols<kVarWg>(p) : fwd ? pw_tmem_cols<kVarFwd>(p) : pw_tmem_cols<kVarPlain>(p); };
+  auto layout = [&]() { return wg ? pw_layout<kVarWg>(p) : fwd ? pw_layout<kVarFwd>(p) : pw_layout<kVarPlain>(p); };
   if (tmem_cols() > 512) p.NA = 1;
   if (tmem_cols() > 512) return 1;
   const bool extras = p.add || p.mul || p.gate_z;
@@ -719,6 +833,7 @@
   else if (!extras && !p.dact && p.act == B2NO_ACT_GELU) mode = 2;
   else if (!extras && p.dact == B2NO_ACT_GELU && p.act == B2NO_ACT_NONE && !p.preact) mode = 3;
   if (wg && mode != 1) return 1;
+  if (fwd && mode == 0) return 1;
   if (mode == 3 && (((uintptr_t)p.dz & 15) == 0) && channels <= kCW * kParts * kGroups) p.Cz = b2no_round_up(channels, 8);
   int dev = 0, max_smem = 0;
   B2NO_CHECK_CUDA(cudaGetDevice(&dev));
@@ -810,14 +925,20 @@
     k_pw_tc<M, W><<<(unsigned)grid, kThreads, L.total, st>>>(tm1, tm2, tm3, p);                                           \
   } while (0)
   if (wg) {
-    LAUNCH(1, true);
+    LAUNCH(1, kVarWg);
     *wg->nblk = 2 * (int)grid;
+  } else if (fwd) {
+    switch (mode) {
+      case 1: LAUNCH(1, kVarFwd); break;
+      case 2: LAUNCH(2, kVarFwd); break;
+      default: LAUNCH(3, kVarFwd); break;
+    }
   } else {
     switch (mode) {
-      case 1: LAUNCH(1, false); break;
-      case 2: LAUNCH(2, false); break;
-      case 3: LAUNCH(3, false); break;
-      default: LAUNCH(0, false); break;
+      case 1: LAUNCH(1, kVarPlain); break;
+      case 2: LAUNCH(2, kVarPlain); break;
+      case 3: LAUNCH(3, kVarPlain); break;
+      default: LAUNCH(0, kVarPlain); break;
     }
   }
 #undef LAUNCH
diff --git a/pde_policylearning_b200/functional.py b/pde_policylearning_b200/functional.py
--- a/pde_policylearning_b200/functional.py
+++ b/pde_policylearning_b200/functional.py
@@ -15,6 +15,10 @@
 
 def _fused_wgrad_ok(g: torch.Tensor) -> bool:
     return g.is_cuda
+
+
+def _fused_fwd_ok(t: torch.Tensor) -> bool:
+    return t.is_cuda
 
 
 def _geom_has_overlap(geom: SpecGeom) -> bool:
@@ -104,20 +108,22 @@
         need_grad = any(ctx.needs_input_grad)
         saved, meta = [], []
         cur = x
+        xh_next = None
         b2d = _contig(bias_all.detach().reshape(L, -1).float())
         for l in range(L):
             pw_w = params[l * per]
             det = [c.detach() for c in params[l * per + 1:(l + 1) * per]]
             B, ci = cur.shape[:2]
             co = det[0].shape[1]
-            xh = ops.dft_forward(plan, 0, cur)
+            xh = xh_next if xh_next is not None else ops.dft_forward(plan, 0, cur)
             yh = ops.mix(plan, 0, xh, det, ci, co)
             act = acts[l]
             need_z = act not in (None, "none") and need_grad
             z = torch.empty((B, co) + tuple(plan.geom.nout), dtype=torch.float32, device=x.device) if need_z else None
             pw2d = _contig(pw_w.detach().reshape(pw_w.shape[0], -1).float())
             epi = ops.make_epilogue(bias=b2d[l], pw_w=pw2d, pw_x=cur, preact=z, act=act)
-            y = ops.dft_inverse(plan, 0, yh, epi)
+            fused = ops.dft_inverse_fwd(plan, 0, yh, epi, 0) if l < L - 1 and _fused_fwd_ok(cur) else None
+            y, xh_next = fused if fused is not None else (ops.dft_inverse(plan, 0, yh, epi), None)
             saved += [cur, xh, z if z is not None else cur.new_empty(0), pw2d] + det
             meta.append((tuple(pw_w.shape), ci, co, need_z))
             cur = y
@@ -140,12 +146,14 @@
         g = _contig(gy.float())
         if meta[L - 1][3]:
             g = ops.act_bwd(g, saved[(L - 1) * per_s + 2], acts[L - 1])
+        gyh_next = None
         for l in range(L - 1, -1, -1):
             x, xh, _, pw2d = saved[l * per_s: l * per_s + 4]
             det = list(saved[l * per_s + 4: (l + 1) * per_s])
             pw_shape, ci, co, _ = meta[l]
             need = ctx.needs_input_grad[5 + l * per: 5 + (l + 1) * per]
-            gyh = ops.dft_forward(plan, 1, g)
+            gyh = gyh_next if gyh_next is not None else ops.dft_forward(plan, 1, g)
+            gyh_next = None
             if any(need[1:]):
                 dcs = ops.mix_dw(plan, xh, gyh, det, needs_zero=_geom_has_overlap(geom))
                 for j in range(nc):
@@ -164,7 +172,8 @@
                     if need_wgrad:
                         dpw, _ = ops.pw_wgrad(g, x, need_bias=need_bias, db_out=db_out)
                         grads[l * per] = dpw.reshape(pw_shape)
-                    g = ops.dft_inverse(plan, 1, gxh, epi)
+                    ff = ops.dft_inverse_fwd(plan, 1, gxh, epi, 1) if zprev is not None and _fused_fwd_ok(g) else None
+                    g, gyh_next = ff if ff is not None else (ops.dft_inverse(plan, 1, gxh, epi), None)
                 else:
                     g = fused[0]
                     grads[l * per] = fused[1].reshape(pw_shape)
diff --git a/pde_policylearning_b200/ops.py b/pde_policylearning_b200/ops.py
--- a/pde_policylearning_b200/ops.py
+++ b/pde_policylearning_b200/ops.py
@@ -337,6 +337,23 @@
     return y, dw, db
 
 
+def dft_inverse_fwd(plan: Plan, which: int, spec: torch.Tensor, epi: Epilogue, fwd_which: int):
+    _require_cuda(spec)
+    assert spec.dtype == torch.complex64 and spec.is_contiguous()
+    B, Cc = plan.spec_bc(spec)
+    grid = plan.geom.nout if which == 0 else plan.geom.nin
+    y = torch.empty((B, Cc) + tuple(grid), dtype=torch.float32, device=spec.device)
+    work = plan.workspace(B, Cc)
+    fspec = torch.empty(plan.spec_shape(B, Cc), dtype=torch.complex64, device=spec.device)
+    fwork = torch.empty(B * Cc * grid[0] * 2 * plan.kept[-1], dtype=torch.float32, device=spec.device)
+    rc = _lib.lib().b2no_dft_inverse_fwd(plan.handle, which, _ptr(spec), _ptr(y), _ptr(work), B, Cc, math.prod(grid),
+                                         C.byref(epi), fwd_which, _ptr(fspec), _ptr(fwork), _stream())
+    if rc == -2:
+        return None
+    check(rc, "dft_inverse_fwd")
+    return y, fspec
+
+
 def mlp_head_fwd(x, w1, b1, w2, b2, act="gelu") -> torch.Tensor:
     B, ci = x.shape[:2]
     grid = tuple(x.shape[2:])
```

Result: slower. 28460 (median of 6 runs) (-5.3%).
